# bluecube/codecad

Measured on AMD Instinct MI355X. Metric: SDF Mvoxels/s (grid_eval+subdivision), 512^3 menger_sponge, higher is better.
Workload: dtype f32

## Files before the change

### codecad_amd/csrc/hip_util.hip

```cpp
#include <hip/hip_runtime.h>
#include <hip/hiprtc.h>

#include <algorithm>
#include <atomic>
#include <cmath>
#include <cstdio>
#include <cstdlib>
#include <cstring>
#include <mutex>
#include <sstream>
#include <string>
#include <vector>

#include <dirent.h>
#include <dlfcn.h>
#include <fcntl.h>
#include <spawn.h>
#include <sys/stat.h>
#include <sys/wait.h>
#include <unistd.h>

extern char** environ;

#include "../../include/hip_util.h"
// ... 35 lines not shown
    size_t lds;
    size_t regfile_bytes;
    int voxels_per_lane;
};

}

struct hu_tape_s {
    Rec* recs_dev = nullptr;
    Rec* recs_do_dev = nullptr;
    float* extra_dev = nullptr;
    int n_instr = 0;
    int n_regs = 0;
    int n_slots = 0;
    int n_point_slots = 0, n_result_slots = 0;
    int flags = 0;
    sdf::SpecProgram program;
    struct SpecKernels* spec = nullptr;
    std::string spec_source;
    sdf::SpecMeta spec_meta;
};

namespace {

bool distance_only(const hu_tape_s* t)
{
    static const bool forced_full = [] { const char* e = getenv("HU_FULL_INTERPRETER"); return e && e[0] == '1'; }();
    return !forced_full && t->recs_do_dev != nullptr;
}

int launch_shape(const hu_tape_s* t, LaunchShape& ls, bool distance_only_kernel, int max_voxels_per_lane = 2,
                 bool lanes_are_independent = false)
{
    static const int forced = [] { const char* e = getenv("HU_VOXELS_PER_LANE"); return e ? atoi(e) : 0; }();
    const size_t lane_bytes = distance_only_kernel ? (size_t)t->n_point_slots * 16 + (size_t)t->n_result_slots * 4
                                                   : (size_t)t->n_slots * 16;
    const size_t two_voxel_limit = distance_only_kernel ? 48 * 1024 : 32 * 1024;
    const int by_rule = (forced == 1 || forced == 2) ? forced : ((lane_bytes * 2 * 256 <= two_voxel_limit) ? 2 : 1);
    const int wanted = by_rule < max_voxels_per_lane ? by_rule : max_voxels_per_lane;
    const Rec* prog = distance_only_kernel ? t->recs_do_dev : t->recs_dev;
    ls.prog = prog;
    ls.n4 = (uint32_t)(distance_only_kernel ? t->n_point_slots : t->n_slots);
    for (int n = wanted; n >= 1; --n) {
        const size_t per_lane = (distance_only_kernel ? (size_t)t->n_point_slots * 16 + (size_t)t->n_result_slots * 4
                                                      : (size_t)t->n_slots * 16) * n;
        uint32_t bs = 256;
        while (bs > 64 && per_lane * bs > 48 * 1024) bs >>= 1;
        auto waves_per_cu = [&](uint32_t lanes) {
            const size_t groups = kMaxLds / (per_lane * lanes + kScratchBytes), waves = groups * (lanes / 64u);
            return waves < 32 ? waves : (size_t)32;
        };
        static const uint32_t forced_block = [] { const char* e = getenv("HU_BLOCK"); return e ? (uint32_t)atoi(e) : 0u; }();
        if (forced_block == 64u || forced_block == 128u || forced_block == 256u) bs = forced_block < bs ? forced_block : bs;
        else if (lanes_are_independent && bs == 256u && waves_per_cu(64u) > waves_per_cu(256u)) bs = 64u;
        const size_t regfile = per_lane * bs;
        if (regfile + kScratchBytes <= kMaxLds) {
            ls.block = bs;
            ls.regfile_bytes = regfile;
            ls.lds = regfile + kScratchBytes;
            ls.voxels_per_lane = n;
            return HU_OK;
        }
    }
    return fail(HU_ERR_UNSUPPORTED, "tape keeps " + std::to_string(t->n_slots) +
                                        " values live at once; at most 159 fit the 160 KiB LDS register file");
}

template <typename K>
int allow_big_lds(K kernel)
{
    HU_HIP(hipFuncSetAttribute(reinterpret_cast<const void*>(kernel), hipFuncAttributeMaxDynamicSharedMemorySize, (int)kMaxLds));
    return HU_OK;
}

template <int N>
int ensure_attrs_n()
{
    int rc;
    if ((rc = allow_big_lds(k_grid_eval<InterpEval<false>, 0, N>))) return rc;
    if ((rc = allow_big_lds(k_grid_eval<InterpEval<false>, 1, N>))) return rc;
    if ((rc = allow_big_lds(k_grid_eval<InterpEval<true>, 1, N>))) return rc;
    if ((rc = allow_big_lds(k_grid_eval_blocks<InterpEval<false>, 0, N>))) return rc;
    if ((rc = allow_big_lds(k_grid_eval_blocks<InterpEval<false>, 1, N>))) return rc;
    if ((rc = allow_big_lds(k_grid_eval_blocks<InterpEval<true>, 1, N>))) return rc;
    if ((rc = allow_big_lds(k_classify<InterpEval<false>, false, false, N>))) return rc;
    if ((rc = allow_big_lds(k_classify<InterpEval<false>, false, true, N>))) return rc;
    if ((rc = allow_big_lds(k_classify<InterpEval<false>, true, false, N>))) return rc;
    if ((rc = allow_big_lds(k_classify<InterpEval<false>, true, true, N>))) return rc;
    if ((rc = allow_big_lds(k_classify<InterpEval<true>, false, false, N>))) return rc;
    if ((rc = allow_big_lds(k_classify<InterpEval<true>, false, true, N>))) return rc;
    if ((rc = allow_big_lds(k_classify<InterpEval<true>, true, false, N>))) return rc;
    if ((rc = allow_big_lds(k_classify<InterpEval<true>, true, true, N>))) return rc;
    return HU_OK;
}

int ensure_attrs()
{
    static thread_local int done_for_device = -1;
    int dev = 0;
    HU_HIP(hipGetDevice(&dev));
    if (done_for_device == dev) return HU_OK;
    int rc;
    if ((rc = ensure_attrs_n<1>())) return rc;
    if ((rc = ensure_attrs_n<2>())) return rc;
    HU_HIP(hu_render::allow_big_lds(kMaxLds));
    HU_HIP(hu_interference::allow_big_lds(kMaxLds));
    HU_HIP(hu_clearance::allow_big_lds(kMaxLds));
    done_for_device = dev;
    return HU_OK;
}

uint32_t brick_tiles(uint32_t nx, uint32_t sy, uint32_t sz)
{
    return (nx % 4u == 0u && sy % 4u == 0u && sz % 8u == 0u) ? 1u : 0u;
}
bool boxes_worthwhile(uint64_t nx, uint64_t sy, uint64_t sz)
{
    const uint64_t padded = ((nx + 3u) & ~3ull) * ((sy + 3u) & ~3ull) * ((sz + 7u) & ~7ull);
    return padded <= 2u * nx * sy * sz;
}

uint32_t units_per_launch(uint32_t chunks, uint32_t threads)
{
    const uint64_t by_items = 0xffffffffull / threads / chunks, by_groups = 0x7fffffffull / chunks;
    const uint64_t n = by_items < by_groups ? by_items : by_groups;
    return n < 1 ? 1u : (uint32_t)n;
}

int check_dims(const uint32_t dims[3], uint64_t& cells)
{
    if (!dims) return fail(HU_ERR_BAD_ARG, "dims is NULL");
    if (dims[0] == 0 || dims[1] == 0 || dims[2] == 0) return fail(HU_ERR_BAD_ARG, "dims must be >= 1 on every axis");
    cells = (uint64_t)dims[0] * dims[1] * dims[2];
    return HU_OK;
}

}

struct SpecKernels {
    std::vector<hipModule_t> modules;
    uint32_t groups = 0;
    hipFunction_t dense[2] = {nullptr, nullptr};
    hipFunction_t blocks[2] = {nullptr, nullptr};
    hipFunction_t dense_ragged[2] = {nullptr, nullptr};
    hipFunction_t blocks_ragged[2] = {nullptr, nullptr};
    hipFunction_t dense_runs[2] = {nullptr, nullptr};
    hipFunction_t blocks_runs[2] = {nullptr, nullptr};
    hipFunction_t classify[2][2] = {{nullptr, nullptr}, {nullptr, nullptr}};
    hipFunction_t ray_caster = nullptr, bitmap = nullptr;
    hipFunction_t box_masks = nullptr;
    bool deferred = false;
    double coord_limit = 0.0;
    int tabs[6] = {0, 0, 0, 0, 0, 0};
    int prune_words = 0;
    int prune_bits = 0;
    bool prune_all = false;
    struct MaskBuffer { hipStream_t stream; uint32_t* ptr; size_t bytes; };
    std::vector<MaskBuffer> mask_buffers;
};

namespace {

constexpr int kSpecVoxelsPerLane = 2;
constexpr uint32_t kSpecBlock = 256;

uint32_t spec_flags(const hu_tape_s* t, double max_abs_coordinate)
{
    static const bool off = [] { const char* e = getenv("HU_INRANGE"); return e && e[0] == '0'; }();
    return (!off && t->spec && max_abs_coordinate < t->spec->coord_limit) ? sdf::kFlagInRange : 0u;
}
double grid_reach(const float corner[3], float step, const uint32_t dims[3])
{
    double m = 0.0;
    for (int c = 0; c < 3; ++c) {
        const double a = std::fabs((double)corner[c]), b = std::fabs((double)corner[c] + (double)step * (double)dims[c]);
        m = std::max(m, std::max(a, b));
    }
    return m;
}
double list_reach(double resolution, double ox, double oy, double oz, double block_extent)
{
    return 2147483648.0 * std::fabs(resolution) + std::max(std::fabs(ox), std::max(std::fabs(oy), std::fabs(oz))) + std::fabs(block_extent);
}

bool defer_directions()
{
    static const bool off = [] { const char* e = getenv("HU_DEFER_DIRECTIONS"); return e && e[0] == '0'; }();
    return !off;
}

std::string generate_source(const hu_tape_s* t, sdf::SpecMeta* meta = nullptr)
{
    return sdf::specialised_source(t->program, defer_directions(), meta);
}
uint32_t box_table_bytes(const SpecKernels* k)
{
    return (uint32_t)((k->tabs[0] + k->tabs[1] + k->tabs[2]) * sdf::BoxTabs::kAxis + (k->tabs[3] + k->tabs[4]) * sdf::BoxTabs::kPairX +
                      k->tabs[5] * sdf::BoxTabs::kPairYZ) * 4u;
}

void keep_programs(hu_tape_s* t, const sdf::DecodedTape& d)
{
    t->program.full = d.recs;
    t->program.dist = d.recs_do;
    t->program.n_slots = d.n_slots;
    t->program.n_point_slots = d.n_point_slots;
    t->program.n_result_slots = d.n_result_slots;
}

struct SpecEval { const float* extra; uint32_t flags; };

constexpr int kSpecKernelCount = 19;
constexpr uint32_t spec_bit(int i) { return 1u << i; }
constexpr uint32_t kSpecGroupOf[kSpecKernelCount] = {spec_bit(0), spec_bit(1), spec_bit(2), spec_bit(3), spec_bit(4), spec_bit(5), spec_bit(6), spec_bit(7),
                                                      spec_bit(8), spec_bit(9), spec_bit(10), spec_bit(11), spec_bit(12), spec_bit(13), spec_bit(14),
                                                      spec_bit(15), spec_bit(16), spec_bit(17), spec_bit(18)};
static_assert(HU_SPEC_DENSE == (spec_bit(0) | spec_bit(1) | spec_bit(10) | spec_bit(11) | spec_bit(12) | spec_bit(15) | spec_bit(16)), "hip_util.h");
static_assert(HU_SPEC_BLOCKS == (spec_bit(2) | spec_bit(3) | spec_bit(10) | spec_bit(13) | spec_bit(14) | spec_bit(17) | spec_bit(18)), "hip_util.h");
static_assert(HU_SPEC_CLASSIFY == (spec_bit(4) | spec_bit(5) | spec_bit(6) | spec_bit(7) | spec_bit(10)), "hip_util.h");
static_assert(HU_SPEC_RENDER == (spec_bit(8) | spec_bit(9)), "hip_util.h");
static_assert(HU_SPEC_ALL == (HU_SPEC_DENSE | HU_SPEC_BLOCKS | HU_SPEC_CLASSIFY | HU_SPEC_RENDER) && HU_SPEC_ALL == spec_bit(kSpecKernelCount) - 1u, "hip_util.h");
const char* const kSpecKernelNames[kSpecKernelCount] = {
    "sdfk::k_grid_eval<sdfk::JitEval, 0, 2>",           "sdfk::k_grid_eval<sdfk::JitEval, 1, 2>",
    "sdfk::k_grid_eval_blocks<sdfk::JitEval, 0, 2>",    "sdfk::k_grid_eval_blocks<sdfk::JitEval, 1, 2>",
    "sdfk::k_classify<sdfk::JitEval, false, false, 2>", "sdfk::k_classify<sdfk::JitEval, false, true, 2>",
    "sdfk::k_classify<sdfk::JitEval, true, false, 2>",  "sdfk::k_classify<sdfk::JitEval, true, true, 2>",
    "sdfk::k_ray_caster<sdfk::JitEval>",                "sdfk::k_bitmap<sdfk::JitEval>",
    "sdfk::k_box_masks<sdfk::JitEval>",
    "sdfk::k_grid_eval_ragged<sdfk::JitEval, 0, 2>",        "sdfk::k_grid_eval_ragged<sdfk::JitEval, 1, 2>",
    "sdfk::k_grid_eval_blocks_ragged<sdfk::JitEval, 0, 2>", "sdfk::k_grid_eval_blocks_ragged<sdfk::JitEval, 1, 2>",
    "sdfk::k_grid_eval_runs<sdfk::JitEval, 0, 2>",          "sdfk::k_grid_eval_runs<sdfk::JitEval, 1, 2>",
    "sdfk::k_grid_eval_blocks_runs<sdfk::JitEval, 0, 2>",   "sdfk::k_grid_eval_blocks_runs<sdfk::JitEval, 1, 2>"};

int prepare_masks(hu_tape_s* t, MaskArgs& m, hipStream_t stream, const uint32_t** masks)
{
    *masks = nullptr;
    SpecKernels* k = t->spec;
    if (!k || !k->box_masks || k->prune_words <= 0 || m.n_boxes == 0) return HU_OK;
    static const bool off = [] { const char* e = getenv("HU_PRUNE_RUN"); return e && e[0] == '0'; }();
    if (off) return HU_OK;
    const size_t bytes = (size_t)m.n_boxes * (size_t)k->prune_words * sizeof(uint32_t);
    SpecKernels::MaskBuffer* buf = nullptr;
    for (auto& b : k->mask_buffers) if (b.stream == stream) buf = &b;
    if (!buf || buf->bytes < bytes) {
        hipStreamCaptureStatus capturing = hipStreamCaptureStatusNone;
        if (stream && hipStreamIsCapturing(stream, &capturing) == hipSuccess && capturing != hipStreamCaptureStatusNone) return HU_OK;
        (void)hipGetLastError();
        if (!buf) { k->mask_buffers.push_back(SpecKernels::MaskBuffer{stream, nullptr, 0}); buf = &k->mask_buffers.back(); }
        if (buf->ptr) HU_HIP(hipFree(buf->ptr));
        buf->ptr = nullptr; buf->bytes = 0;
        const size_t want = bytes + bytes / 2 + 4096;
        HU_HIP(hipMalloc((void**)&buf->ptr, want));
        buf->bytes = want;
    }
    m.out = buf->ptr;
    SpecEval ev{t->extra_dev, 0u};
    void* args[] = {&ev, &m};
    HU_HIP(hipModuleLaunchKernel(k->box_masks, (m.n_boxes + 63u) / 64u, 1, 1, 64, 1, 1, 0, stream, args, nullptr));
    *masks = buf->ptr;
    return HU_OK;
}

}

int hu_fail_external(int code, const char* message)
{
    if (code == HU_ERR_HIP) (void)hipGetLastError();
    return fail(code, message);
}

extern "C" {

int hu_abi_version(void) { return HU_ABI_VERSION; }
const char* hu_last_error(void) { return g_last_error.c_str(); }

int hu_device_count(int* count)
{
    if (!count) return fail(HU_ERR_BAD_ARG, "count is NULL");
    int n = 0;
    hipError_t e = hipGetDeviceCount(&n);
    if (e != hipSuccess) {
        *count = 0;
        return fail(HU_ERR_NO_DEVICE, std::string("hipGetDeviceCount: ") + hipGetErrorString(e));
    }
    *count = n;
    return HU_OK;
}

int hu_set_device(int ordinal)
{
    HU_HIP(hipSetDevice(ordinal));
    return HU_OK;
}

int hu_device_name(int ordinal, char* buf, size_t buflen)
{
    if (!buf || !buflen) return fail(HU_ERR_BAD_ARG, "buf is NULL");
    hipDeviceProp_t prop;
    HU_HIP(hipGetDeviceProperties(&prop, ordinal));
    std::snprintf(buf, buflen, "%s (%s, %d CUs)", prop.name, prop.gcnArchName, prop.multiProcessorCount);
    return HU_OK;
}

int hu_synchronize(void)
{
    HU_HIP(hipDeviceSynchronize());
    return HU_OK;
}

int hu_malloc(void** out_dev, size_t bytes)
{
    if (!out_dev) return fail(HU_ERR_BAD_ARG, "out_dev is NULL");
    *out_dev = nullptr;
    HU_HIP(hipMalloc(out_dev, bytes ? bytes : 1));
    return HU_OK;
}

int hu_free(void* dev)
{
    if (dev) HU_HIP(hipFree(dev));
    return HU_OK;
}

int hu_host_alloc(void** out_host, size_t bytes)
{
    if (!out_host) return fail(HU_ERR_BAD_ARG, "out_host is NULL");
    HU_HIP(hipHostMalloc(out_host, bytes ? bytes : 1, hipHostMallocDefault));
    return HU_OK;
}

int hu_host_free(void* host)
{
    if (host) HU_HIP(hipHostFree(host));
    return HU_OK;
}

int hu_memcpy_h2d(void* dst, const void* src, size_t n, void* stream)
{
    HU_HIP(hipMemcpyAsync(dst, src, n, hipMemcpyHostToDevice, (hipStream_t)stream));
    return HU_OK;
}

int hu_memcpy_d2h(void* dst, const void* src, size_t n, void* stream)
{
    HU_HIP(hipMemcpyAsync(dst, src, n, hipMemcpyDeviceToHost, (hipStream_t)stream));
    return HU_OK;
}

int hu_memcpy_d2d(void* dst, const void* src, size_t n, void* stream)
{
    HU_HIP(hipMemcpyAsync(dst, src, n, hipMemcpyDeviceToDevice, (hipStream_t)stream));
// ... 21 lines not shown
    return HU_OK;
}

int hu_stream_synchronize(void* s)
{
    HU_HIP(hipStreamSynchronize((hipStream_t)s));
    return HU_OK;
}

int hu_stream_wait_event(void* s, void* ev)
{
    HU_HIP(hipStreamWaitEvent((hipStream_t)s, (hipEvent_t)ev, 0));
    return HU_OK;
}

int hu_event_create(void** out)
{
    if (!out) return fail(HU_ERR_BAD_ARG, "out is NULL");
    hipEvent_t e;
    HU_HIP(hipEventCreate(&e));
    *out = e;
    return HU_OK;
}

int hu_event_destroy(void* e)
{
    if (e) HU_HIP(hipEventDestroy((hipEvent_t)e));
    return HU_OK;
}

int hu_event_record(void* e, void* s)
{
    HU_HIP(hipEventRecord((hipEvent_t)e, (hipStream_t)s));
    return HU_OK;
}

int hu_event_synchronize(void* e)
{
    HU_HIP(hipEventSynchronize((hipEvent_t)e));
    return HU_OK;
}

int hu_event_elapsed_ms(void* a, void* b, float* out_ms)
{
    if (!out_ms) return fail(HU_ERR_BAD_ARG, "out_ms is NULL");
    HU_HIP(hipEventElapsedTime(out_ms, (hipEvent_t)a, (hipEvent_t)b));
    return HU_OK;
}

int hu_tape_create(const float* tape, size_t n, hu_tape* out)
{
    if (!tape || !out) return fail(HU_ERR_BAD_ARG, "tape/out is NULL");
    *out = nullptr;
    sdf::DecodedTape d;
    std::string err = sdf::decode_tape(tape, n, d);
    if (!err.empty()) return fail(HU_ERR_BAD_TAPE, "malformed tape: " + err);
    hu_tape_s* t = new hu_tape_s();
    t->n_instr = d.n_instructions;
    t->n_regs = d.n_regs;
    t->n_slots = d.n_slots;
    t->n_point_slots = d.n_point_slots;
    t->n_result_slots = d.n_result_slots;
    t->flags = d.direction_feeds_distance ? 1 : 0;
    keep_programs(t, d);
    hipError_t e = hipMalloc((void**)&t->recs_dev, d.fused.size() * sizeof(Rec));
    if (e == hipSuccess && !d.fused_do.empty()) {
        e = hipMalloc((void**)&t->recs_do_dev, d.fused_do.size() * sizeof(Rec));
        if (e == hipSuccess) e = hipMemcpy(t->recs_do_dev, d.fused_do.data(), d.fused_do.size() * sizeof(Rec), hipMemcpyHostToDevice);
    }
    if (e == hipSuccess) e = hipMalloc((void**)&t->extra_dev, d.extra.size() * sizeof(float));
    if (e == hipSuccess) e = hipMemcpy(t->recs_dev, d.fused.data(), d.fused.size() * sizeof(Rec), hipMemcpyHostToDevice);
    if (e == hipSuccess) e = hipMemcpy(t->extra_dev, d.extra.data(), d.extra.size() * sizeof(float), hipMemcpyHostToDevice);
    if (e != hipSuccess) {
        (void)hipFree(t->recs_dev);
        (void)hipFree(t->recs_do_dev);
        (void)hipFree(t->extra_dev);
        delete t;
        return fail(HU_ERR_HIP, std::string("tape upload: ") + hipGetErrorString(e));
    }
    *out = t;
    return HU_OK;
}

int hu_tape_destroy(hu_tape t)
{
    if (!t) return HU_OK;
    if (t->spec) {
        for (auto& b : t->spec->mask_buffers) (void)hipFree(b.ptr);
        for (hipModule_t m : t->spec->modules) (void)hipModuleUnload(m);
        delete t->spec;
    }
    (void)hipFree(t->recs_dev);
    (void)hipFree(t->recs_do_dev);
    (void)hipFree(t->extra_dev);
    delete t;
    return HU_OK;
}

int hu_tape_info(hu_tape t, int* n_instructions, int* n_registers, int* flags)
{
    if (!t) return fail(HU_ERR_BAD_ARG, "tape is NULL");
    if (n_instructions) *n_instructions = t->n_instr;
    if (n_registers) *n_registers = t->n_slots;
    if (flags) *flags = t->flags;
    return HU_OK;
}

int hu_grid_eval_slab(hu_tape t, const float corner[4], float step, const uint32_t dims[3],
                      uint32_t x0, uint32_t x_count, int layout, void* out_dev, void* stream)
{
    if (!t || !corner || !out_dev) return fail(HU_ERR_BAD_ARG, "NULL argument");
    if (layout != 0 && layout != 1) return fail(HU_ERR_BAD_ARG, "layout must be 0 (float4) or 1 (pymcubes float)");
    uint64_t cells;
    int rc;
    if ((rc = check_dims(dims, cells))) return rc;
    if ((uint64_t)x0 + x_count > dims[0]) return fail(HU_ERR_BAD_ARG, "slab exceeds the grid's x extent");
    const uint64_t plane = (uint64_t)dims[1] * dims[2];
    if (plane >= (1ull << 30)) return fail(HU_ERR_BAD_ARG, "dims[1]*dims[2] must be below 2^30");
    const uint32_t spec_max_x = [&] { const uint32_t m = (uint32_t)((1ull << 30) / plane); return m >= 16u ? m & ~15u : m; }();
    const bool spec_ragged = t->spec && t->spec->deferred && !(brick_tiles(x_count, dims[1], dims[2]) && (x_count <= spec_max_x || spec_max_x % 4u == 0u));
    const bool spec_runs = spec_ragged && !boxes_worthwhile(x_count < spec_max_x ? x_count : spec_max_x, dims[1], dims[2]);
    if (t->spec && t->spec->dense[layout] && (!spec_ragged || (spec_runs ? t->spec->dense_runs[layout] : t->spec->dense_ragged[layout]))) {
        const uint32_t max_x = spec_max_x;
        SpecEval ev{t->extra_dev, spec_flags(t, grid_reach(corner, step, dims))};
        float cx = corner[0], cy = corner[1], cz = corner[2];
        uint32_t sx = dims[0];
        Dim sy = make_dim(dims[1]), sz = make_dim(dims[2]);
        for (uint32_t done = 0; done < x_count;) {
            const uint32_t nx = (x_count - done < max_x) ? (x_count - done) : max_x;
            uint32_t n_cells = (uint32_t)(nx * plane), xs = x0 + done;
            void* o = (layout == 0) ? (void*)(static_cast<float4*>(out_dev) + (size_t)done * plane) : out_dev;
            uint32_t boxes = (t->spec->deferred && !spec_runs) ? 1u : 0u;
            const bool ragged = boxes && !brick_tiles(nx, dims[1], dims[2]);
            static const uint32_t run_block = [] { const char* e = getenv("HU_RUN_BLOCK"); const int v = e ? atoi(e) : 0; return (v == 64 || v == 128 || v == 256) ? (uint32_t)v : 256u; }();
            const uint32_t block = boxes ? kSpecBlock : run_block;
            static const uint32_t store_bound_kib = [] { const char* e = getenv("HU_STORE_BOUND_LDS"); const int v = e ? atoi(e) : 40; return (uint32_t)((v >= 0 && v <= 64) ? v : 40); }();
            const uint32_t idle_lds = (layout == 0 && !boxes && !t->spec->deferred && t->n_instr <= 16) ? store_bound_kib * 1024u : 0u;
            const uint32_t per_block = block * kSpecVoxelsPerLane;
            uint32_t grid = (n_cells + per_block - 1) / per_block;
            const uint32_t* masks = nullptr;
            if (boxes) {
                grid = ((nx + 15u) / 16u) * ((dims[1] + 15u) / 16u) * ((dims[2] + 15u) / 16u);
                MaskArgs m{};
                m.mode = 0u; m.n_boxes = grid; m.chunks = grid; m.boxes_y = (dims[1] + 15u) / 16u; m.boxes_z = (dims[2] + 15u) / 16u;
                m.nx = nx; m.ny = dims[1]; m.nz = dims[2]; m.xs0 = xs; m.cx = cx; m.cy = cy; m.cz = cz; m.step = step;
                if ((layout == 1 || t->spec->prune_all) && (rc = prepare_masks(t, m, (hipStream_t)stream, &masks))) return rc;
            }
            if (spec_runs) {
                void* args[] = {&ev, &cx, &cy, &cz, &step, &sx, &sy, &sz, &xs, &n_cells, &o};
                HU_HIP(hipModuleLaunchKernel(t->spec->dense_runs[layout], grid, 1, 1, block, 1, 1, 0u, (hipStream_t)stream, args, nullptr));
            } else {
                void* args[] = {&ev, &cx, &cy, &cz, &step, &sx, &sy, &sz, &xs, &n_cells, &boxes, &o, &masks};
                HU_HIP(hipModuleLaunchKernel(ragged ? t->spec->dense_ragged[layout] : t->spec->dense[layout], grid, 1, 1, block, 1, 1,
                                             boxes ? box_table_bytes(t->spec) : idle_lds, (hipStream_t)stream, args, nullptr));
            }
            done += nx;
        }
        return HU_OK;
    }
    LaunchShape ls;
    if ((rc = launch_shape(t, ls, layout == 1 && distance_only(t), 2, true))) return rc;
    if ((rc = ensure_attrs())) return rc;
    const uint32_t max_x = (uint32_t)((1ull << 30) / plane);
    for (uint32_t done = 0; done < x_count;) {
        const uint32_t nx = (x_count - done < max_x) ? (x_count - done) : max_x;
        const uint32_t n_cells = (uint32_t)(nx * plane);
        const uint32_t per_block = ls.block * ls.voxels_per_lane;
        const uint32_t blocks = (n_cells + per_block - 1) / per_block;
        void* o = (layout == 0) ? (void*)(static_cast<float4*>(out_dev) + (size_t)done * plane) : out_dev;
#define HU_LAUNCH_DENSE(L, D, NV)                                                                                  \
    hipLaunchKernelGGL((k_grid_eval<InterpEval<D>, L, NV>), dim3(blocks), dim3(ls.block), ls.lds, (hipStream_t)stream, \
                       (InterpEval<D>{ls.prog, t->extra_dev, ls.n4}), corner[0], corner[1], corner[2], step, dims[0],  \
                       make_dim(dims[1]), make_dim(dims[2]), x0 + done, n_cells,                                       \
                       0u , o, (const uint32_t*)nullptr)
        const bool d_only = layout == 1 && distance_only(t);
        if (ls.voxels_per_lane == 2) {
            if (layout == 0) HU_LAUNCH_DENSE(0, false, 2);
            else if (d_only) HU_LAUNCH_DENSE(1, true, 2);
            else HU_LAUNCH_DENSE(1, false, 2);
        } else {
            if (layout == 0) HU_LAUNCH_DENSE(0, false, 1);
            else if (d_only) HU_LAUNCH_DENSE(1, true, 1);
            else HU_LAUNCH_DENSE(1, false, 1);
        }
#undef HU_LAUNCH_DENSE
        HU_HIP(hipGetLastError());
        done += nx;
    }
    return HU_OK;
}

int hu_grid_eval(hu_tape t, const float corner[4], float step, const uint32_t dims[3], void* out_dev, void* stream)
{
    if (!dims) return fail(HU_ERR_BAD_ARG, "dims is NULL");
    return hu_grid_eval_slab(t, corner, step, dims, 0, dims[0], 0, out_dev, stream);
}

int hu_grid_eval_pymcubes(hu_tape t, const float corner[4], float step, const uint32_t dims[3], void* out_dev, void* stream)
{
    if (!dims) return fail(HU_ERR_BAD_ARG, "dims is NULL");
    return hu_grid_eval_slab(t, corner, step, dims, 0, dims[0], 1, out_dev, stream);
}

static int grid_eval_blocks_impl(hu_tape t, const int32_t* blocks_dev, uint32_t n_blocks, const uint32_t* n_dev, double resolution,
                                 const double origin[3], float step, const uint32_t dims[3], int layout,
                                 void* out_dev, void* stream)
{
    if (!t || !origin || !out_dev || (!blocks_dev && n_blocks)) return fail(HU_ERR_BAD_ARG, "NULL argument");
    if (layout != 0 && layout != 1) return fail(HU_ERR_BAD_ARG, "layout must be 0 or 1");
    uint64_t cells;
    int rc;
    if ((rc = check_dims(dims, cells))) return rc;
    if (cells > (1ull << 24)) return fail(HU_ERR_BAD_ARG, "a block may have at most 2^24 cells (256^3)");
    if (n_blocks == 0) return HU_OK;
    const bool blocks_ragged = t->spec && t->spec->deferred && !brick_tiles(dims[0], dims[1], dims[2]);
    const bool blocks_runs = blocks_ragged && !boxes_worthwhile(dims[0], dims[1], dims[2]);
    if (t->spec && t->spec->blocks[layout] && (!blocks_ragged || (blocks_runs ? t->spec->blocks_runs[layout] : t->spec->blocks_ragged[layout]))) {
        const uint32_t per_block = kSpecBlock * kSpecVoxelsPerLane;
        uint32_t chunks = (uint32_t)((cells + per_block - 1) / per_block);
        uint32_t bricks = 0u;
        const bool ragged = blocks_ragged && !blocks_runs;
        if (t->spec->deferred && !blocks_runs) {
            const uint32_t bxn = (dims[0] + 15u) / 16u, byn = (dims[1] + 15u) / 16u, bzn = (dims[2] + 15u) / 16u;
            bricks = (byn << 16) | bzn;
            chunks = bxn * byn * bzn;
        }
        const double extent = (double)step * (double)std::max(dims[0], std::max(dims[1], dims[2]));
        SpecEval ev{t->extra_dev, spec_flags(t, list_reach(resolution, origin[0], origin[1], origin[2], extent))};
        const int4* b = (const int4*)blocks_dev;
        double res = resolution, ox = origin[0], oy = origin[1], oz = origin[2];
        uint32_t sx = dims[0];
        Dim sy = make_dim(dims[1]), sz = make_dim(dims[2]);
        const uint32_t piece = units_per_launch(chunks, kSpecBlock);
        for (uint32_t b0 = 0; b0 < n_blocks; b0 += piece) {
            uint32_t first = b0;
            const uint32_t count = n_blocks - b0 < piece ? n_blocks - b0 : piece;
            const uint32_t* masks = nullptr;
            if (bricks) {
                MaskArgs m{};
                m.mode = 1u; m.n_boxes = chunks * count; m.chunks = chunks; m.boxes_y = bricks >> 16; m.boxes_z = bricks & 0xffffu;
                m.nx = dims[0]; m.ny = dims[1]; m.nz = dims[2]; m.unit_base = b0; m.units = b; m.n_units_dev = n_dev; m.step = step;
                m.res = res; m.ox = ox; m.oy = oy; m.oz = oz;
                if ((layout == 1 || t->spec->prune_all) && (rc = prepare_masks(t, m, (hipStream_t)stream, &masks))) return rc;
            }
            if (blocks_runs) {
                void* args[] = {&ev, &b, &n_dev, &first, &chunks, &res, &ox, &oy, &oz, &step, &sx, &sy, &sz, &out_dev};
                HU_HIP(hipModuleLaunchKernel(t->spec->blocks_runs[layout], chunks * count, 1, 1, kSpecBlock, 1, 1, 0u, (hipStream_t)stream, args, nullptr));
            } else {
                void* args[] = {&ev, &b, &n_dev, &first, &chunks, &bricks, &res, &ox, &oy, &oz, &step, &sx, &sy, &sz, &out_dev, &masks};
                HU_HIP(hipModuleLaunchKernel(ragged ? t->spec->blocks_ragged[layout] : t->spec->blocks[layout], chunks * count, 1, 1, kSpecBlock, 1, 1,
                                             bricks ? box_table_bytes(t->spec) : 0u, (hipStream_t)stream, args, nullptr));
            }
        }
        return HU_OK;
    }
    LaunchShape ls;
    if ((rc = launch_shape(t, ls, layout == 1 && distance_only(t), 2, true))) return rc;
    if ((rc = ensure_attrs())) return rc;
    const uint32_t per_block = ls.block * ls.voxels_per_lane;
    const uint32_t chunks = (uint32_t)((cells + per_block - 1) / per_block);
    const dim3 block(ls.block);
    const uint32_t piece = units_per_launch(chunks, ls.block);
#define HU_LAUNCH_BLOCKS(L, D, NV)                                                                                 \
    hipLaunchKernelGGL((k_grid_eval_blocks<InterpEval<D>, L, NV>), grid, block, ls.lds, (hipStream_t)stream,           \
                       (InterpEval<D>{ls.prog, t->extra_dev, ls.n4}), (const int4*)blocks_dev, n_dev, b0, chunks, 0u, resolution, \
                       origin[0], origin[1], origin[2], step, dims[0], make_dim(dims[1]), make_dim(dims[2]), out_dev, (const uint32_t*)nullptr)
    const bool d_only = layout == 1 && distance_only(t);
    for (uint32_t b0 = 0; b0 < n_blocks; b0 += piece) {
        const dim3 grid(chunks * (n_blocks - b0 < piece ? n_blocks - b0 : piece));
        if (ls.voxels_per_lane == 2) {
            if (layout == 0) HU_LAUNCH_BLOCKS(0, false, 2);
            else if (d_only) HU_LAUNCH_BLOCKS(1, true, 2);
            else HU_LAUNCH_BLOCKS(1, false, 2);
        } else {
            if (layout == 0) HU_LAUNCH_BLOCKS(0, false, 1);
            else if (d_only) HU_LAUNCH_BLOCKS(1, true, 1);
            else HU_LAUNCH_BLOCKS(1, false, 1);
        }
    }
#undef HU_LAUNCH_BLOCKS
    HU_HIP(hipGetLastError());
    return HU_OK;
}

int hu_grid_eval_blocks(hu_tape t, const int32_t* blocks_dev, uint32_t n_blocks, double resolution,
                        const double origin[3], float step, const uint32_t dims[3], int layout,
                        void* out_dev, void* stream)
{
    return grid_eval_blocks_impl(t, blocks_dev, n_blocks, nullptr, resolution, origin, step, dims, layout, out_dev, stream);
}

int hu_grid_eval_blocks_indirect(hu_tape t, const int32_t* blocks_dev, const uint32_t* n_blocks_dev, uint32_t max_blocks,
                                 double resolution, const double origin[3], float step, const uint32_t dims[3], int layout,
                                 void* out_dev, void* stream)
{
    if (!n_blocks_dev) return fail(HU_ERR_BAD_ARG, "n_blocks_dev is NULL");
    return grid_eval_blocks_impl(t, blocks_dev, max_blocks, n_blocks_dev, resolution, origin, step, dims, layout, out_dev, stream);
}

}

namespace {

template <bool MASS, bool BATCH>
int launch_classify(hu_tape t, ClassifyArgs& a, uint32_t n_parents, const uint32_t dims[3], void* stream)
{
    uint64_t cells;
    int rc;
    if ((rc = check_dims(dims, cells))) return rc;
    if (cells > (1ull << 24)) return fail(HU_ERR_BAD_ARG, "at most 2^24 cells (256^3) per block: cell indices are uchar4");
    if (dims[0] > 256 || dims[1] > 256 || dims[2] > 256)
        return fail(HU_ERR_BAD_ARG, "grid size > 256 would overflow the uchar4 cell index (reference subdivision.py:206-208)");
    if (n_parents == 0) return HU_OK;
    if (t->spec && t->spec->classify[MASS ? 1 : 0][BATCH ? 1 : 0]) {
        const uint32_t per_block = kSpecBlock * kSpecVoxelsPerLane;
        a.sx = dims[0]; a.sy = dims[1]; a.sz = dims[2];
        a.dy = make_dim(dims[1]); a.dz = make_dim(dims[2]);
        a.chunks = (uint32_t)((cells + per_block - 1) / per_block);
        a.scratch_offset = 0;
        a.boxes = 0;

        const uint64_t bxn = (dims[0] + 15u) / 16u, byn = (dims[1] + 15u) / 16u, bzn = (dims[2] + 15u) / 16u;
        uint64_t enough = t->spec->prune_bits > 0 ? 64u : 8192u;
        if (const char* e = getenv("HU_CLASSIFY_BOX_MIN")) enough = (uint64_t)atoll(e);
        if (t->spec->deferred && cells > 256u && bxn * byn * bzn * n_parents >= enough && boxes_worthwhile(dims[0], dims[1], dims[2])) {
            a.boxes = ((uint32_t)byn << 16) | (uint32_t)bzn;
            a.chunks = (uint32_t)(bxn * byn * bzn);
            a.scratch_offset = box_table_bytes(t->spec);
        }
        const double extent = (double)a.step * (double)std::max(dims[0], std::max(dims[1], dims[2]));
        const float c3[3] = {a.cx, a.cy, a.cz};
        const double reach = !BATCH ? grid_reach(c3, a.step, dims)
                             : MASS ? HUGE_VAL
                                    : list_reach(a.res, a.ox, a.oy, a.oz, extent + std::fabs((double)a.int_step * a.res));
        SpecEval ev{t->extra_dev, spec_flags(t, reach)};
        const uint32_t piece = units_per_launch(a.chunks, kSpecBlock);
        for (uint32_t p0 = 0; p0 < n_parents; p0 += piece) {
            a.parent_base = p0;
            a.masks = nullptr;
            if (a.boxes) {
                MaskArgs m{};
                m.mode = !BATCH ? 2u : MASS ? 4u : 3u;
                m.n_boxes = a.chunks * (n_parents - p0 < piece ? n_parents - p0 : piece); m.chunks = a.chunks;
                m.boxes_y = a.boxes >> 16; m.boxes_z = a.boxes & 0xffffu; m.nx = dims[0]; m.ny = dims[1]; m.nz = dims[2];
                m.unit_base = p0; m.units = a.parents; m.n_units_dev = a.n_parents_dev; m.cx = a.cx; m.cy = a.cy; m.cz = a.cz; m.step = a.step;
                m.int_step = a.int_step; m.dimension = a.dimension; m.res = a.res; m.ox = a.ox; m.oy = a.oy; m.oz = a.oz; m.s = a.s;
                if ((rc = prepare_masks(t, m, (hipStream_t)stream, &a.masks))) return rc;
            }
            void* args[] = {&ev, &a};
            HU_HIP(hipModuleLaunchKernel(t->spec->classify[MASS ? 1 : 0][BATCH ? 1 : 0],
                                         a.chunks * (n_parents - p0 < piece ? n_parents - p0 : piece), 1, 1, kSpecBlock, 1, 1,
                                         (unsigned)(a.scratch_offset + kScratchBytes), (hipStream_t)stream, args, nullptr));
        }
        return HU_OK;
    }
    LaunchShape ls;
    if ((rc = launch_shape(t, ls, distance_only(t)))) return rc;
    if ((rc = ensure_attrs())) return rc;
    a.sx = dims[0];
    a.sy = dims[1];
    a.sz = dims[2];
    a.dy = make_dim(dims[1]);
    a.dz = make_dim(dims[2]);
    const uint32_t per_block = ls.block * ls.voxels_per_lane;
    a.chunks = (uint32_t)((cells + per_block - 1) / per_block);
    a.scratch_offset = (uint32_t)ls.regfile_bytes;
    a.boxes = 0;
    a.masks = nullptr;
    const dim3 block(ls.block);
    const bool d_only = distance_only(t);
    const uint32_t piece = units_per_launch(a.chunks, ls.block);
#define HU_LAUNCH_CLASSIFY(D, NV)                                                                                \
    hipLaunchKernelGGL((k_classify<InterpEval<D>, MASS, BATCH, NV>), grid, block, ls.lds, (hipStream_t)stream,     \
                       (InterpEval<D>{ls.prog, t->extra_dev, ls.n4}), a)
    for (uint32_t p0 = 0; p0 < n_parents; p0 += piece) {
        a.parent_base = p0;
        const dim3 grid(a.chunks * (n_parents - p0 < piece ? n_parents - p0 : piece));
        if (ls.voxels_per_lane == 2) {
            if (d_only) HU_LAUNCH_CLASSIFY(true, 2);
            else HU_LAUNCH_CLASSIFY(false, 2);
        } else {
            if (d_only) HU_LAUNCH_CLASSIFY(true, 1);
            else HU_LAUNCH_CLASSIFY(false, 1);
        }
    }
#undef HU_LAUNCH_CLASSIFY
    HU_HIP(hipGetLastError());
    return HU_OK;
}

}

extern "C" {

int hu_subdivision_step(hu_tape t, const float corner[4], float step, float threshold, const uint32_t dims[3],
                        uint32_t* counter_dev, void* list_dev, void* stream)
{
    if (!t || !corner || !counter_dev || !list_dev) return fail(HU_ERR_BAD_ARG, "NULL argument");
    ClassifyArgs a;
    std::memset(&a, 0, sizeof(a));
    a.cx = corner[0]; a.cy = corner[1]; a.cz = corner[2];
    a.step = step; a.thr = threshold;
    a.counter = counter_dev; a.list = list_dev; a.capacity = 0xffffffffu;
    return launch_classify<false, false>(t, a, 1, dims, stream);
}

int hu_mass_properties(hu_tape t, const float corner[4], float step, float threshold, const uint32_t dims[3],
                       uint32_t* sum_dev, uint32_t* counter_dev, void* list_dev, void* stream)
{
    if (!t || !corner || !sum_dev || !counter_dev || !list_dev) return fail(HU_ERR_BAD_ARG, "NULL argument");
    ClassifyArgs a;
    std::memset(&a, 0, sizeof(a));
    a.cx = corner[0]; a.cy = corner[1]; a.cz = corner[2];
    a.step = step; a.thr = threshold;
    a.counter = counter_dev; a.list = list_dev; a.capacity = 0xffffffffu;
    a.sums = sum_dev;
    return launch_classify<true, false>(t, a, 1, dims, stream);
}

int hu_subdivision_level(hu_tape t, const int32_t* parents_dev, uint32_t n_parents, int32_t int_step,
                         const uint32_t dims[3], int dimension, double resolution, const double origin[3],
                         float step, float threshold, uint32_t* counter_dev, int32_t* children_dev,
                         uint32_t capacity, void* stream)
{
    if (!t || !origin || !counter_dev || (!children_dev && capacity) || (!parents_dev && n_parents))
        return fail(HU_ERR_BAD_ARG, "NULL argument");
    if (dimension != 2 && dimension != 3) return fail(HU_ERR_BAD_ARG, "dimension must be 2 or 3");
    ClassifyArgs a;
    std::memset(&a, 0, sizeof(a));
    a.parents = parents_dev;
    a.int_step = int_step; a.dimension = dimension;
    a.res = resolution; a.ox = origin[0]; a.oy = origin[1]; a.oz = origin[2];
    a.step = step; a.thr = threshold;
    a.counter = counter_dev; a.list = children_dev; a.capacity = capacity;
    return launch_classify<false, true>(t, a, n_parents, dims, stream);
}

int hu_subdivision_level_indirect(hu_tape t, const int32_t* parents_dev, const uint32_t* n_parents_dev, uint32_t max_parents,
                                  int32_t int_step, const uint32_t dims[3], int dimension, double resolution,
                                  const double origin[3], float step, float threshold, uint32_t* counter_dev,
                                  int32_t* children_dev, uint32_t capacity, void* stream)
{
    if (!t || !origin || !counter_dev || !n_parents_dev || (!children_dev && capacity) || (!parents_dev && max_parents))
        return fail(HU_ERR_BAD_ARG, "NULL argument");
    if (dimension != 2 && dimension != 3) return fail(HU_ERR_BAD_ARG, "dimension must be 2 or 3");
    ClassifyArgs a;
    std::memset(&a, 0, sizeof(a));
    a.parents = parents_dev;
    a.n_parents_dev = n_parents_dev;
    a.int_step = int_step; a.dimension = dimension;
    a.res = resolution; a.ox = origin[0]; a.oy = origin[1]; a.oz = origin[2];
    a.step = step; a.thr = threshold;
    a.counter = counter_dev; a.list = children_dev; a.capacity = capacity;
    return launch_classify<false, true>(t, a, max_parents, dims, stream);
}

int hu_subdivision_level_owned(hu_tape t, const int32_t* parents_dev, const uint32_t* n_parents_dev, uint32_t max_parents,
                               int32_t int_step, const uint32_t dims[3], int dimension, double resolution,
                               const double origin[3], float step, float threshold, uint32_t* counter_dev,
                               int32_t* children_dev, uint32_t capacity, uint32_t world, uint32_t rank, void* stream)
{
    if (!t || !origin || !counter_dev || !n_parents_dev || (!children_dev && capacity) || (!parents_dev && max_parents))
        return fail(HU_ERR_BAD_ARG, "NULL argument");
    if (dimension != 2 && dimension != 3) return fail(HU_ERR_BAD_ARG, "dimension must be 2 or 3");
    if (world == 0 || rank >= world) return fail(HU_ERR_BAD_ARG, "rank must be below world");
    ClassifyArgs a;
    std::memset(&a, 0, sizeof(a));
    a.parents = parents_dev;
    a.n_parents_dev = n_parents_dev;
    a.int_step = int_step; a.dimension = dimension;
    a.res = resolution; a.ox = origin[0]; a.oy = origin[1]; a.oz = origin[2];
    a.step = step; a.thr = threshold;
    a.counter = counter_dev; a.list = children_dev; a.capacity = capacity;
    a.own = make_dim(world); a.own_rank = rank;
    return launch_classify<false, true>(t, a, max_parents, dims, stream);
}

int hu_mass_properties_level_owned(hu_tape t, const double* parents_dev, const uint32_t* n_parents_dev, uint32_t max_parents, double s,
                                   const uint32_t dims[3], float step, float threshold, uint32_t* sums_dev,
                                   uint32_t* counter_dev, double* children_dev, uint32_t capacity, uint32_t world, uint32_t rank, void* stream)
{
// ... 628 lines not shown
    for (int i = 0; i < kSpecKernelCount; ++i)
        if (kSpecGroupOf[i] & groups) (void)hiprtcAddNameExpression(prog, kSpecKernelNames[i]);
    std::vector<const char*> opts;
    for (const std::string& w : options) opts.push_back(w.c_str());
    const hiprtcResult rc = hiprtcCompileProgram(prog, (int)opts.size(), opts.data());
    if (rc != HIPRTC_SUCCESS) {
        size_t n = 0;
        std::string log;
        if (hiprtcGetProgramLogSize(prog, &n) == HIPRTC_SUCCESS && n > 1) {
            log.resize(n);
            (void)hiprtcGetProgramLog(prog, &log[0]);
        }
        (void)hiprtcDestroyProgram(&prog);
        return fail(HU_ERR_UNSUPPORTED, std::string("hipRTC compile failed: ") + hiprtcGetErrorString(rc) + "\n" + log.substr(0, 4000));
    }
    size_t size = 0;
    (void)hiprtcGetCodeSize(prog, &size);
    img.code.resize(size);
    (void)hiprtcGetCode(prog, img.code.data());
    img.lowered.clear();
    for (int i = 0; i < kSpecKernelCount; ++i) {
        if (!(kSpecGroupOf[i] & groups)) continue;
        const char* name = kSpecKernelNames[i];
        const char* lowered = nullptr;
        if (hiprtcGetLoweredName(prog, name, &lowered) != HIPRTC_SUCCESS || !lowered) {
            (void)hiprtcDestroyProgram(&prog);
            return fail(HU_ERR_UNSUPPORTED, std::string("kernel missing from the specialised module: ") + name);
        }
        img.lowered.emplace_back(lowered);
    }
    (void)hiprtcDestroyProgram(&prog);
    return HU_OK;
}

static int specialised_image(const std::string& src, const char* include_dir, const char* cache_dir, bool only_if_cached, uint32_t groups,
                             SpecImage& img, int* from_cache, bool replace_cached = false)
{
    if (from_cache) *from_cache = 0;
    img.code.clear();
    const std::vector<std::string> options = spec_options(include_dir, spec_source_is_big(src.size()));
    uint64_t key[2];
    std::string path;
    const bool cached = cache_dir && *cache_dir && spec_cache_key(src, include_dir, options, groups, key);
    if (cached) {
        path = spec_cache_path(cache_dir, key);
        if (!replace_cached && spec_cache_load(path, key, groups, img)) {
            if (from_cache) *from_cache = 1;
            return HU_OK;
        }
        img.code.clear();
    }
    if (only_if_cached) return HU_OK;
    int rc = HU_ERR_UNSUPPORTED;
    for (int attempt = 0; attempt < 2 && rc != HU_OK; ++attempt) {
        const std::string pch = spec_pch(include_dir, cache_dir, options, g_pch_beside_refused);
        if (pch.empty()) break;
        std::vector<std::string> with = options;
        with.push_back("-include-pch");
        with.push_back(pch);
        if ((rc = compile_specialised(src, with, groups, img))) {
            const bool in_dir = cache_dir && *cache_dir && pch.compare(0, std::strlen(cache_dir), cache_dir) == 0;
            if (in_dir) {
                g_pch_refused = true;
                (void)std::remove(pch.c_str());
            } else {
                g_pch_beside_refused = true;
            }
        }
    }
    if (rc != HU_OK && (rc = compile_specialised(src, options, groups, img))) return rc;
    if (cached) {
        spec_cache_store(cache_dir, path, key, img);
        spec_cache_prune(cache_dir);
    }
    return HU_OK;
}

int hu_tape_compile_cached(const float* tape, size_t n, const char* include_dir, const char* cache_dir, size_t* code_bytes,
                           int* from_cache)
{
    return hu_tape_compile_groups(tape, n, include_dir, cache_dir, HU_SPEC_ALL, code_bytes, from_cache);
}

int hu_tape_compile_groups(const float* tape, size_t n, const char* include_dir, const char* cache_dir, uint32_t groups,
                           size_t* code_bytes, int* from_cache)
{
    if (!tape || !include_dir) return fail(HU_ERR_BAD_ARG, "NULL argument");
    if (groups == 0 || (groups & ~(uint32_t)HU_SPEC_ALL)) return fail(HU_ERR_BAD_ARG, "groups must be a non-empty set of HU_SPEC_* bits");
    sdf::DecodedTape d;
    const std::string err = sdf::decode_tape(tape, n, d);
    if (!err.empty()) return fail(HU_ERR_BAD_TAPE, "malformed tape: " + err);
    hu_tape_s t;
    t.n_slots = d.n_slots;
    keep_programs(&t, d);
    SpecImage img;
    int rc;
    if ((rc = specialised_image(generate_source(&t), include_dir, cache_dir, false, groups, img, from_cache))) return rc;
    if (code_bytes) *code_bytes = img.code.size();
    return HU_OK;
}

int hu_spec_pch_prepare(const char* include_dir, const char* dir, char* path, size_t capacity)
{
    if (!include_dir || !dir) return fail(HU_ERR_BAD_ARG, "NULL argument");
    const std::string pch = spec_pch(include_dir, dir, spec_options(include_dir, false), true);
    const std::string pch_big = spec_pch(include_dir, dir, spec_options(include_dir, true), true);
    if (path && capacity) std::snprintf(path, capacity, "%s%s%s", pch.c_str(), (pch.empty() || pch_big.empty()) ? "" : "\n", pch_big.c_str());
    return HU_OK;
}

int hu_tape_compile_check(const float* tape, size_t n, const char* include_dir, size_t* code_bytes)
{
    return hu_tape_compile_cached(tape, n, include_dir, nullptr, code_bytes, nullptr);
}

int hu_tape_specialize_cached(hu_tape t, const char* include_dir, const char* cache_dir, int only_if_cached, int* from_cache)
{
    return hu_tape_specialize_groups(t, include_dir, cache_dir, only_if_cached, HU_SPEC_ALL, from_cache);
}

static int load_specialised(hu_tape t, const SpecImage& img, uint32_t set, hipError_t* why)
{
    hipModule_t module = nullptr;
    hipFunction_t loaded[kSpecKernelCount] = {};
    hipError_t e = hipModuleLoadData(&module, img.code.data());
    size_t next = 0;
    for (int i = 0; i < kSpecKernelCount && e == hipSuccess; ++i)
        if (kSpecGroupOf[i] & set) e = (next < img.lowered.size()) ? hipModuleGetFunction(&loaded[i], module, img.lowered[next++].c_str()) : hipErrorNotFound;
    if (e != hipSuccess) {
        if (module) (void)hipModuleUnload(module);
        (void)hipGetLastError();
        if (why) *why = e;
        return HU_ERR_HIP;
    }
    if (!t->spec) t->spec = new SpecKernels();
    SpecKernels* k = t->spec;
    hipFunction_t* slots[kSpecKernelCount] = {&k->dense[0], &k->dense[1], &k->blocks[0], &k->blocks[1],
                                              &k->classify[0][0], &k->classify[0][1], &k->classify[1][0], &k->classify[1][1],
                                              &k->ray_caster, &k->bitmap, &k->box_masks,
                                              &k->dense_ragged[0], &k->dense_ragged[1], &k->blocks_ragged[0], &k->blocks_ragged[1],
                                              &k->dense_runs[0], &k->dense_runs[1], &k->blocks_runs[0], &k->blocks_runs[1]};
    const uint32_t missing = set & ~k->groups;
    for (int i = 0; i < kSpecKernelCount; ++i)
        if (kSpecGroupOf[i] & missing) *slots[i] = loaded[i];
    k->modules.push_back(module);
    k->groups |= missing;
    const sdf::SpecMeta& meta = t->spec_meta;
    k->deferred = meta.deferred;
    k->coord_limit = meta.coord_limit;
    k->prune_words = meta.prune_words;
    k->prune_bits = meta.prune_bits;
    k->prune_all = meta.prune_all;
    std::memcpy(k->tabs, meta.tabs, sizeof k->tabs);
    return HU_OK;
}

int hu_tape_specialize_groups(hu_tape t, const char* include_dir, const char* cache_dir, int only_if_cached, uint32_t groups, int* from_cache)
{
    if (from_cache) *from_cache = 0;
    if (!t || !include_dir) return fail(HU_ERR_BAD_ARG, "NULL argument");
    if (groups & ~(uint32_t)HU_SPEC_ALL) return fail(HU_ERR_BAD_ARG, "groups must be a set of HU_SPEC_* bits");
    auto missing = [&] { return t->spec ? (groups & ~t->spec->groups) : groups; };
    if (missing() == 0) return HU_OK;
    if (t->spec_source.empty()) t->spec_source = generate_source(t, &t->spec_meta);
    const std::string& src = t->spec_source;
    const bool cache = cache_dir && *cache_dir;
    bool all_cached = true;
    for (int step = 0; step < 3 && missing(); ++step) {
        if (step < 2 && !cache) continue;
        if (step == 2 && only_if_cached) break;
        std::vector<uint32_t> sets;
        if (step == 1) {
            for (int i = 0; i < kSpecKernelCount; ++i)
                if ((kSpecGroupOf[i] & missing()) && kSpecGroupOf[i] != groups) sets.push_back(kSpecGroupOf[i]);
        } else {
            sets.push_back(step == 0 ? groups : missing());
        }
        for (uint32_t set : sets) {
            for (int attempt = 0; attempt < 2; ++attempt) {
                SpecImage img;
                int crc, cached = 0;
                if ((crc = specialised_image(src, include_dir, cache_dir, step < 2, set, img, &cached, attempt != 0))) return crc;
                if (img.code.empty()) break;
                hipError_t e = hipSuccess;
                if (load_specialised(t, img, set, &e) == HU_OK) {
                    all_cached = all_cached && cached;
                    break;
                }
                if (step < 2) break;
                if (!cached || attempt == 1) return fail(HU_ERR_HIP, std::string("loading the specialised module: ") + hipGetErrorString(e));
            }
        }
    }
    if (from_cache) *from_cache = (all_cached && missing() == 0) ? 1 : 0;
    return HU_OK;
}

int hu_tape_specialize(hu_tape t, const char* include_dir) { return hu_tape_specialize_cached(t, include_dir, nullptr, 0, nullptr); }

static int launch_process_polygon(bool batch, PolygonArgs& a, uint32_t n_blocks, void* stream)
{
    if (a.gx < 2 || a.gy < 2) return fail(HU_ERR_BAD_ARG, "the corner grid needs at least 2x2 samples");
    if (a.gx > 512 || a.gy > 512) return fail(HU_ERR_BAD_ARG, "corner grids above 512 overflow the link encoding (polygon2d.py:46)");
    if (n_blocks == 0) return HU_OK;
    if (n_blocks > 65535u) return fail(HU_ERR_BAD_ARG, "at most 65535 blocks per launch");
    const uint32_t cells = (a.gx - 1u) * (a.gy - 1u) * 2u;
    HU_HIP(hu_render::process_polygon(batch, a, dim3((cells + 255u) / 256u, n_blocks), (hipStream_t)stream));
    return HU_OK;
}

int hu_process_polygon(const float box_corner[2], float box_step, const void* corners_dev, const uint32_t grid[2],
                       void* vertices_dev, uint32_t* links_dev, uint32_t* starts_dev, uint32_t* start_counter_dev,
                       void* stream)
{
    if (!box_corner || !corners_dev || !grid || !vertices_dev || !links_dev || !starts_dev || !start_counter_dev)
        return fail(HU_ERR_BAD_ARG, "NULL argument");
    PolygonArgs a{};
    a.corners = static_cast<const float4*>(corners_dev);
    a.gx = grid[0] + 1u;
    a.gy = grid[1] + 1u;
    a.cx = box_corner[0];
    a.cy = box_corner[1];
    a.step = box_step;
    a.vertices = static_cast<float2*>(vertices_dev);
    a.links = links_dev;
    a.starts = starts_dev;
    a.start_counter = start_counter_dev;
    return launch_process_polygon(false, a, 1, stream);
}

int hu_process_polygon_blocks(const void* corners_dev, const int32_t* blocks_dev, uint32_t n_blocks, double resolution,
                              const double origin[3], float step, const uint32_t dims[2], void* vertices_dev,
                              uint32_t* links_dev, uint32_t* starts_dev, uint32_t* start_counters_dev, void* stream)
{
    if (!origin || !dims) return fail(HU_ERR_BAD_ARG, "NULL argument");
    if (n_blocks && (!corners_dev || !blocks_dev || !vertices_dev || !links_dev || !starts_dev || !start_counters_dev))
        return fail(HU_ERR_BAD_ARG, "NULL argument");
    PolygonArgs a{};
    a.corners = static_cast<const float4*>(corners_dev);
    a.gx = dims[0];
    a.gy = dims[1];
    a.step = step;
    a.blocks = reinterpret_cast<const int4*>(blocks_dev);
    a.res = resolution;
    a.ox = origin[0];
    a.oy = origin[1];
    a.vertices = static_cast<float2*>(vertices_dev);
    a.links = links_dev;
    a.starts = starts_dev;
    a.start_counter = start_counters_dev;
    return launch_process_polygon(true, a, n_blocks, stream);
}

int hu_selftest_math(uint64_t counts[4])
{
    if (!counts) return fail(HU_ERR_BAD_ARG, "counts is NULL");
    unsigned long long* dev = nullptr;
    HU_HIP(hipMalloc((void**)&dev, 4 * sizeof(unsigned long long)));
    hipError_t e = hipMemset(dev, 0, 4 * sizeof(unsigned long long));
    if (e == hipSuccess) {
        e = hu_render::selftest_math(dev);
    }
    unsigned long long host[4] = {0, 0, 0, 0};
    if (e == hipSuccess) e = hipMemcpy(host, dev, sizeof host, hipMemcpyDeviceToHost);
    (void)hipFree(dev);
    if (e != hipSuccess) return fail(HU_ERR_HIP, std::string("hu_selftest_math: ") + hipGetErrorString(e));
    for (int i = 0; i < 4; ++i) counts[i] = host[i];
    return HU_OK;
}

int hu_selftest_minmax3(uint64_t counts[3])
{
    if (!counts) return fail(HU_ERR_BAD_ARG, "counts is NULL");
    unsigned long long* dev = nullptr;
    HU_HIP(hipMalloc((void**)&dev, 3 * sizeof(unsigned long long)));
    hipError_t e = hipMemset(dev, 0, 3 * sizeof(unsigned long long));
    if (e == hipSuccess) e = hu_render::selftest_minmax3(dev);
    unsigned long long host[3] = {0, 0, 0};
    if (e == hipSuccess) e = hipMemcpy(host, dev, sizeof host, hipMemcpyDeviceToHost);
    (void)hipFree(dev);
    if (e != hipSuccess) return fail(HU_ERR_HIP, std::string("hu_selftest_minmax3: ") + hipGetErrorString(e));
    for (int i = 0; i < 3; ++i) counts[i] = host[i];
    return HU_OK;
}

int hu_tape_source(const float* tape, size_t n, char* buf, size_t capacity, size_t* needed)
{
    if (!tape || !needed || (!buf && capacity)) return fail(HU_ERR_BAD_ARG, "NULL argument");
    sdf::DecodedTape d;
    const std::string err = sdf::decode_tape(tape, n, d);
    if (!err.empty()) return fail(HU_ERR_BAD_TAPE, "malformed tape: " + err);
    hu_tape_s t;
    t.n_slots = d.n_slots;
    keep_programs(&t, d);
    const std::string src = generate_source(&t);
    *needed = src.size() + 1;
    if (capacity >= src.size() + 1) std::memcpy(buf, src.c_str(), src.size() + 1);
    return HU_OK;
}

int hu_tape_listing(const float* tape, size_t n, int which, char* buf, size_t capacity, size_t* needed)
{
    if (!tape || !needed || (!buf && capacity)) return fail(HU_ERR_BAD_ARG, "NULL argument");
    if (which < 0 || which > 3) return fail(HU_ERR_BAD_ARG, "which must be 0..3");
    sdf::DecodedTape d;
    const std::string err = sdf::decode_tape(tape, n, d);
// ... 57 lines not shown
```

### codecad_amd/csrc/kernels.hpp

```cpp
#pragma once

#include "interp.hpp"

#ifdef SDF_WAVES_PER_EU
#define SDF_KERNEL_ATTRS __attribute__((amdgpu_waves_per_eu(SDF_WAVES_PER_EU, SDF_WAVES_PER_EU)))
#else
#define SDF_KERNEL_ATTRS
#endif

namespace sdfk {

using sdf::Rec;

template <bool DO> struct InterpEval {
    static constexpr bool kBricks = false;
    const Rec* prog;
    const float* extra;
    uint32_t n4;
    template <class T> __device__ __forceinline__ sdf::V4<T> operator()(T px, T py, T pz, void* lds) const
    {
        sdf::Regs<T> regs(lds, threadIdx.x, blockDim.x, n4);
        return sdf::run_tape<T, DO>(prog, extra, px, py, pz, regs);
    }
    template <class T> __device__ __forceinline__ T dist(T px, T py, T pz, void* lds) const { return (*this)(px, py, pz, lds).w; }
};


__device__ __forceinline__ float sample(float corner, float step, uint32_t i) { return corner + step * (float)i; }

struct Dim {
    uint32_t n, m, s;
};
inline Dim make_dim(uint32_t n)
{
    if (n <= 1u) return Dim{n, 0u, 0u};
    uint32_t L = 0;
    while ((1ull << L) < n) ++L;
    return Dim{n, (uint32_t)((((1ull << L) - n) << 32) / n + 1ull), L - 1u};
}
__device__ __forceinline__ uint32_t div(uint32_t x, Dim d)
{
    const uint32_t t = __umulhi(d.m, x);
    const uint32_t q = (t + ((x - t) >> 1)) >> d.s;
    return d.n == 1u ? x : q;
}

#ifndef SDF_NT_STORES
#define SDF_NT_STORES 0
#endif
typedef float f4v __attribute__((ext_vector_type(4)));
__device__ __forceinline__ void store_voxel(float4* p, float4 v)
{
#if SDF_NT_STORES
    f4v t;
    t.x = v.x; t.y = v.y; t.z = v.z; t.w = v.w;
    __builtin_nontemporal_store(t, reinterpret_cast<f4v*>(p));
#else
    *p = v;
#endif
}
__device__ __forceinline__ void store_voxel(float* p, float v)
{
#if SDF_NT_STORES
    __builtin_nontemporal_store(v, p);
#else
    *p = v;
#endif
}

template <int N> struct Pack { using T = float; };
template <> struct Pack<2> { using T = sdf::f2; };
__device__ __forceinline__ float pack(const float (&v)[1]) { return v[0]; }
__device__ __forceinline__ sdf::f2 pack(const float (&v)[2]) { return sdf::make_f2(v[0], v[1]); }

template <int N> struct Cells {
    uint32_t x[N], y[N], z[N];
    bool active[N];
    __device__ __forceinline__ Cells(uint32_t lin0, uint32_t n_cells, Dim dy, Dim dz, uint32_t stride = 1u)
    {
        const uint32_t sy = dy.n, sz = dz.n;
#pragma unroll
        for (int i = 0; i < N; ++i) {
            if (i == 0 || stride != 1u) {
                const uint32_t lin = lin0 + (uint32_t)i * stride;
                active[i] = lin < n_cells;
                const uint32_t l = active[i] ? lin : 0u;
                const uint32_t t = div(l, dz);
                z[i] = l - t * sz;
                x[i] = div(t, dy);
                y[i] = t - x[i] * sy;
            } else {
                active[i] = active[0] && (lin0 + i < n_cells);
                const bool wrap_z = z[i - 1] + 1u == sz;
                const bool wrap_y = wrap_z && (y[i - 1] + 1u == sy);
                z[i] = wrap_z ? 0u : z[i - 1] + 1u;
                y[i] = wrap_y ? 0u : (wrap_z ? y[i - 1] + 1u : y[i - 1]);
                x[i] = wrap_y ? x[i - 1] + 1u : x[i - 1];
            }
        }
    }
    __device__ __forceinline__ typename Pack<N>::T position(float corner, float step, const uint32_t (&c)[N], uint32_t c0 = 0) const
    {
        float v[N];
#pragma unroll
        for (int i = 0; i < N; ++i) v[i] = sample(corner, step, c0 + c[i]);
        return pack(v);
    }
};
__device__ __forceinline__ uint32_t sx_slab(uint32_t n_cells, uint32_t sy, uint32_t sz) { return n_cells / (sy * sz); }

template <int N> __device__ __forceinline__ uint32_t first_cell(uint32_t block)
{
    return (block * blockDim.x + (threadIdx.x & ~63u)) * N + (threadIdx.x & 63u);
}
constexpr uint32_t kLaneStride = 64u;

template <int N>
__device__ __forceinline__ void wg_compact_slots(const bool (&flag)[N], uint32_t* __restrict__ counter, uint32_t* scratch,
                                                 uint32_t (&slot)[N])
{
    const uint32_t lane = threadIdx.x & 63u, wave = threadIdx.x >> 6;
    const uint64_t below = (1ull << lane) - 1ull;
    uint32_t prefix = 0, total_w = 0;
#pragma unroll
    for (int i = 0; i < N; ++i) {
        const uint64_t mask = __ballot(flag[i]);
        prefix += __popcll(mask & below);
        total_w += __popcll(mask);
    }
    if (lane == 0) scratch[wave] = total_w;
    __syncthreads();
    if (threadIdx.x == 0) {
        const uint32_t nw = (blockDim.x + 63u) >> 6;
        uint32_t total = 0;
        for (uint32_t w = 0; w < nw; ++w) {
            uint32_t c = scratch[w];
            scratch[w] = total;
            total += c;
        }
        scratch[4] = total ? atomicAdd(counter, total) : 0u;
    }
    __syncthreads();
    slot[0] = scratch[4] + scratch[wave] + prefix;
#pragma unroll
    for (int i = 1; i < N; ++i) slot[i] = slot[i - 1] + (flag[i - 1] ? 1u : 0u);
}

__device__ __forceinline__ uint32_t wave_sum_to_last_lane(uint32_t v)
{
    v += (uint32_t)__builtin_amdgcn_update_dpp(0, (int)v, 0x111, 0xf, 0xf, false);
    v += (uint32_t)__builtin_amdgcn_update_dpp(0, (int)v, 0x112, 0xf, 0xf, false);
    v += (uint32_t)__builtin_amdgcn_update_dpp(0, (int)v, 0x114, 0xf, 0xf, false);
    v += (uint32_t)__builtin_amdgcn_update_dpp(0, (int)v, 0x118, 0xf, 0xf, false);
    v += (uint32_t)__builtin_amdgcn_update_dpp(0, (int)v, 0x142, 0xa, 0xf, false);
    v += (uint32_t)__builtin_amdgcn_update_dpp(0, (int)v, 0x143, 0xc, 0xf, false);
    return v;
}

struct BoxOut {
    void* out;
    size_t base;
    uint32_t sxa, sy, sz, xa;
    uint32_t nx;
};
template <class E> __device__ __forceinline__ float walk_coordinate(float v)
{
    if constexpr (E::kPruneAll) return sdf::opaque(v);
    else return v;
}
struct BoxTables {
    sdf::lds_float *x, *y, *z, *xy, *xz, *yz;
};
template <class E, class PR>
__device__ __forceinline__ BoxTables box_tables(const E& ev, float4* lds, float cx, float cy, float cz, float step, uint32_t xs0,
                                                uint32_t x0, uint32_t y0, uint32_t z0, uint32_t nx, uint32_t ny, uint32_t nz, const PR& pr)
{
    const uint32_t lane = threadIdx.x & 63u, wave = threadIdx.x >> 6;
    constexpr int NX = E::kTabXX, NY = E::kTabXY, NZ = E::kTabXZ, NXY = E::kPairXY, NXZ = E::kPairXZ, NYZ = E::kPairYZ;
    using Tabs = sdf::BoxTabs;
    sdf::lds_float* const tx = (sdf::lds_float*)lds;
    sdf::lds_float* const ty = tx + NX * Tabs::kAxis;
    sdf::lds_float* const tz = ty + NY * Tabs::kAxis;
    sdf::lds_float* const txy = tz + NZ * Tabs::kAxis;
    sdf::lds_float* const txz = txy + NXY * Tabs::kPairX;
    sdf::lds_float* const tyz = txz + NXZ * Tabs::kPairX;
    if constexpr (NX + NY + NZ > 0) {
        if (wave == 0u) {
            if constexpr (NX > 0)
                if (lane < nx) ev.template tab_x_x<Tabs::kAxis>(sample(cx, step, xs0 + x0 + lane), tx + lane);
        } else if (wave == 1u) {
            if constexpr (NY > 0)
                if (lane < ny) ev.template tab_x_y<Tabs::kAxis>(sample(cy, step, y0 + lane), ty + lane);
        } else if (wave == 2u) {
            if constexpr (NZ > 0)
                if (lane < nz) ev.template tab_x_z<Tabs::kAxis>(sample(cz, step, z0 + lane), tz + lane);
        }
        __syncthreads();
    }
    if constexpr (NXY + NXZ + NYZ > 0) {
        const uint32_t r = threadIdx.x >> 4, c = threadIdx.x & 15u;
        if constexpr (NXY > 0)
            if (r < ny && c < nx)
                ev.template tab_x_xy<Tabs::kPairX>(sample(cx, step, xs0 + x0 + c), sample(cy, step, y0 + r), Tabs{tx + c, ty + r, tz, txy, txz, tyz}, pr,
                                                   txy + (r * Tabs::kRowX + c));
        if constexpr (NXZ > 0)
            if (r < nz && c < nx)
                ev.template tab_x_xz<Tabs::kPairX>(sample(cx, step, xs0 + x0 + c), sample(cz, step, z0 + r), Tabs{tx + c, ty, tz + r, txy, txz, tyz}, pr,
                                                   txz + (r * Tabs::kRowX + c));
        if constexpr (NYZ > 0)
            if (r < ny && c < nz)
                ev.template tab_x_yz<Tabs::kPairYZ>(sample(cy, step, y0 + r), sample(cz, step, z0 + c), Tabs{tx, ty + r, tz + c, txy, txz, tyz}, pr,
                                                    tyz + (r * Tabs::kRowYZ + c));
        __syncthreads();
    }
    return BoxTables{tx, ty, tz, txy, txz, tyz};
}

template <class E, int LAYOUT, int N, bool RAGGED = false>
__device__ __forceinline__ void box_eval(const E& ev, float4* lds, float cx, float cy, float cz, float step, uint32_t xs0,
                                         uint32_t x0, uint32_t y0, uint32_t z0, const BoxOut& o, const uint32_t* __restrict__ masks,
                                         uint32_t box = blockIdx.x)
{
    using T = typename Pack<N>::T;
    using Tabs = sdf::BoxTabs;
    const uint32_t lane = threadIdx.x & 63u, wave = threadIdx.x >> 6;
    const uint32_t sx = o.sxa, sy = o.sy, sz = o.sz;
    const uint32_t nx = min(16u, o.nx - x0), ny = min(16u, sy - y0), nz = min(16u, sz - z0);
    const sdf::Prune<E::kPruneWords> pr = sdf::load_prune<E::kPruneWords>(masks, box);
    const BoxTables t = box_tables(ev, lds, cx, cy, cz, step, xs0, x0, y0, z0, nx, ny, nz, pr);
    sdf::lds_float* const tx = t.x; sdf::lds_float* const ty = t.y; sdf::lds_float* const tz = t.z;
    sdf::lds_float* const txy = t.xy; sdf::lds_float* const txz = t.xz; sdf::lds_float* const tyz = t.yz;
    const uint32_t nbz = RAGGED ? (nz + 7u) >> 3 : nz >> 3;
    const uint32_t bz = nbz == 2u ? (wave & 1u) : 0u, dby = 4u / nbz;
    const uint32_t zl = bz * 8u + (lane & 7u), z = z0 + zl, xl = lane >> 5;
    const bool z_inside = !RAGGED || zl < nz;
    const float pz = sample(cz, step, z);
    uint32_t yl = (nbz == 2u ? (wave >> 1) : wave) * 4u + ((lane >> 3) & 3u);
    Tabs col{tx + xl, ty + yl, tz + zl, txy + (yl * Tabs::kRowX + xl), txz + (zl * Tabs::kRowX + xl), tyz + (yl * Tabs::kRowYZ + zl)};
    const size_t plane = (size_t)sy * sz;
    size_t at = LAYOUT == 0 ? o.base + ((size_t)z + (size_t)sz * ((size_t)(y0 + yl) + (size_t)sy * (x0 + xl)))
                            : o.base + ((size_t)z + ((size_t)(o.xa + x0 + xl) + (size_t)(sy - 1u - (y0 + yl)) * sx) * sz);
    const size_t second = LAYOUT == 0 ? 2u * plane : 2u * (size_t)sz, brick = 2u * second;
    const size_t rows = (size_t)(4u * dby) * (LAYOUT == 0 ? (size_t)sz : (size_t)sx * sz);
    const uint32_t row_in_brick = (lane >> 3) & 3u, bricks_x = RAGGED ? (nx + 3u) >> 2 : nx >> 2;
    for (; (RAGGED ? yl - row_in_brick : yl) < ny; yl += 4u * dby) {
        const float py = sample(cy, step, y0 + yl);
        const bool row_inside = !RAGGED || (z_inside && yl < ny);
        Tabs tb = col;
        const auto hoisted = ev.hoist_x(py, walk_coordinate<E>(pz), tb, pr);
        size_t p = at;
#pragma unroll 1
        for (uint32_t j = 0; j < bricks_x; ++j) {
            asm volatile("" ::: "memory");
            float xs[N];
#pragma unroll
            for (int i = 0; i < N; ++i) xs[i] = sample(cx, step, xs0 + x0 + j * 4u + xl + 2u * i);
            const T px = pack(xs);
            const float pyb = walk_coordinate<E>(py), pzb = walk_coordinate<E>(pz);
            const auto prb = pr.fresh();
            if (LAYOUT == 0) {
                const sdf::V4<T> r = ev.eval_hoisted_x(px, pyb, pzb, hoisted, tb, prb);
#pragma unroll
                for (int i = 0; i < N; ++i)
                    if (!RAGGED || (row_inside && j * 4u + xl + 2u * (uint32_t)i < nx))
                        store_voxel(static_cast<float4*>(o.out) + p + (size_t)i * second, sdf::voxel(r, i));
            } else {
                const T w = ev.dist_hoisted_x(px, pyb, pzb, hoisted, tb, prb);
#pragma unroll
                for (int i = 0; i < N; ++i)
                    if (!RAGGED || (row_inside && j * 4u + xl + 2u * (uint32_t)i < nx))
                        store_voxel(static_cast<float*>(o.out) + p + (size_t)i * second, sdf::get(w, i));
            }
            tb.x += 4; tb.xy += 4; tb.xz += 4;
            p += brick;
        }
        col.y += 4u * dby; col.xy += 4u * dby * Tabs::kRowX; col.yz += 4u * dby * Tabs::kRowYZ;
        at = LAYOUT == 0 ? at + rows : at - rows;
    }
}

template <class E, int LAYOUT, int N>
__device__ __forceinline__ void grid_eval_runs(const E& ev, float4* lds, float cx, float cy, float cz, float step, uint32_t sx, Dim dy, Dim dz,
                                               uint32_t x0, uint32_t n_cells, void* __restrict__ out);

template <class E, int LAYOUT, int N, bool RAGGED>
__device__ __forceinline__ void grid_eval_boxes(const E& ev, float4* lds, float cx, float cy, float cz, float step, uint32_t sx, uint32_t sy, uint32_t sz,
                                                uint32_t x0, uint32_t n_cells, void* __restrict__ out, const uint32_t* __restrict__ masks)
{
    const uint32_t nx_slab = sx_slab(n_cells, sy, sz);
    const uint32_t boxes_z = (sz + 15u) >> 4, boxes_y = (sy + 15u) >> 4;
    uint32_t b = blockIdx.x;
#if !defined(SDF_BOX_ORDER) || SDF_BOX_ORDER
    {
        const uint32_t k = b & 7u, q = gridDim.x >> 3, r = gridDim.x & 7u;
        b = k * q + (k < r ? k : r) + (b >> 3);
    }
#endif
    const uint32_t qz = b % boxes_z, qt = b / boxes_z, qy = qt % boxes_y, qx = qt / boxes_y;
    const BoxOut o{out, 0, sx, sy, sz, LAYOUT == 0 ? 0u : x0, nx_slab};
    box_eval<E, LAYOUT, N, RAGGED>(ev, lds, cx, cy, cz, step, x0, qx * 16u, qy * 16u, qz * 16u, o, masks, b);
}

template <class E, int LAYOUT, int N>
__global__ void __launch_bounds__(256) SDF_KERNEL_ATTRS
k_grid_eval(const E ev, float cx, float cy, float cz, float step, uint32_t sx, Dim dy, Dim dz, uint32_t x0,
            uint32_t n_cells, uint32_t boxes, void* __restrict__ out, const uint32_t* __restrict__ masks)
{
    extern __shared__ float4 lds[];
    if constexpr (E::kBricks && N == 2) {
        grid_eval_boxes<E, LAYOUT, N, false>(ev, lds, cx, cy, cz, step, sx, dy.n, dz.n, x0, n_cells, out, masks);
    } else {
        grid_eval_runs<E, LAYOUT, N>(ev, lds, cx, cy, cz, step, sx, dy, dz, x0, n_cells, out);
    }
}
template <class E, int LAYOUT, int N>
__global__ void __launch_bounds__(256) SDF_KERNEL_ATTRS
k_grid_eval_ragged(const E ev, float cx, float cy, float cz, float step, uint32_t sx, Dim dy, Dim dz, uint32_t x0,
                   uint32_t n_cells, uint32_t boxes, void* __restrict__ out, const uint32_t* __restrict__ masks)
{
    extern __shared__ float4 lds[];
    if constexpr (E::kBricks && N == 2) grid_eval_boxes<E, LAYOUT, N, true>(ev, lds, cx, cy, cz, step, sx, dy.n, dz.n, x0, n_cells, out, masks);
}

template <class E, int LAYOUT, int N>
__global__ void __launch_bounds__(256) SDF_KERNEL_ATTRS
k_grid_eval_runs(const E ev, float cx, float cy, float cz, float step, uint32_t sx, Dim dy, Dim dz, uint32_t x0,
                 uint32_t n_cells, void* __restrict__ out)
{
    extern __shared__ float4 lds[];
    if constexpr (E::kBricks) grid_eval_runs<E, LAYOUT, N>(ev, lds, cx, cy, cz, step, sx, dy, dz, x0, n_cells, out);
}

template <class E, int LAYOUT, int N>
__device__ __forceinline__ void grid_eval_runs(const E& ev, float4* lds, float cx, float cy, float cz, float step, uint32_t sx, Dim dy, Dim dz,
                                               uint32_t x0, uint32_t n_cells, void* __restrict__ out)
{
    const uint32_t sy = dy.n, sz = dz.n;
    using T = typename Pack<N>::T;
    const uint32_t lin0 = first_cell<N>(blockIdx.x);
    const Cells<N> c(lin0, n_cells, dy, dz, kLaneStride);
    const T px = c.position(cx, step, c.x, x0), py = c.position(cy, step, c.y), pz = c.position(cz, step, c.z);
    if (LAYOUT == 0) {
        const sdf::V4<T> r = ev(px, py, pz, lds);
#pragma unroll
        for (int i = 0; i < N; ++i) {
            if (!c.active[i]) continue;
            store_voxel(static_cast<float4*>(out) + lin0 + (uint32_t)i * kLaneStride, sdf::voxel(r, i));
        }
    } else {
        const T w = ev.dist(px, py, pz, lds);
#pragma unroll
        for (int i = 0; i < N; ++i) {
            if (!c.active[i]) continue;
            const size_t idx = (size_t)c.z[i] + ((size_t)(x0 + c.x[i]) + (size_t)(sy - 1u - c.y[i]) * sx) * sz;
            store_voxel(static_cast<float*>(out) + idx, sdf::get(w, i));
        }
    }
}

template <class E, int LAYOUT, int N, bool BOXES, bool RAGGED = false>
__device__ __forceinline__ void grid_eval_blocks_body(const E& ev, float4* lds, const int4* __restrict__ blocks, const uint32_t* __restrict__ n_blocks_dev,
                                                      uint32_t b0, uint32_t chunks, uint32_t bricks, double res, double ox, double oy, double oz, float step,
                                                      uint32_t sx, Dim dy, Dim dz, void* __restrict__ out, const uint32_t* __restrict__ masks)
{
    const uint32_t sy = dy.n, sz = dz.n;
    using T = typename Pack<N>::T;
    const uint32_t chunk = blockIdx.x % chunks, b = b0 + blockIdx.x / chunks;
    if (n_blocks_dev && b >= *n_blocks_dev) return;
    const uint32_t cells = sx * sy * sz;
    const int4 ic = blocks[b];
    const float cx = (float)((double)ic.x * res + ox);
    const float cy = (float)((double)ic.y * res + oy);
    const float cz = (float)((double)ic.z * res + oz);
    if constexpr (BOXES) {
        const uint32_t boxes_z = bricks & 0xffffu, boxes_y = bricks >> 16;
        const uint32_t qz = chunk % boxes_z, qt = chunk / boxes_z, qy = qt % boxes_y, qx = qt / boxes_y;
        const BoxOut o{out, (size_t)b * cells, sx, sy, sz, 0u, sx};
        box_eval<E, LAYOUT, N, RAGGED>(ev, lds, cx, cy, cz, step, 0u, qx * 16u, qy * 16u, qz * 16u, o, masks);
        return;
    }
    const uint32_t lin0 = first_cell<N>(chunk);
    const Cells<N> c(lin0, cells, dy, dz, kLaneStride);
    const T px = c.position(cx, step, c.x), py = c.position(cy, step, c.y), pz = c.position(cz, step, c.z);
    const size_t base = (size_t)b * cells;
    if (LAYOUT == 0) {
        const sdf::V4<T> r = ev(px, py, pz, lds);
#pragma unroll
        for (int i = 0; i < N; ++i)
            if (c.active[i]) store_voxel(static_cast<float4*>(out) + base + lin0 + (uint32_t)i * kLaneStride, sdf::voxel(r, i));
    } else {
        const T w = ev.dist(px, py, pz, lds);
#pragma unroll
        for (int i = 0; i < N; ++i)
            if (c.active[i])
                store_voxel(static_cast<float*>(out) + base + (size_t)c.z[i] + ((size_t)c.x[i] + (size_t)(sy - 1u - c.y[i]) * sx) * sz, sdf::get(w, i));
    }
}
template <class E, int LAYOUT, int N>
__global__ void __launch_bounds__(256) SDF_KERNEL_ATTRS
k_grid_eval_blocks(const E ev, const int4* __restrict__ blocks, const uint32_t* __restrict__ n_blocks_dev, uint32_t b0,
                   uint32_t chunks, uint32_t bricks, double res, double ox, double oy, double oz, float step, uint32_t sx,
                   Dim dy, Dim dz, void* __restrict__ out, const uint32_t* __restrict__ masks)
{
    extern __shared__ float4 lds[];
    grid_eval_blocks_body<E, LAYOUT, N, (E::kBricks && N == 2)>(ev, lds, blocks, n_blocks_dev, b0, chunks, bricks, res, ox, oy, oz, step, sx, dy, dz, out, masks);
}
template <class E, int LAYOUT, int N>
__global__ void __launch_bounds__(256) SDF_KERNEL_ATTRS
k_grid_eval_blocks_ragged(const E ev, const int4* __restrict__ blocks, const uint32_t* __restrict__ n_blocks_dev, uint32_t b0,
                          uint32_t chunks, uint32_t bricks, double res, double ox, double oy, double oz, float step, uint32_t sx,
                          Dim dy, Dim dz, void* __restrict__ out, const uint32_t* __restrict__ masks)
{
    extern __shared__ float4 lds[];
    if constexpr (E::kBricks && N == 2)
        grid_eval_blocks_body<E, LAYOUT, N, true, true>(ev, lds, blocks, n_blocks_dev, b0, chunks, bricks, res, ox, oy, oz, step, sx, dy, dz, out, masks);
}

template <class E, int LAYOUT, int N>
__global__ void __launch_bounds__(256) SDF_KERNEL_ATTRS
k_grid_eval_blocks_runs(const E ev, const int4* __restrict__ blocks, const uint32_t* __restrict__ n_blocks_dev, uint32_t b0,
                        uint32_t chunks, double res, double ox, double oy, double oz, float step, uint32_t sx, Dim dy, Dim dz,
                        void* __restrict__ out)
{
    extern __shared__ float4 lds[];
    if constexpr (E::kBricks)
        grid_eval_blocks_body<E, LAYOUT, N, false>(ev, lds, blocks, n_blocks_dev, b0, chunks, 0u, res, ox, oy, oz, step, sx, dy, dz, out, nullptr);
}

struct ClassifyArgs {
    const void* parents;
    uint32_t parent_base;
    const uint32_t* n_parents_dev;
    uint32_t chunks;
    uint32_t sx, sy, sz;
    Dim dy, dz;
    float cx, cy, cz;
    float step, thr;
    int32_t int_step;
    int32_t dimension;
    double res, ox, oy, oz;
    double s;
    uint32_t* counter;
    void* list;
    uint32_t capacity;
    uint32_t* sums;
    uint32_t scratch_offset;
    uint32_t boxes;
    const uint32_t* masks;
    Dim own;
    uint32_t own_rank;
};
__device__ __forceinline__ uint32_t row_hash(uint32_t a, uint32_t b, uint32_t c, uint32_t d)
{
    uint32_t h = a * 0x9e3779b1u;
    h = (h ^ (h >> 15)) + b * 0x85ebca77u;
    h = (h ^ (h >> 13)) + c * 0xc2b2ae3du;
    h = (h ^ (h >> 16)) + d * 0x27d4eb2fu;
    return h ^ (h >> 15);
}
__device__ __forceinline__ bool owned(const ClassifyArgs& a, uint32_t parent_hash, uint32_t cell)
{
    uint32_t v = parent_hash + cell * 0x9e3779b1u;
    v = (v ^ (v >> 15)) * 0x85ebca77u;
    v ^= v >> 13;
    const bool mine = v - div(v, a.own) * a.own.n == a.own_rank;
    return a.own.n <= 1u ? true : mine;
}

template <class E, bool MASS, bool BATCH, int N>
__global__ void __launch_bounds__(256) k_classify(const E ev, const ClassifyArgs a)
{
    using T = typename Pack<N>::T;
    extern __shared__ float4 lds[];
    uint32_t* scratch = reinterpret_cast<uint32_t*>(reinterpret_cast<char*>(lds) + a.scratch_offset);
    const uint32_t b = BATCH ? a.parent_base + blockIdx.x / a.chunks : 0u;
    const uint32_t chunk = BATCH ? blockIdx.x % a.chunks : blockIdx.x;
    const uint32_t cells = a.sx * a.sy * a.sz;
    if (BATCH && a.n_parents_dev && b >= *a.n_parents_dev) return;

    float cx = a.cx, cy = a.cy, cz = a.cz;
    int4 ipar = make_int4(0, 0, 0, 0);
    double pcx = 0.0, pcy = 0.0, pcz = 0.0, pcw = 0.0;
    if (BATCH) {
        if (MASS) {
            const double4 pc = static_cast<const double4*>(a.parents)[b];
            pcx = pc.x; pcy = pc.y; pcz = pc.z; pcw = pc.w;
            const double h = a.s / 2;
            cx = (float)(pcx + h); cy = (float)(pcy + h); cz = (float)(pcz + h);
        } else {
            ipar = static_cast<const int4*>(a.parents)[b];
            const double h = (double)a.int_step / 2;
            cx = (float)(((double)ipar.x + h) * a.res + a.ox);
            cy = (float)(((double)ipar.y + h) * a.res + a.oy);
            cz = (float)(((double)ipar.z + (a.dimension == 3 ? h : 0.0)) * a.res + a.oz);
        }
    }
    if (MASS) {
        if (threadIdx.x < 10) scratch[8 + threadIdx.x] = 0u;
    }
    const uint32_t phash = !BATCH ? 0u
                           : MASS ? row_hash((uint32_t)__double2loint(pcx) ^ (uint32_t)__double2hiint(pcx), (uint32_t)__double2loint(pcy) ^ (uint32_t)__double2hiint(pcy),
                                             (uint32_t)__double2loint(pcz) ^ (uint32_t)__double2hiint(pcz), (uint32_t)__double2loint(pcw) ^ (uint32_t)__double2hiint(pcw))
                                  : row_hash((uint32_t)ipar.x, (uint32_t)ipar.y, (uint32_t)ipar.z, (uint32_t)ipar.w);

    if constexpr (E::kBricks && N == 2) {
        if (a.boxes) {
            using Tabs = sdf::BoxTabs;
            const uint32_t lane = threadIdx.x & 63u, wave = threadIdx.x >> 6;
            const uint32_t boxes_z = a.boxes & 0xffffu, boxes_y = a.boxes >> 16;
            const uint32_t qz = chunk % boxes_z, qt = chunk / boxes_z, qy = qt % boxes_y, qx = qt / boxes_y;
            const uint32_t x0 = qx * 16u, y0 = qy * 16u, z0 = qz * 16u;
            const uint32_t nx = min(16u, a.sx - x0), ny = min(16u, a.sy - y0), nz = min(16u, a.sz - z0);
            const sdf::Prune<E::kPruneWords> pr = sdf::load_prune<E::kPruneWords>(a.masks, blockIdx.x);
            const BoxTables t = box_tables(ev, lds, cx, cy, cz, a.step, 0u, x0, y0, z0, nx, ny, nz, pr);
            if (MASS) __syncthreads();
            const bool nothing_ambiguous = MASS && a.thr == 0.0f;
            const uint64_t below = (1ull << lane) - 1ull;
            uint32_t v[10] = {0, 0, 0, 0, 0, 0, 0, 0, 0, 0};
            constexpr uint32_t kStep = (uint32_t)Tabs::kPairStep;
            const uint32_t x_end = x0 + nx;
            auto brick = [&](uint32_t xv, uint32_t y, uint32_t z, float py, float pz, const Tabs& tb, const auto& hoisted, bool live) {
                const T px = sdf::make_f2(sample(cx, a.step, xv), sample(cx, a.step, xv + kStep));
                const T w = ev.dist_hoisted_x(px, walk_coordinate<E>(py), walk_coordinate<E>(pz), hoisted, tb, pr.fresh());
                bool amb[2];
#pragma unroll
                for (int i = 0; i < 2; ++i) {
                    const float wi = sdf::get(w, i);
                    const uint32_t x = xv + kStep * (uint32_t)i;
                    const bool mine = live & (x < x_end) & owned(a, phash, z + a.sz * (y + a.sy * x));
                    if (MASS) {
                        const bool in = wi <= -a.thr, inside = in && mine;
                        amb[i] = mine && !in && (wi < a.thr);
                        const uint32_t m = inside ? 1u : 0u;
                        const uint32_t xm = inside ? x : 0u, ym = inside ? y : 0u, zm = inside ? z : 0u;
                        v[0] += __umul24(xm, x); v[1] += __umul24(xm, y); v[2] += __umul24(xm, z); v[3] += xm;
                        v[4] += __umul24(ym, y); v[5] += __umul24(ym, z); v[6] += ym;
                        v[7] += __umul24(zm, z); v[8] += zm; v[9] += m;
                    } else {
                        amb[i] = mine && (wi > -a.thr) && (wi < a.thr);
                    }
                }
                if (!nothing_ambiguous) {
                    const uint64_t m0 = __ballot(amb[0]), m1 = __ballot(amb[1]);
                    const uint32_t n0 = __popcll(m0), total = n0 + __popcll(m1);
                    if (total) {
                        uint32_t base = 0u;
                        if (lane == 0u) base = atomicAdd(a.counter, total);
                        base = __builtin_amdgcn_readfirstlane(base);
                        const uint32_t slot[2] = {base + (uint32_t)__popcll(m0 & below), base + n0 + (uint32_t)__popcll(m1 & below)};
#pragma unroll
                        for (int i = 0; i < 2; ++i) {
                            if (!(amb[i] && slot[i] < a.capacity)) continue;
                            const uint32_t x = xv + kStep * (uint32_t)i;
                            if (!BATCH) {
                                static_cast<uchar4*>(a.list)[slot[i]] = make_uchar4((unsigned char)x, (unsigned char)y, (unsigned char)z, 0);
                            } else if (MASS) {
                                static_cast<double4*>(a.list)[slot[i]] =
                                    make_double4((double)x * a.s + pcx, (double)y * a.s + pcy, (double)z * a.s + pcz, pcw);
                            } else {
                                static_cast<int4*>(a.list)[slot[i]] =
                                    make_int4(ipar.x + (int)x * a.int_step, ipar.y + (int)y * a.int_step, ipar.z + (int)z * a.int_step, ipar.w);
                            }
                        }
                    }
                }
            };
            const uint32_t nbz = (nz + 7u) >> 3, bz = nbz == 2u ? (wave & 1u) : 0u, dby = 4u / nbz;
            const uint32_t zl = bz * 8u + (lane & 7u), z = z0 + zl, xl = lane >> 5;
            const float pz = sample(cz, a.step, z);
            const uint32_t row_in_brick = (lane >> 3) & 3u;
            for (uint32_t yl = (nbz == 2u ? (wave >> 1) : wave) * 4u + row_in_brick; yl - row_in_brick < ny; yl += 4u * dby) {
                const uint32_t y = y0 + yl;
                const bool live = (zl < nz) & (yl < ny);
                const float py = sample(cy, a.step, y);
                Tabs tb{t.x + xl, t.y + yl, t.z + zl, t.xy + (yl * Tabs::kRowX + xl), t.xz + (zl * Tabs::kRowX + xl), t.yz + (yl * Tabs::kRowYZ + zl)};
                const auto hoisted = ev.hoist_x(py, walk_coordinate<E>(pz), tb, pr);
#pragma unroll 1
                for (uint32_t j = 0; j < ((nx + 3u) >> 2); ++j) {
                    asm volatile("" ::: "memory");
                    brick(x0 + j * 4u + xl, y, z, py, pz, tb, hoisted, live);
                    tb.x += 4; tb.xy += 4; tb.xz += 4;
                }
            }
            if (MASS) {
#pragma unroll
                for (int i = 0; i < 10; ++i) {
                    const uint32_t sum = wave_sum_to_last_lane(v[i]);
                    if (lane == 63u && sum) atomicAdd(&scratch[8 + i], sum);
                }
                __syncthreads();
                if (threadIdx.x < 10) {
                    const uint32_t total = scratch[8 + threadIdx.x];
                    if (total) atomicAdd(&a.sums[(size_t)b * 10 + threadIdx.x], total);
                }
            }
            return;
        }
    }

    const uint32_t lin0 = (chunk * blockDim.x + threadIdx.x) * N;
    const Cells<N> c(lin0, cells, a.dy, a.dz);
    const T w = ev.dist(c.position(cx, a.step, c.x), c.position(cy, a.step, c.y), c.position(cz, a.step, c.z), lds);

    bool ambiguous[N];
    if (MASS) {
        bool inside[N];
        bool any_inside = false;
#pragma unroll
        for (int i = 0; i < N; ++i) {
            const float wi = sdf::get(w, i);
            const bool own = owned(a, phash, lin0 + (uint32_t)i);
            const bool mine = c.active[i] & own, in = wi <= -a.thr;
            inside[i] = mine & in;
            ambiguous[i] = mine & !in & (wi < a.thr);
            any_inside |= inside[i];
        }
        const uint64_t imask = __ballot(any_inside);
        __syncthreads();
        if (imask != 0ull) {
            uint32_t v[10] = {0, 0, 0, 0, 0, 0, 0, 0, 0, 0};
#pragma unroll
            for (int i = 0; i < N; ++i) {
                const uint32_t m = inside[i] ? 1u : 0u;
                const uint32_t x = c.x[i], y = c.y[i], z = c.z[i];
                const uint32_t xm = inside[i] ? x : 0u, ym = inside[i] ? y : 0u, zm = inside[i] ? z : 0u;
                v[0] += __umul24(xm, x); v[1] += __umul24(xm, y); v[2] += __umul24(xm, z); v[3] += xm;
                v[4] += __umul24(ym, y); v[5] += __umul24(ym, z); v[6] += ym;
                v[7] += __umul24(zm, z); v[8] += zm; v[9] += m;
            }
#pragma unroll
            for (int i = 0; i < 10; ++i) {
                const uint32_t sum = wave_sum_to_last_lane(v[i]);
                if ((threadIdx.x & 63u) == 63u && sum) atomicAdd(&scratch[8 + i], sum);
            }
        }
    } else {
#pragma unroll
        for (int i = 0; i < N; ++i) {
            const float wi = sdf::get(w, i);
            const bool own = owned(a, phash, lin0 + (uint32_t)i);
            ambiguous[i] = c.active[i] & own & (wi > -a.thr) & (wi < a.thr);
        }
    }

    const bool nothing_ambiguous = MASS && a.thr == 0.0f;
    uint32_t slot[N];
    if (nothing_ambiguous) {
#pragma unroll
        for (int i = 0; i < N; ++i) slot[i] = 0u;
        __syncthreads();
    } else {
        wg_compact_slots<N>(ambiguous, a.counter, scratch, slot);
    }
#pragma unroll
    for (int i = 0; i < N; ++i) {
        if (nothing_ambiguous || !(ambiguous[i] && slot[i] < a.capacity)) continue;
        const uint32_t x = c.x[i], y = c.y[i], z = c.z[i];
        if (!BATCH) {
            static_cast<uchar4*>(a.list)[slot[i]] = make_uchar4((unsigned char)x, (unsigned char)y, (unsigned char)z, 0);
        } else if (MASS) {
            static_cast<double4*>(a.list)[slot[i]] =
                make_double4((double)x * a.s + pcx, (double)y * a.s + pcy, (double)z * a.s + pcz, pcw);
        } else {
            static_cast<int4*>(a.list)[slot[i]] =
                make_int4(ipar.x + (int)x * a.int_step, ipar.y + (int)y * a.int_step, ipar.z + (int)z * a.int_step, ipar.w);
        }
    }
    if (MASS) {
        if (threadIdx.x < 10) {
            const uint32_t v = scratch[8 + threadIdx.x];
            if (v) atomicAdd(&a.sums[(size_t)b * 10 + threadIdx.x], v);
        }
    }
}

struct MaskArgs {
    uint32_t mode;
    uint32_t n_boxes;
    uint32_t chunks;
    uint32_t boxes_y, boxes_z;
    uint32_t nx, ny, nz;
    uint32_t xs0;
    uint32_t unit_base;
    const void* units;
    const uint32_t* n_units_dev;
    float cx, cy, cz, step;
    int32_t int_step, dimension;
    double res, ox, oy, oz, s;
    uint32_t* out;
};
template <class E> __global__ void __launch_bounds__(64) k_box_masks(const E ev, const MaskArgs a)
{
    if constexpr (E::kBricks) {
        constexpr int W = E::kPruneWords;
        if constexpr (W > 0) {
            const uint32_t box = blockIdx.x * blockDim.x + threadIdx.x;
            if (box >= a.n_boxes) return;
            const uint32_t unit = a.unit_base + box / a.chunks, chunk = box % a.chunks;
            sdf::Prune<W> pr;
#pragma unroll
            for (int i = 0; i < W; ++i) pr.w[i] = 0xffffffffu;
            if (!(a.n_units_dev && unit >= *a.n_units_dev)) {
                float cx = a.cx, cy = a.cy, cz = a.cz;
                if (a.mode == 1u) {
                    const int4 ic = static_cast<const int4*>(a.units)[unit];
                    cx = (float)((double)ic.x * a.res + a.ox); cy = (float)((double)ic.y * a.res + a.oy); cz = (float)((double)ic.z * a.res + a.oz);
                } else if (a.mode == 3u) {
                    const int4 ip = static_cast<const int4*>(a.units)[unit];
                    const double h = (double)a.int_step / 2;
                    cx = (float)(((double)ip.x + h) * a.res + a.ox); cy = (float)(((double)ip.y + h) * a.res + a.oy);
                    cz = (float)(((double)ip.z + (a.dimension == 3 ? h : 0.0)) * a.res + a.oz);
                } else if (a.mode == 4u) {
                    const double4 pc = static_cast<const double4*>(a.units)[unit];
                    const double h = a.s / 2;
                    cx = (float)(pc.x + h); cy = (float)(pc.y + h); cz = (float)(pc.z + h);
                }
                const uint32_t qz = chunk % a.boxes_z, qt = chunk / a.boxes_z, qy = qt % a.boxes_y, qx = qt / a.boxes_y;
                const uint32_t x0 = qx * 16u, y0 = qy * 16u, z0 = qz * 16u;
                const float ex = 0.5f * (float)(min(16u, a.nx - x0) - 1u), ey = 0.5f * (float)(min(16u, a.ny - y0) - 1u),
                            ez = 0.5f * (float)(min(16u, a.nz - z0) - 1u);
                const float hx = a.step * ex, hy = a.step * ey, hz = a.step * ez;
                ev.prune(sample(cx, a.step, a.xs0 + x0) + hx, sample(cy, a.step, y0) + hy, sample(cz, a.step, z0) + hz,
                         __builtin_fabsf(hx), __builtin_fabsf(hy), __builtin_fabsf(hz), pr);
            }
#pragma unroll
            for (int i = 0; i < W; ++i) a.out[(size_t)box * W + i] = pr.w[i];
        }
    }
}
// ... 352 lines not shown
```

### codecad_amd/csrc/specialise.hpp

```cpp
#pragma once

#include <algorithm>
#include <array>
#include <cmath>
#include <cstdio>
#include <cstdlib>
#include <cstring>
#include <functional>
#include <numeric>
#include <sstream>
#include <string>
#include <vector>

#include "tape.hpp"

namespace sdf {

struct SpecProgram {
    std::vector<Rec> full;
    std::vector<Rec> dist;
    int n_slots = 0, n_point_slots = 0, n_result_slots = 0;
};

namespace spec_detail {

inline std::string rec_literal(const Rec& r, bool clear_fold, uint32_t hdr)
{
    std::ostringstream o;
    char buf[32];
    std::snprintf(buf, sizeof buf, "0x%08xu", hdr);
    o << "Rec{" << buf << ", {";
    for (int i = 0; i < SDF_REC_DWORDS - 1; ++i) {
        uint32_t bits;
        std::memcpy(&bits, &r.p[i], 4);
        if (clear_fold && i == kFoldParam) bits = 0;
        std::snprintf(buf, sizeof buf, "0x%08xu", bits);
        o << (i ? ", " : "") << "__builtin_bit_cast(float, " << buf << ")";
    }
    o << "}}";
    return o.str();
}

inline std::string flit(float v)
{
    uint32_t bits;
    std::memcpy(&bits, &v, 4);
    char buf[48];
    std::snprintf(buf, sizeof buf, "__builtin_bit_cast(float, 0x%08xu)", bits);
    return buf;
}

inline uint32_t fold_of(const Rec& r)
{
    uint32_t f;
    std::memcpy(&f, &r.p[kFoldParam], 4);
    return f;
}

enum Kind { POINT, RESULT };
enum Role { LEAF, UNARY, WITH_POINT, SELECT, POINT_OP };

struct Node {
    Kind kind;
    Role role;
    int rec;
    uint32_t op;
    int a = -1;
    int b = -1;
};

inline bool is_leaf(uint32_t op)
{
    switch (op) {
    case OP_RECTANGLE: case OP_CIRCLE: case OP_REGULAR_POLYGON2D: case OP_POLYGON2D: case OP_SPHERE: case OP_HALF_SPACE:
    case OP_INVOLUTE_GEAR:
        return true;
    default: return false;
    }
}
inline bool is_unary_result(uint32_t op)
{
    switch (op) {
    case OP_TRANSFORMATION_FROM: case OPX_FROM_SCALE: case OPX_FROM_AXIS_X: case OPX_FROM_AXIS_Y: case OPX_FROM_AXIS_Z:
    case OPX_FROM_MATRIX: case OP_OFFSET: case OP_SHELL:
        return true;
    default: return false;
    }
}
inline bool is_select(uint32_t op) { return op == OP_UNION || op == OP_INTERSECTION || op == OP_SUBTRACTION; }
inline bool reads_input_distance(uint32_t op) { return op == OP_SHELL || op == OP_EXTRUSION; }

inline bool build_graph(const std::vector<Rec>& recs, std::vector<Node>& nodes, int& root, std::vector<int>* rec_node = nullptr)
{
    std::vector<int> slot(256, -1);
    int last = -1;
    root = -1;
    if (rec_node) rec_node->assign(recs.size(), -1);
    for (int i = 0; i < (int)recs.size(); ++i) {
        const Rec& r = recs[i];
        const uint32_t op = r.hdr & 0xffu, reg = (r.hdr >> 8) & 0xffffu, fold = fold_of(r);
        if (reg >= 256u) return false;
        if (fold & kFoldLoad) last = slot[fold & 0xffu];
        Node n;
        n.rec = i;
        n.op = op;
        bool made = true;
        if (op == OP_RETURN) { root = last; break; }
        else if (op == OP_STORE) { slot[reg] = last; made = false; }
        else if (op == OP_LOAD) { last = slot[reg]; made = false; }
        else if (op == OPX_POINT || op == OP_INITIAL_TRANSFORMATION_TO || op == OPX_INIT_ROW_X) { n.kind = POINT; n.role = POINT_OP; }
        else if (op == OPX_INIT_ROWS_YZ) {
            if (last < 0 || nodes[last].op != OPX_INIT_ROW_X) return false;
            n.kind = POINT; n.role = POINT_OP; n.a = last;
        }
        else if (produces_point(op)) {
            if (last < 0 || nodes[last].kind != POINT) return false;
            n.kind = POINT; n.role = POINT_OP; n.a = last;
        }
        else if (op == OP_MIRROR) {
            if (last < 0) return false;
            n.kind = nodes[last].kind; n.role = n.kind == POINT ? POINT_OP : UNARY; n.a = last;
        }
        else if (is_leaf(op)) {
            if (last < 0 || nodes[last].kind != POINT) return false;
            n.kind = RESULT; n.role = LEAF; n.a = last;
        }
        else if (is_unary_result(op)) {
            if (last < 0 || nodes[last].kind != RESULT) return false;
            n.kind = RESULT; n.role = UNARY; n.a = last;
        }
        else if (reads_point_operand(op)) {
            if (last < 0 || nodes[last].kind != RESULT || slot[reg] < 0 || nodes[slot[reg]].kind != POINT) return false;
            n.kind = RESULT; n.role = WITH_POINT; n.a = last; n.b = slot[reg];
        }
        else if (is_select(op)) {
            if (r.p[0] >= 0.0f) return false;
            if (last < 0 || nodes[last].kind != RESULT || slot[reg] < 0 || nodes[slot[reg]].kind != RESULT) return false;
            n.kind = RESULT; n.role = SELECT; n.a = last; n.b = slot[reg];
        }
        else return false;
        if (made) {
            nodes.push_back(n);
            last = (int)nodes.size() - 1;
        }
        if (rec_node) (*rec_node)[i] = last;
        if (fold & kFoldStore) slot[(fold >> 16) & 0xffu] = last;
    }
    return root >= 0 && nodes[root].kind == RESULT;
}

struct Step { int node; int negate; };

struct Path {
    int leaf;
    std::vector<std::pair<int, bool>> choices;
    std::vector<Step> up;
};

inline bool collect_paths(const std::vector<Node>& nodes, int at, Path cur, std::vector<Path>& out, size_t limit)
{
    const Node& n = nodes[at];
// ... 412 lines not shown
constexpr const char* kTableName[6] = {"X", "Y", "Z", "XY", "XZ", "YZ"};

inline std::string table_load(const Stmt& s, int column, bool single = false)
{
    return std::string("tb.template ") + kTableName[table_slot(s.deps)] + (single && (s.deps & DX) ? "1" : "") + "<" + std::to_string(column) + ">()";
}

struct PruneInfo {
    int n_bits = 0;
    std::vector<int> scope_of;
    std::vector<int> parent;
    std::vector<int> bit;
    struct Sel { int a_scope = 0, b_scope = 0; };
    std::vector<Sel> sel;
    std::vector<int> select_of_choice;
    std::vector<char> need_iv;
    int words() const { return (n_bits + 31) / 32; }
    bool guarded(int i) const { return i < (int)sel.size() && (sel[i].a_scope || sel[i].b_scope); }
    std::string alive(int scope) const { return "pr.template alive<" + std::to_string(bit[scope]) + ">()"; }
    std::vector<int> path(int scope) const
    {
        std::vector<int> p;
        for (int s = scope; s > 0; s = parent[s]) p.push_back(s);
        std::reverse(p.begin(), p.end());
        return p;
    }
};
constexpr int kMaxPruneBits = 512;

inline PruneInfo analyse_pruning(const Phase1& ph, int min_cost)
{
    const std::vector<Stmt>& st = ph.e.st;
    const int n = ph.n_phase1;
    PruneInfo pi;
    pi.scope_of.assign(st.size(), 0);
    pi.sel.assign(st.size(), PruneInfo::Sel());
    pi.select_of_choice.assign(st.size(), -1);
    pi.need_iv.assign(st.size(), 0);
    pi.parent.push_back(-1);
    pi.bit.push_back(-1);
    if (min_cost <= 0 || ph.root < 0) return pi;
    std::vector<char> lo(st.size(), 0), hi(st.size(), 0);
    for (int i = 0; i < n; ++i) {
        const Stmt& s = st[i];
        const int a = s.iv_a, b = s.iv_b;
        switch (s.iv) {
        case IV_LEAF: lo[i] = hi[i] = 1; break;
        case IV_SCALE: if (s.iv_c > 0.0f) { lo[i] = lo[a]; hi[i] = hi[a]; } else if (s.iv_c < 0.0f) { lo[i] = hi[a]; hi[i] = lo[a]; } else lo[i] = hi[i] = 1; break;
        case IV_OFFSET: lo[i] = lo[a]; hi[i] = hi[a]; break;
        case IV_SHELL: lo[i] = 1; hi[i] = lo[a] && hi[a]; break;
        case IV_PERP: lo[i] = lo[a] || lo[b]; hi[i] = hi[a] && hi[b]; break;
        case IV_MIN: lo[i] = lo[a] && lo[b]; hi[i] = hi[a] || hi[b]; break;
        case IV_MAX: lo[i] = lo[a] || lo[b]; hi[i] = hi[a] && hi[b]; break;
        case IV_MAXNEG: lo[i] = lo[a] || hi[b]; hi[i] = hi[a] && lo[b]; break;
        default: break;
        }
    }
    auto is_select = [&](int i) { return st[i].iv == IV_MIN || st[i].iv == IV_MAX || st[i].iv == IV_MAXNEG; };
    for (const auto& sc : ph.choice_of_select) pi.select_of_choice[sc.second] = sc.first;
    std::vector<int> choice_of(st.size(), -1);
    for (const auto& sc : ph.choice_of_select) choice_of[sc.first] = sc.second;
    std::vector<char> in_graph(st.size(), 0);
    std::vector<std::vector<int>> users(st.size());
    {
        std::vector<int> stack{ph.root};
        for (const auto& sc : ph.choice_of_select) stack.push_back(sc.second);
        while (!stack.empty()) {
            const int i = stack.back();
            stack.pop_back();
            if (in_graph[i]) continue;
            in_graph[i] = 1;
            for (int o : st[i].ops) { users[o].push_back(i); stack.push_back(o); }
        }
    }
    const std::vector<int> cost = statement_costs(ph);
    auto depth_of = [&](int s) { int d = 0; for (; s > 0; s = pi.parent[s]) ++d; return d; };
    auto lca = [&](int x, int y) {
        int dx = depth_of(x), dy = depth_of(y);
        while (dx > dy) { x = pi.parent[x]; --dx; }
        while (dy > dx) { y = pi.parent[y]; --dy; }
        while (x != y) { x = pi.parent[x]; y = pi.parent[y]; }
        return x;
    };
    std::vector<char> placed(st.size(), 0);
    auto place = [&](int i) {
        if (!in_graph[i] || placed[i]) return;
        placed[i] = 1;
        int scope = -1;
        if (i == ph.root) scope = 0;
        if (pi.select_of_choice[i] >= 0) scope = pi.scope_of[pi.select_of_choice[i]];
        for (int u : users[i]) {
            int at = pi.scope_of[u];
            const int sel = is_select(u) ? u : pi.select_of_choice[u];
            if (sel >= 0 && pi.guarded(sel) && st[u].ops.size() == 2) {
                const bool on_a = st[u].ops[0] == i, on_b = st[u].ops[1] == i;
                const int base = pi.scope_of[sel];
                if (on_a && !on_b) at = pi.sel[sel].a_scope ? pi.sel[sel].a_scope : base;
                else if (on_b && !on_a) at = pi.sel[sel].b_scope ? pi.sel[sel].b_scope : base;
                else at = base;
            }
            scope = scope < 0 ? at : lca(scope, at);
        }
        pi.scope_of[i] = scope < 0 ? 0 : scope;
        if (is_select(i)) {
            const int a = st[i].iv_a, b = st[i].iv_b;
            bool can_a = false, can_b = false;
            if (st[i].iv == IV_MIN) { can_b = hi[a] && lo[b]; can_a = hi[b] && lo[a]; }
            else if (st[i].iv == IV_MAX) { can_b = lo[a] && hi[b]; can_a = lo[b] && hi[a]; }
            else { can_b = lo[a] && lo[b]; can_a = hi[b] && hi[a]; }
            if (a == b) can_a = can_b = false;
            auto open = [&](int operand) {
                if (cost[operand] < min_cost || pi.n_bits >= kMaxPruneBits) return 0;
                pi.parent.push_back(pi.scope_of[i]);
                pi.bit.push_back(pi.n_bits++);
                return (int)pi.parent.size() - 1;
            };
            if (can_a) pi.sel[i].a_scope = open(a);
            if (can_b) pi.sel[i].b_scope = open(b);
        }
    };
    for (int i = (int)st.size() - 1; i >= 0; --i) {
        if (i < n && is_select(i) && choice_of[i] >= 0) {
            place(i);
            place(choice_of[i]);
        }
        place(i);
    }
    if (pi.n_bits == 0) return pi;
    std::vector<int> stack;
    for (int i = 0; i < n; ++i) if (in_graph[i] && pi.guarded(i)) { stack.push_back(st[i].iv_a); stack.push_back(st[i].iv_b); }
    int leaves = 0, conditional = 0;
    while (!stack.empty()) {
        const int i = stack.back();
        stack.pop_back();
        if (i < 0 || pi.need_iv[i]) continue;
        pi.need_iv[i] = 1;
        if (st[i].iv == IV_LEAF) { ++leaves; conditional += st[i].iv_conds.empty() ? 0 : 1; }
        if (st[i].iv != IV_LEAF && st[i].iv != IV_UNKNOWN) { stack.push_back(st[i].iv_a); stack.push_back(st[i].iv_b); }
    }
    static const int cond_share = [] { const char* e = std::getenv("HU_PRUNE_COND_SHARE"); return e && *e ? std::atoi(e) : 50; }();
    if (leaves > 0 && conditional * 100 > leaves * cond_share) {
        PruneInfo none;
        none.scope_of.assign(st.size(), 0);
        none.sel.assign(st.size(), PruneInfo::Sel());
        none.select_of_choice = pi.select_of_choice;
        none.need_iv.assign(st.size(), 0);
        none.parent.push_back(-1);
        none.bit.push_back(-1);
        return none;
    }
    return pi;
}

struct ScopedItem {
    int id;
    std::string decl;
    std::string assign;
};
inline std::string emit_scoped(const PruneInfo& pi, const std::vector<ScopedItem>& items, const std::string& pad = "    ")
{
    std::ostringstream o;
    for (const ScopedItem& it : items) o << pad << "decltype(" << it.decl << ") t" << it.id << ";\n";
    std::vector<int> open;
    auto indent = [&]() { return pad + std::string(4 * open.size(), ' '); };
    for (const ScopedItem& it : items) {
        const std::vector<int> want = pi.path(pi.scope_of[it.id]);
        size_t keep = 0;
        while (keep < open.size() && keep < want.size() && open[keep] == want[keep]) ++keep;
        while (open.size() > keep) { open.pop_back(); o << indent() << "}\n"; }
        while (open.size() < want.size()) {
            o << indent() << "if (" << pi.alive(want[open.size()]) << ") {\n";
            open.push_back(want[open.size()]);
        }
        o << indent() << it.assign << "\n";
    }
    while (!open.empty()) { open.pop_back(); o << indent() << "}\n"; }
    return o.str();
}
inline std::string guarded_select(const PruneInfo& pi, const Stmt& s, int id, const std::function<std::string(int)>& name)
{
    const PruneInfo::Sel& g = pi.sel[id];
    const std::string t = "t" + std::to_string(id), a = name(s.ops[0]), b = name(s.ops[1]);
    const std::string as = "as<decltype(" + t + ")>(";
    const std::string only_a = t + " = " + as + a + ");", only_b = t + " = " + as + (s.iv == IV_MAXNEG ? "-(" + b + ")" : b) + ");";
    const std::string both = t + " = " + render(s, name) + ";";
    if (g.a_scope && g.b_scope)
        return "if (" + pi.alive(g.a_scope) + " && " + pi.alive(g.b_scope) + ") " + both + " else if (" + pi.alive(g.a_scope) + ") " + only_a + " else " + only_b;
    if (g.b_scope) return "if (" + pi.alive(g.b_scope) + ") " + both + " else " + only_a;
    return "if (" + pi.alive(g.a_scope) + ") " + both + " else " + only_b;
}
inline std::string guarded_choice(const PruneInfo& pi, const Stmt& s, int id, int select, const std::function<std::string(int)>& name)
{
    const PruneInfo::Sel& g = pi.sel[select];
    const std::string t = "t" + std::to_string(id), both = t + " = " + render(s, name) + ";";
    const std::string constant = t + " = mask_const<decltype(" + t + ")>(";
    if (g.a_scope && g.b_scope)
        return "if (" + pi.alive(g.a_scope) + " && " + pi.alive(g.b_scope) + ") " + both + " else " + constant + pi.alive(g.a_scope) + ");";
    if (g.b_scope) return "if (" + pi.alive(g.b_scope) + ") " + both + " else " + constant + "true);";
    return "if (" + pi.alive(g.a_scope) + ") " + both + " else " + constant + "false);";
}

inline Variant render_variant(const Phase1& ph, const std::vector<char>& hoistable, const std::vector<int>& roots,
                              const std::vector<char>& tabc = std::vector<char>(), const std::vector<int>* tab_index = nullptr,
                              const std::vector<char>& held = std::vector<char>(), const PruneInfo* pi = nullptr)
{
    const bool scoped = pi && pi->n_bits > 0;
    const std::vector<Stmt>& st = ph.e.st;
    const int n = (int)st.size();
    auto invariant = [&](int i) { return hoistable[i] != 0; };
    auto tabled = [&](int i) { return i < (int)tabc.size() && tabc[i] != 0; };
    auto is_held = [&](int i) { return i < (int)held.size() && held[i] != 0; };
    auto column = [&](int i) { return table_load(st[i], tab_index ? (*tab_index)[i] : 0); };
    std::vector<char> in_main(n, 0), frontier(n, 0), in_pre(n, 0), tab_read(n, 0), pre_load(n, 0);
    std::vector<int> stack(roots.begin(), roots.end());
    while (!stack.empty()) {
        const int i = stack.back();
        stack.pop_back();
        if (i < 0) continue;
        if (is_held(i)) { frontier[i] = 1; continue; }
        if (tabled(i)) { tab_read[i] = 1; continue; }
        if (invariant(i)) { frontier[i] = 1; continue; }
        if (in_main[i]) continue;
        in_main[i] = 1;
        for (int o : st[i].ops) stack.push_back(o);
    }
    for (int i = 0; i < n; ++i) if (frontier[i]) stack.push_back(i);
    while (!stack.empty()) {
        const int i = stack.back();
        stack.pop_back();
        if (in_pre[i] || pre_load[i]) continue;
        if (tabled(i)) { pre_load[i] = 1; continue; }
        in_pre[i] = 1;
        for (int o : st[i].ops) stack.push_back(o);
    }
    Variant v;
    auto plain = [&](int i) { return st[i].ops.empty() ? st[i].text : "t" + std::to_string(i); };
    std::ostringstream pre, main;
    auto scoped_item = [&](int i, const std::string& rhs, const std::function<std::string(int)>& name) {
        const std::string t = "t" + std::to_string(i);
        if (pi->guarded(i) && rhs.compare(0, 3, "tb.") != 0) return ScopedItem{i, rhs, guarded_select(*pi, st[i], i, name)};
        const int sel = pi->select_of_choice[i];
        if (sel >= 0 && pi->guarded(sel)) return ScopedItem{i, rhs, guarded_choice(*pi, st[i], i, sel, name)};
        return ScopedItem{i, rhs, t + " = " + rhs + ";"};
    };
    std::vector<ScopedItem> pre_items;
    for (int i = 0; i < n; ++i) {
        if (st[i].ops.empty()) continue;
        if (scoped) {
            if (pre_load[i]) pre_items.push_back(ScopedItem{i, column(i), "t" + std::to_string(i) + " = " + column(i) + ";"});
            else if (in_pre[i]) pre_items.push_back(scoped_item(i, render(st[i], plain), plain));
            continue;
        }
        if (pre_load[i]) pre << "    const auto t" << i << " = " << column(i) << ";\n";
        else if (in_pre[i]) pre << "    const auto t" << i << " = " << render(st[i], plain) << ";\n";
    }
    if (scoped) pre << emit_scoped(*pi, pre_items);
    std::ostringstream members, values;
    for (int i = 0; i < n; ++i)
        if (frontier[i]) {
            members << " plain_t<decltype(t" << i << ")> t" << i << ";";
            values << (v.n_hoisted ? ", " : "") << "t" << i;
            ++v.n_hoisted;
        }
    if (v.n_hoisted) {
        pre << "    struct Hoisted {" << members.str() << " };\n    return Hoisted{" << values.str() << "};\n";
        v.pre = pre.str();
    }
    auto in_walk = [&](int i) { return st[i].ops.empty() ? st[i].text : (frontier[i] ? "h.t" : "t") + std::to_string(i); };
    std::vector<int> readers(n, 0), fused_inner(n, -1);
    static const bool fuse = [] { const char* e = std::getenv("HU_MINMAX3"); return !(e && e[0] == '0'); }();
    for (int i = 0; i < n; ++i) if (in_main[i]) for (int o : st[i].ops) ++readers[o];
    for (int r : roots) if (r >= 0) ++readers[r];
    std::vector<char> dead(n, 0);
    for (int i = 0; fuse && i < n; ++i) {
        if (!in_main[i] || st[i].ops.size() != 2) continue;
        if (st[i].text != "min_x($0, $1)" && st[i].text != "max_x($0, $1)") continue;
        const int j = st[i].ops[0];
        if (!in_main[j] || readers[j] != 1 || st[j].text != st[i].text || fused_inner[j] >= 0) continue;
        if (scoped && (pi->guarded(i) || pi->guarded(j) || pi->scope_of[i] != pi->scope_of[j])) continue;
        fused_inner[i] = j;
        dead[j] = 1;
    }
    std::vector<ScopedItem> main_items;
    for (int i = 0; i < n; ++i) {
        if (st[i].ops.empty()) continue;
        std::string rhs;
        if (tab_read[i]) rhs = column(i);
        else if (in_main[i] && !dead[i]) {
            if (fused_inner[i] >= 0) {
                const Stmt& in = st[fused_inner[i]];
                rhs = std::string(st[i].text[1] == 'i' ? "min3_x(" : "max3_x(") + in_walk(in.ops[0]) + ", " + in_walk(in.ops[1]) + ", " + in_walk(st[i].ops[1]) + ")";
            } else rhs = render(st[i], in_walk);
        } else continue;
        if (!scoped) main << "    const auto t" << i << " = " << rhs << ";\n";
        else if (tab_read[i] || fused_inner[i] >= 0) main_items.push_back(ScopedItem{i, rhs, "t" + std::to_string(i) + " = " + rhs + ";"});
        else main_items.push_back(scoped_item(i, rhs, in_walk));
    }
    if (scoped) main << emit_scoped(*pi, main_items);
    v.main = main.str();
    v.handed = frontier;
    v.tab_read = tab_read;
    v.tab_main = tab_read;
    for (int i = 0; i < n; ++i) if (pre_load[i]) v.tab_read[i] = 1;
    return v;
}

inline std::string render_table_builder(const Phase1& ph, uint8_t deps, const std::vector<int>& tab_index, const std::vector<char>& tabc,
                                        const std::vector<char>& used, std::vector<char>* reads = nullptr, const PruneInfo* pi = nullptr)
{
    const std::vector<Stmt>& st = ph.e.st;
    const int n = (int)st.size();
    const bool pair = (deps & (deps - 1)) != 0;
    std::vector<char> in(n, 0), loads(n, 0);
    std::vector<int> stack;
    for (int i = 0; i < n; ++i) if (used[i] && st[i].deps == deps && !st[i].ops.empty()) stack.push_back(i);
    while (!stack.empty()) {
        const int i = stack.back();
        stack.pop_back();
        if (in[i] || loads[i]) continue;
        if (pair && i < (int)tabc.size() && tabc[i] == 1) { loads[i] = 1; if (reads) (*reads)[i] = 1; continue; }
        in[i] = 1;
        for (int o : st[i].ops) stack.push_back(o);
    }
    auto plain = [&](int i) { return st[i].ops.empty() ? st[i].text : "t" + std::to_string(i); };
    std::ostringstream o;
    const bool scoped = pi && pi->n_bits > 0 && pair;
    std::vector<ScopedItem> items;
    for (int i = 0; i < n; ++i) {
        if (st[i].ops.empty()) continue;
        const std::string t = "t" + std::to_string(i);
        if (loads[i]) {
            const std::string rhs = table_load(st[i], tab_index[i], true);
            if (scoped) items.push_back(ScopedItem{i, rhs, t + " = " + rhs + ";"});
            else o << "    const auto " << t << " = " << rhs << ";\n";
        }
        if (!in[i]) continue;
        const std::string rhs = render(st[i], plain);
        const std::string store = used[i] && st[i].deps == deps ? "out[" + std::to_string(tab_index[i]) + " * S] = " + t + ";" : std::string();
        if (scoped) {
            const int sel = pi->select_of_choice[i];
            const std::string assign = pi->guarded(i) ? guarded_select(*pi, st[i], i, plain)
                                       : sel >= 0 && pi->guarded(sel) ? guarded_choice(*pi, st[i], i, sel, plain) : t + " = " + rhs + ";";
            items.push_back(ScopedItem{i, rhs, assign + (store.empty() ? "" : " " + store)});
        } else {
            o << "    const auto " << t << " = " << rhs << ";\n";
            if (!store.empty()) o << "    " << store << "\n";
        }
    }
    if (scoped) o << emit_scoped(*pi, items);
    return o.str();
}

inline std::string render_prune_function(const Phase1& ph, const PruneInfo& pi)
{
    const std::vector<Stmt>& st = ph.e.st;
    const int n = ph.n_phase1;
    std::ostringstream o;
    o << "template <class PR> __device__ __forceinline__ void tape_prune(float px, float py, float pz, float hx, float hy, float hz, "
         "const float* __restrict__ extra, PR& out)\n{\n    using namespace sdf;\n";
    if (pi.n_bits == 0) { o << "}\n"; return o.str(); }
    o << "    const uint32_t flags = 0u;\n";
    std::vector<char> in(st.size(), 0), cond_used(ph.conds.size(), 0);
    std::vector<int> stack;
    for (int i = 0; i < n; ++i)
        if (pi.need_iv[i] && st[i].iv == IV_LEAF) {
            stack.push_back(i);
            for (int c : st[i].iv_conds) { cond_used[c] = 1; stack.push_back(ph.conds[c].u); }
        }
    while (!stack.empty()) {
        const int i = stack.back();
        stack.pop_back();
        if (in[i]) continue;
        in[i] = 1;
        for (int op : st[i].ops) stack.push_back(op);
    }
    auto plain = [&](int i) { return st[i].ops.empty() ? st[i].text : "t" + std::to_string(i); };
    for (int i = 0; i < n; ++i)
        if (in[i] && !st[i].ops.empty()) o << "    const auto t" << i << " = " << render(st[i], plain) << ";\n";
    o << "    const float kUp = 1.0009765625f;\n"
      << "    const float rad[8] = {0.0f, hx * kUp, hy * kUp, iv_hypot(hx, hy) * kUp, hz * kUp, iv_hypot(hx, hz) * kUp, iv_hypot(hy, hz) * kUp, "
         "iv_hypot(iv_hypot(hx, hy), hz) * kUp};\n"
      << "    const float B = __builtin_fmaxf(__builtin_fmaxf(__builtin_fabsf(px) + hx, __builtin_fabsf(py) + hy), __builtin_fabsf(pz) + hz);\n";
    auto up = [](double v) { return flit(std::nextafter((float)(v * (1.0 + 1e-6)), HUGE_VALF)); };
    auto iv = [](int i) { return "i" + std::to_string(i); };
    for (size_t c = 0; c < ph.conds.size(); ++c) {
        if (!cond_used[c]) continue;
        const Phase1::Cond& k = ph.conds[c];
        const Stmt& u = st[k.u];
        o << "    const bool same" << c << " = iv_same_cell(" << plain(k.u) << ", " << up(k.lip) << " * rad[" << (int)u.deps << "] + (" << up(u.g)
          << " * B + " << up(u.o) << ") * kIvMargin, " << flit(k.inv) << ");\n";
    }
    for (int i = 0; i < n; ++i) {
        if (!pi.need_iv[i]) continue;
        const Stmt& s = st[i];
        o << "    const Iv " << iv(i) << " = ";
        switch (s.iv) {
        case IV_LEAF: {
            std::string ok;
            for (int c : s.iv_conds) ok += (ok.empty() ? "" : " && ") + ("same" + std::to_string(c));
            if (!ok.empty()) o << "!(" << ok << ") ? iv_unknown() : ";
            o << "iv_leaf(" << plain(i) << ", " << up(s.iv_l) << " * rad[" << (int)s.deps << "], (" << up(s.g) << " * B + " << up(s.o) << ") * kIvMargin)";
            break;
        }
        case IV_SCALE: o << (s.iv_c == 0.0f ? std::string("iv_zero()") : "iv_scale(" + iv(s.iv_a) + ", " + flit(s.iv_c) + ")"); break;
        case IV_OFFSET: o << "iv_offset(" << iv(s.iv_a) << ", " << flit(s.iv_c) << ")"; break;
        case IV_SHELL: o << "iv_shell(" << iv(s.iv_a) << ", " << flit(s.iv_c) << ")"; break;
        case IV_PERP: o << "iv_perp(" << iv(s.iv_a) << ", " << iv(s.iv_b) << ")"; break;
        case IV_MIN: o << "iv_min(" << iv(s.iv_a) << ", " << iv(s.iv_b) << ")"; break;
        case IV_MAX: o << "iv_max(" << iv(s.iv_a) << ", " << iv(s.iv_b) << ")"; break;
        case IV_MAXNEG: o << "iv_max(" << iv(s.iv_a) << ", iv_neg(" << iv(s.iv_b) << "))"; break;
        default: o << "iv_unknown()"; break;
        }
        o << ";\n";
    }
    const int words = pi.words();
    for (int w = 0; w < words; ++w) o << "    uint32_t w" << w << " = 0xffffffffu;\n";
    auto kill = [&](int scope, const std::string& cond) {
        if (!scope) return;
        const int b = pi.bit[scope];
        o << "    if (" << cond << ") w" << (b >> 5) << " &= ~" << (1u << (b & 31)) << "u;\n";
    };
    for (int i = 0; i < n; ++i) {
        if (!pi.guarded(i)) continue;
        const Stmt& s = st[i];
        const std::string a = iv(s.iv_a), b = iv(s.iv_b);
        if (s.iv == IV_MIN) { kill(pi.sel[i].b_scope, a + ".hi < " + b + ".lo"); kill(pi.sel[i].a_scope, b + ".hi < " + a + ".lo"); }
        else if (s.iv == IV_MAX) { kill(pi.sel[i].b_scope, a + ".lo > " + b + ".hi"); kill(pi.sel[i].a_scope, b + ".lo > " + a + ".hi"); }
        else { kill(pi.sel[i].b_scope, a + ".lo > -" + b + ".lo"); kill(pi.sel[i].a_scope, "-" + b + ".hi > " + a + ".hi"); }
    }
    for (int w = 0; w < words; ++w) o << "    out.w[" << w << "] = w" << w << ";\n";
    o << "}\n";
    return o.str();
}

}

struct SpecMeta {
    bool deferred = false;
    double coord_limit = 0.0;
    int tabs[6] = {0, 0, 0, 0, 0, 0};
    int prune_words = 0;
    int prune_bits = 0;
    bool prune_all = false;
    bool plain_in_place = false;
};
constexpr size_t kInPlaceDeferredPaths = 40;
constexpr int kMaxTableColumns = 48;
constexpr int kMaxPairColumns = 16;
constexpr int kMaxPairTotal = 24;

inline bool emit_deferred(std::ostringstream& o, const SpecProgram& p, size_t max_paths = 400, SpecMeta* meta = nullptr)
{
    using namespace spec_detail;
    if (p.dist.empty() || p.dist.size() != p.full.size()) return false;
    std::vector<Node> nodes;
    int root;
    if (!build_graph(p.full, nodes, root)) return false;
    std::vector<Path> paths;
    if (!collect_paths(nodes, root, Path(), paths, max_paths)) return false;
    if (paths.size() < 2) return false;

    std::vector<char> is_choice(p.full.size(), 0), keep_w(p.full.size(), 0);
    for (const Path& path : paths) {
        for (auto& c : path.choices) is_choice[c.first] = 1;
        for (const Step& s : path.up)
            if (s.node >= 0 && reads_input_distance(nodes[s.node].op)) keep_w[nodes[s.node].rec] = 1;
    }
    Phase1 ph;
    std::vector<std::array<int, 3>> pt(nodes.size(), {{-1, -1, -1}});
    if (!symbolic_phase1(p, nodes, root, is_choice, keep_w, ph, &pt)) return false;
    if (meta) meta->coord_limit = coordinate_limit(ph);
    ph.n_phase1 = (int)ph.e.st.size();
    static const int prune_min = [] {
        const char* off = std::getenv("HU_PRUNE");
        if (off && off[0] == '0') return 0;
        const char* e = std::getenv("HU_PRUNE_MIN");
        return e && *e ? std::atoi(e) : 6;
    }();
    const PruneInfo prune = analyse_pruning(ph, prune_min);
    static const int prune_eval_min = [] { const char* e = std::getenv("HU_PRUNE_EVAL_MIN"); return e && *e ? std::atoi(e) : 64; }();
    const bool prune_all = prune.n_bits >= prune_eval_min;
    if (meta) { meta->prune_bits = prune.n_bits; meta->prune_words = prune.words(); meta->prune_all = prune_all; }
    std::vector<int> dist_roots{ph.root}, eval_roots{ph.root};
    for (int v : ph.choice_of_rec) if (v >= 0) eval_roots.push_back(v);
    for (int v : ph.keep_w_of_rec) if (v >= 0) eval_roots.push_back(v);

    Emitter& e = ph.e;
    const int zero = e.add("0.0f", {});
    struct PathCode { std::string mask; int d[3]; };
    std::vector<PathCode> codes;
    {
        auto full_record = [&](const Rec& r, const int (&last)[4], const int (&operand)[4]) {
            const uint32_t op = r.hdr & 0xffu;
            return e.add("run_record_full<" + std::to_string(op) + ">(" + rec_literal(r, true, op) + ", extra, v4x($0, $1, $2, $3), v4x($4, $5, $6, $7), m)",
                         {last[0], last[1], last[2], last[3], operand[0], operand[1], operand[2], operand[3]});
        };
        auto mulc = [&](int v, float c) { return e.add("$0 * " + flit(c), {v}); };
        for (const Path& path : paths) {
            PathCode code;
            for (size_t k = 0; k < path.choices.size(); ++k)
                code.mask += std::string(k ? " & " : "") + (path.choices[k].second ? "" : "~") + "as_mask(@" + std::to_string(ph.choice_of_rec[path.choices[k].first]) + "@, T())";
            if (path.choices.empty()) code.mask = "mask_of<T>::all()";
            const Node& leaf = nodes[path.leaf];
            const Rec& lr = p.full[leaf.rec];
            const std::array<int, 3>& c = pt[leaf.a];
            int d[3] = {zero, zero, zero};
            if (leaf.op == OP_RECTANGLE) {
                const int v = e.add("rect_dir_x($0, $1, " + flit(lr.p[0]) + ", " + flit(lr.p[1]) + ", m, flags)", {c[0], c[1]});
                d[0] = e.add("$0.x", {v}); d[1] = e.add("$0.y", {v});
            } else if (leaf.op == OP_CIRCLE) {
                const int v = e.add("circle_dir_x($0, $1, m)", {c[0], c[1]});
                d[0] = e.add("$0.x", {v}); d[1] = e.add("$0.y", {v});
            } else if (leaf.op == OP_SPHERE) {
                const int v = e.add("sphere_dir_x($0, $1, $2, m)", {c[0], c[1], c[2]});
                d[0] = e.add("$0.x", {v}); d[1] = e.add("$0.y", {v}); d[2] = e.add("$0.z", {v});
            } else if (leaf.op == OP_HALF_SPACE) {
                d[1] = e.add("-1.0f", {});
            } else {
                const int last[4] = {c[0], c[1], zero, zero}, none4[4] = {zero, zero, zero, zero};
                const int v = full_record(lr, last, none4);
                d[0] = e.add("$0.x", {v}); d[1] = e.add("$0.y", {v}); d[2] = e.add("$0.z", {v});
            }
            for (const Step& stp : path.up) {
                if (stp.node < 0) {
                    for (int k = 0; k < 3; ++k) d[k] = e.neg(d[k]);
                    continue;
                }
                const Node& n = nodes[stp.node];
                const Rec& r = p.full[n.rec];
                const float* q = r.p;
                const int w_in = reads_input_distance(n.op) ? ph.keep_w_of_rec[n.rec] : zero;
                switch (n.op) {
                case OPX_FROM_SCALE:
                    for (int k = 0; k < 3; ++k) d[k] = mulc(d[k], q[0]);
                    break;
                case OPX_FROM_AXIS_X: case OPX_FROM_AXIS_Y: case OPX_FROM_AXIS_Z: {
                    const int ax = n.op == OPX_FROM_AXIS_X ? 0 : n.op == OPX_FROM_AXIS_Y ? 1 : 2, u = (ax + 1) % 3, v = (ax + 2) % 3;
                    const int along = d[ax], du = d[u], dv = d[v];
                    d[ax] = mulc(along, q[0]);
                    int ru = mulc(e.neg(dv), q[2]), rv = mulc(du, q[2]);
                    if (q[1] != 0.0f) {
                        ru = e.add("fma_x($0, " + flit(q[1]) + ", $1)", {du, ru});
                        rv = e.add("fma_x($0, " + flit(q[1]) + ", $1)", {dv, rv});
                    }
                    d[u] = ru;
                    d[v] = rv;
                    break;
                }
                case OPX_FROM_MATRIX: {
                    const int x = d[0], y = d[1], z = d[2];
                    for (int k = 0; k < 3; ++k)
                        d[k] = e.add("fma_x($0, " + flit(q[3 * k]) + ", fma_x($1, " + flit(q[3 * k + 1]) + ", $2 * " + flit(q[3 * k + 2]) + "))", {x, y, z});
                    break;
                }
                case OP_OFFSET: break;
                case OP_SHELL:
                    for (int k = 0; k < 3; ++k) d[k] = e.add("shell_dir_x($0, $1)", {d[k], w_in});
                    break;
                case OP_MIRROR: d[0] = e.neg(d[0]); break;
                case OP_EXTRUSION: {
                    const int v = e.add("extrusion_dir_x($0, $1, $2, $3, $4, " + flit(q[0]) + ", m, flags)", {d[0], d[1], d[2], w_in, pt[n.b][2]});
                    d[0] = e.add("$0.x", {v}); d[1] = e.add("$0.y", {v}); d[2] = e.add("$0.z", {v});
                    break;
                }
                case OP_SYMMETRICAL_FROM: d[0] = e.add("symm_dir_x($0, $1)", {d[0], pt[n.b][0]}); break;
                default: {
                    const int last[4] = {d[0], d[1], d[2], w_in};
                    const int operand[4] = {n.role == WITH_POINT ? pt[n.b][0] : zero, n.role == WITH_POINT ? pt[n.b][1] : zero,
                                            n.role == WITH_POINT ? pt[n.b][2] : zero, zero};
                    const int v = full_record(r, last, operand);
                    d[0] = e.add("$0.x", {v}); d[1] = e.add("$0.y", {v}); d[2] = e.add("$0.z", {v});
                    break;
                }
                }
            }
            code.d[0] = d[0]; code.d[1] = d[1]; code.d[2] = d[2];
            codes.push_back(code);
        }
    }
    std::vector<char> lives(e.st.size(), 0), kept_w(e.st.size(), 0);
    for (int v : ph.choice_of_rec) if (v >= 0) lives[v] = 1;
    for (int v : ph.keep_w_of_rec) if (v >= 0) kept_w[v] = 1;
    const std::vector<int> p1_cost = statement_costs(ph);
    static const int recompute_limit = [] { const char* e = std::getenv("HU_KEEP_RECOMPUTE"); return e && *e ? std::atoi(e) : 40; }();
    auto phase2_for = [&](const std::vector<char>& hoistable, const std::vector<char>& tabc, const std::vector<int>* tab_index,
                          std::vector<char>* tab_used) {
        const std::vector<Stmt>& st = e.st;
        auto outer = [&](int id) { return st[id].ops.empty() ? st[id].text : (id < (int)hoistable.size() && hoistable[id] ? "h.t" : "t") + std::to_string(id); };
        auto tabled = [&](int id) { return id < (int)tabc.size() && tabc[id] != 0; };
        auto handed = [&](int id) { return id < (int)hoistable.size() && hoistable[id] != 0; };
        std::function<bool(int)> again = [&](int id) -> bool {
            if (e.st[id].ops.empty() || tabled(id) || handed(id)) return true;
            if (e.st[id].mask || prune.guarded(id) || e.st[id].text.compare(0, 10, "run_record") == 0) return false;
            for (int op : e.st[id].ops) if (!again(op)) return false;
            return true;
        };
        std::vector<char> live_here = lives;
        for (int i = 0; i < (int)kept_w.size(); ++i)
            if (kept_w[i] && !handed(i) && !tabled(i) && !(p1_cost[i] <= recompute_limit && again(i))) live_here[i] = 1;
        std::ostringstream o2;
        o2 << "    // ---- phase 2\n"
           << "    const auto qx = opaque(px); const auto qy = opaque(py); const auto qz = opaque(pz);\n";
        if (!tabc.empty()) o2 << "    asm volatile(\"\" ::: \"memory\");\n";
        o2 << "    V4<T> dir = v4<T>(bc<T>(0.0f), bc<T>(0.0f), bc<T>(0.0f), bc<T>(0.0f));\n";
        auto block_body = [&](size_t k, const std::string& pad) {
            const PathCode& code = codes[k];
            std::ostringstream ob;
            std::vector<char> inside(st.size(), 0), loads(st.size(), 0);
            std::vector<int> stack{code.d[0], code.d[1], code.d[2]};
            while (!stack.empty()) {
                const int i = stack.back();
                stack.pop_back();
                if (inside[i] || loads[i] || st[i].ops.empty() || live_here[i] || (i < (int)hoistable.size() && hoistable[i])) continue;
                if (tabled(i)) { loads[i] = 1; if (tab_used) (*tab_used)[i] = 1; continue; }
                inside[i] = 1;
                for (int op : st[i].ops) stack.push_back(op);
            }
            auto name = [&](int id) -> std::string {
                if (st[id].ops.empty()) return st[id].text == "px" ? "qx" : st[id].text == "py" ? "qy" : st[id].text == "pz" ? "qz" : st[id].text;
                return inside[id] || loads[id] ? "u" + std::to_string(id) : outer(id);
            };
            for (int i = 0; i < (int)st.size(); ++i) {
                if (loads[i]) ob << pad << "const auto u" << i << " = " << table_load(st[i], tab_index ? (*tab_index)[i] : 0) << ";\n";
                else if (inside[i]) ob << pad << "const auto u" << i << " = " << render(st[i], name) << ";\n";
            }
            ob << pad << "dir.x = sel(m, as<T>(" << name(code.d[0]) << "), dir.x); dir.y = sel(m, as<T>(" << name(code.d[1])
               << "), dir.y); dir.z = sel(m, as<T>(" << name(code.d[2]) << "), dir.z);\n";
            return ob.str();
        };
        static const bool tree = [] { const char* e = std::getenv("HU_PHASE2_TREE"); return !(e && e[0] == '0'); }();
        if (tree) {
            size_t next = 0;
            std::function<void(int, const std::string&, int)> walk = [&](int at, const std::string& lanes, int depth) {
                const Node& n = nodes[at];
                const std::string pad(4 + 4 * (size_t)depth, ' ');
                if (n.role == LEAF) {
                    o2 << pad << "{   // the primitive of record " << n.rec << "\n" << pad << "    const M m = " << (lanes.empty() ? "mask_of<T>::all()" : lanes) << ";\n"
                       << block_body(next++, pad + "    ") << pad << "}\n";
                } else if (n.role == SELECT) {
                    const std::string c = "as_mask(" + outer(ph.choice_of_rec[n.rec]) + ", T())", id = std::to_string(n.rec);
                    const std::string ma = "m" + id + "a", mb = "m" + id + "b";
                    o2 << pad << "const M " << ma << " = " << (lanes.empty() ? "" : lanes + " & ") << c << ", " << mb << " = " << (lanes.empty() ? "" : lanes + " & ") << "~" << c << ";\n"
                       << pad << "if (wave_any(" << ma << ")) {\n";
                    walk(n.a, ma, depth + 1);
                    o2 << pad << "}\n" << pad << "if (wave_any(" << mb << ")) {\n";
                    walk(n.b, mb, depth + 1);
                    o2 << pad << "}\n";
                } else walk(n.a, lanes, depth);
            };
            walk(root, "", 0);
        } else
        for (size_t k = 0; k < paths.size(); ++k) {
            const PathCode& code = codes[k];
            std::string mask;
            for (size_t i = 0; i < code.mask.size(); ++i) {
                if (code.mask[i] != '@') { mask += code.mask[i]; continue; }
                const size_t end = code.mask.find('@', i + 1);
                mask += outer(std::atoi(code.mask.substr(i + 1, end - i - 1).c_str()));
                i = end;
            }
            o2 << "    {   // the primitive of record " << nodes[paths[k].leaf].rec << " along one path to the root\n        const M m = " << mask
               << ";\n        if (wave_any(m)) {\n" << block_body(k, "            ") << "        }\n    }\n";
        }
        return o2.str();
    };

    const char* head = "    using namespace sdf;\n    using T = wider_t<wider_t<PX, PY>, PZ>;\n    using M = typename mask_of<T>::type;\n";
    struct Form { const char* suffix; uint8_t walk; };
    const Form forms[2] = {{"", 0}, {"_x", DX}};
    auto knob = [](const char* name, int fallback) { const char* e = std::getenv(name); return e && *e ? std::atoi(e) : fallback; };
    const int tab_min = knob("HU_TAB_MIN", 2);
    const bool plain_in_place = paths.size() > kInPlaceDeferredPaths;
    if (meta) meta->plain_in_place = plain_in_place;
    for (const Form& f : forms) {
        if (f.walk == 0 && plain_in_place) continue;
        const std::vector<char> hoistable = hoistable_set(ph, f.walk, knob("HU_HOIST_MIN_X", 8));
        std::vector<char> tabc;
        std::vector<int> tab_index(ph.e.st.size(), -1);
        int n_tab[6] = {0, 0, 0, 0, 0, 0};
        std::vector<char> held, used;
        if (f.walk != 0 && tab_min > 0) {
            const std::vector<int> tab_cost = statement_costs(ph);
            tabc = table_candidates(ph, tab_min, knob("HU_TAB_PAIR_MIN", 3));
            for (;;) {
                const Variant probe = render_variant(ph, hoistable, dist_roots, tabc);
                held.assign(ph.e.st.size(), 0);
                int budget = knob("HU_TAB_HOLD_X", prune_all ? 0 : 12);
                for (int i = 0; i < (int)probe.tab_main.size(); ++i) {
                    if (!probe.tab_main[i] || !tabc[i] || (ph.e.st[i].deps & f.walk)) continue;
                    const int regs = (ph.e.st[i].deps & DX) ? 2 : 1;
                    if (budget >= regs) { held[i] = 1; budget -= regs; }
                }
                const Variant all = render_variant(ph, hoistable, eval_roots, tabc, nullptr, held);
                used = all.tab_read;
                for (int i = 0; i < (int)held.size(); ++i) if (held[i]) used[i] = 1;
                (void)phase2_for(all.handed, tabc, nullptr, &used);
                for (uint8_t pair : {(uint8_t)(DX | DY), (uint8_t)(DX | DZ), (uint8_t)(DY | DZ)})
                    (void)render_table_builder(ph, pair, tab_index, tabc, std::vector<char>(used), &used);
                std::fill(tab_index.begin(), tab_index.end(), -1);
                std::fill(n_tab, n_tab + 6, 0);
                bool over = false;
                std::vector<int> order;
                for (int i = 0; i < (int)used.size(); ++i) if (used[i]) order.push_back(i);
                int wanted[6] = {0, 0, 0, 0, 0, 0};
                for (int i : order) ++wanted[table_slot(ph.e.st[i].deps)];
                const bool crowded = wanted[0] > kMaxTableColumns || wanted[1] > kMaxTableColumns || wanted[2] > kMaxTableColumns || wanted[3] > kMaxPairColumns ||
                                     wanted[4] > kMaxPairColumns || wanted[5] > kMaxPairColumns || wanted[3] + wanted[4] + wanted[5] > kMaxPairTotal;
                if (crowded) std::stable_sort(order.begin(), order.end(), [&](int x, int y) { return tab_cost[x] > tab_cost[y]; });
                for (int i : order) {
                    const int slot = table_slot(ph.e.st[i].deps);
                    const bool fits = slot < 3 ? n_tab[slot] < kMaxTableColumns
                                               : n_tab[slot] < kMaxPairColumns && n_tab[3] + n_tab[4] + n_tab[5] < kMaxPairTotal;
                    if (fits) tab_index[i] = n_tab[slot]++;
                    else { over = true; used[i] = 0; }
                }
                if (!over) break;
                for (int i = 0; i < (int)tabc.size(); ++i) if (tab_index[i] < 0) tabc[i] = 0;
            }
            if (std::accumulate(n_tab, n_tab + 6, 0) == 0) { tabc.clear(); held.clear(); }
        }
        if (meta && f.walk != 0) for (int a = 0; a < 6; ++a) meta->tabs[a] = n_tab[a];
        const PruneInfo* pi_dist = f.walk != 0 ? &prune : nullptr;
        const PruneInfo* pi = f.walk != 0 && prune_all ? &prune : nullptr;
        const Variant vd = render_variant(ph, hoistable, dist_roots, tabc, &tab_index, held, pi_dist),
                      ve = render_variant(ph, hoistable, eval_roots, tabc, &tab_index, held, pi);
        const Variant& pre_of = ve;
        const bool hoists = f.walk != 0 && pre_of.n_hoisted > 0;
        if (f.walk != 0) {
            o << "// hoisted out of walks along x: " << pre_of.n_hoisted << " values; table columns: "
              << n_tab[0] << " / " << n_tab[1] << " / " << n_tab[2] << " (x / y / z), " << n_tab[3] << " / " << n_tab[4] << " / " << n_tab[5] << " (xy / xz / yz)\n"
              << "template <class PX, class PY, class PZ, class TB, class PR> __device__ __forceinline__ auto tape_pre" << f.suffix
              << "(PX px, PY py, PZ pz, const float* __restrict__ extra, uint32_t flags, const TB& tb, const PR& pr)\n{\n    using namespace sdf;\n";
            if (hoists) o << pre_of.pre;
            else o << "    struct Hoisted {};\n    return Hoisted{};\n";
            o << "}\n";
            const char* slot_name[6] = {"x", "y", "z", "xy", "xz", "yz"};
            const uint8_t slot_deps[6] = {DX, DY, DZ, DX | DY, DX | DZ, DY | DZ};
            for (int a = 0; a < 3; ++a)
                o << "template <int S, class L> __device__ __forceinline__ void tape_tab" << f.suffix << "_" << slot_name[a] << "(float p"
                  << slot_name[a] << ", const float* __restrict__ extra, uint32_t flags, L out)\n{\n    using namespace sdf;\n"
                  << (n_tab[a] ? render_table_builder(ph, slot_deps[a], tab_index, tabc, used) : std::string()) << "}\n";
            for (int a = 3; a < 6; ++a)
                o << "template <int S, class TB, class PR, class L> __device__ __forceinline__ void tape_tab" << f.suffix << "_" << slot_name[a]
                  << "(float px, float py, float pz, const float* __restrict__ extra, uint32_t flags, const TB& tb, const PR& pr, L out)\n{\n    using namespace sdf;\n"
                  << (n_tab[a] ? render_table_builder(ph, slot_deps[a], tab_index, tabc, used, nullptr, pi) : std::string()) << "}\n";
            o << render_prune_function(ph, prune);
        }
        const std::string h_param = f.walk != 0 ? ", const H& h, const TB& tb, const PR& pr" : "";
        const std::string h_tmpl = f.walk != 0 ? ", class H, class TB, class PR" : "";
        const std::string root_name = ph.e.st[ph.root].ops.empty() ? ph.e.st[ph.root].text : ((ve.handed[ph.root] ? "h.t" : "t") + std::to_string(ph.root));
        o << "template <class PX, class PY, class PZ" << h_tmpl << "> __device__ __forceinline__ auto tape_dist" << f.suffix
          << "(PX px, PY py, PZ pz, const float* __restrict__ extra, uint32_t flags" << h_param << ")\n{\n" << head
          << vd.main << "    return as<T>(" << root_name << ");\n}\n";
        o << "template <class PX, class PY, class PZ" << h_tmpl << "> __device__ __forceinline__ auto tape_eval" << f.suffix
          << "(PX px, PY py, PZ pz, const float* __restrict__ extra, uint32_t flags" << h_param << ")\n{\n" << head
          << ve.main << phase2_for(ve.handed, tabc, &tab_index, nullptr)
          << "    return v4<T>(dir.x, dir.y, dir.z, as<T>(" << root_name << "));\n}\n";
    }
    o << "// deferred directions: " << paths.size() << " (primitive, path) pairs; " << ph.e.st.size() << " statements in phase 1; box pruning: "
      << prune.n_bits << " scopes\n";
    return true;
}

inline std::string specialised_source(const SpecProgram& p, bool allow_deferred, SpecMeta* meta = nullptr)
{
    std::ostringstream o, d;
    SpecMeta m;
    static const size_t max_paths = [] { const char* e = std::getenv("HU_MAX_PATHS"); return e && *e ? (size_t)std::atoi(e) : (size_t)400; }();
    const bool ok = allow_deferred && emit_deferred(d, p, max_paths, &m);
    if (!ok) m = SpecMeta();
    m.deferred = ok;
    if (meta) *meta = m;
    o << "#include \"kernels.hpp\"\nnamespace sdfk {\nusing sdf::Rec;\n";
    if (ok) o << d.str();
    if (!ok || m.plain_in_place) emit_plain(o, p);
    o << "struct JitEval {\n    static constexpr bool kBricks = " << (ok ? "true" : "false") << ";\n"
      << "    const float* extra;\n"
      << "    uint32_t flags;   // sdf::kFlagInRange: the launch's coordinates cannot leave the fast range of sqrt_cr\n";
    if (ok) {
        if (m.plain_in_place)
            o << "    template <class T> __device__ __forceinline__ sdf::V4<T> operator()(T px, T py, T pz, void*) const\n"
              << "    { return tape_eval<T>(px, py, pz, extra); }\n"
              << "    template <class T> __device__ __forceinline__ T dist(T px, T py, T pz, void*) const\n"
              << "    { return tape_dist<T>(px, py, pz, extra); }\n";
        else
            o << "    template <class T> __device__ __forceinline__ sdf::V4<T> operator()(T px, T py, T pz, void*) const\n"
              << "    { return tape_eval(px, py, pz, extra, flags); }\n"
              << "    template <class T> __device__ __forceinline__ T dist(T px, T py, T pz, void*) const\n"
              << "    { return tape_dist(px, py, pz, extra, flags); }\n";
        o
          << "    static constexpr int kTabXX = " << m.tabs[0] << ", kTabXY = " << m.tabs[1] << ", kTabXZ = " << m.tabs[2]
          << ", kPairXY = " << m.tabs[3] << ", kPairXZ = " << m.tabs[4] << ", kPairYZ = " << m.tabs[5] << ";\n"
          << "    static constexpr int kPruneWords = " << m.prune_words << ";\n"
          << "    static constexpr bool kPruneAll = " << (m.prune_all ? "true" : "false") << ";\n"
          << "    template <class PR> __device__ __forceinline__ void prune(float cx, float cy, float cz, float hx, float hy, float hz, PR& out) const\n"
          << "    { tape_prune(cx, cy, cz, hx, hy, hz, extra, out); }\n";
        for (const char* axis : {"x", "y", "z"})
            o << "    template <int S, class L> __device__ __forceinline__ void tab_x_" << axis << "(float p, L out) const\n"
              << "    { tape_tab_x_" << axis << "<S>(p, extra, flags, out); }\n";
        o << "    template <int S, class TB, class PR, class L> __device__ __forceinline__ void tab_x_xy(float a, float b, const TB& tb, const PR& pr, L out) const\n"
          << "    { tape_tab_x_xy<S>(a, b, 0.0f, extra, flags, tb, pr, out); }\n"
          << "    template <int S, class TB, class PR, class L> __device__ __forceinline__ void tab_x_xz(float a, float b, const TB& tb, const PR& pr, L out) const\n"
          << "    { tape_tab_x_xz<S>(a, 0.0f, b, extra, flags, tb, pr, out); }\n"
          << "    template <int S, class TB, class PR, class L> __device__ __forceinline__ void tab_x_yz(float a, float b, const TB& tb, const PR& pr, L out) const\n"
          << "    { tape_tab_x_yz<S>(0.0f, a, b, extra, flags, tb, pr, out); }\n"
          << "    template <class PY, class PZ, class TB, class PR> __device__ __forceinline__ auto hoist_x(PY py, PZ pz, const TB& tb, const PR& pr) const\n"
          << "    { return tape_pre_x(0.0f, py, pz, extra, flags, tb, pr); }\n"
          << "    template <class PX, class PY, class PZ, class H, class TB, class PR> __device__ __forceinline__ auto eval_hoisted_x(PX px, PY py, PZ pz, const H& h, const TB& tb, const PR& pr) const\n"
          << "    { return tape_eval_x(px, py, pz, extra, flags, h, tb, pr); }\n"
          << "    template <class PX, class PY, class PZ, class H, class TB, class PR> __device__ __forceinline__ auto dist_hoisted_x(PX px, PY py, PZ pz, const H& h, const TB& tb, const PR& pr) const\n"
          << "    { return tape_dist_x(px, py, pz, extra, flags, h, tb, pr); }\n";
    } else {
        o << "    template <class T> __device__ __forceinline__ sdf::V4<T> operator()(T px, T py, T pz, void*) const\n"
          << "    { return tape_eval<T>(px, py, pz, extra); }\n"
          << "    template <class T> __device__ __forceinline__ T dist(T px, T py, T pz, void*) const\n"
          << "    { return tape_dist<T>(px, py, pz, extra); }\n";
    }
    o << "};\n}  // namespace sdfk\n";
    return o.str();
}

}
```

Before: 495,500.

## Fold min/max chains by axis dependence and build separate distance-only tables

Adds a compiler pass that flattens chains of min/max (through positive scales) and regroups the terms by which axes they depend on. Terms depending on only some axes can then be hoisted or tabulated per box. It also builds a separate table layout and hoisted-value set for the distance-only path (layout 1 and subdivision), sized by its own table counts instead of reusing the eval layout. This aims to cut per-voxel work for deep CSG trees like the Menger sponge, at the cost of more generated code, more compile complexity and different LDS use.

```diff
diff --git a/codecad_amd/csrc/hip_util.hip b/codecad_amd/csrc/hip_util.hip
--- a/codecad_amd/csrc/hip_util.hip
+++ b/codecad_amd/csrc/hip_util.hip
@@ -211,6 +211,7 @@
     bool deferred = false;
     double coord_limit = 0.0;
     int tabs[6] = {0, 0, 0, 0, 0, 0};
+    int dtabs[6] = {0, 0, 0, 0, 0, 0};
     int prune_words = 0;
     int prune_bits = 0;
     bool prune_all = false;
@@ -252,10 +253,10 @@
 {
     return sdf::specialised_source(t->program, defer_directions(), meta);
 }
-uint32_t box_table_bytes(const SpecKernels* k)
-{
-    return (uint32_t)((k->tabs[0] + k->tabs[1] + k->tabs[2]) * sdf::BoxTabs::kAxis + (k->tabs[3] + k->tabs[4]) * sdf::BoxTabs::kPairX +
-                      k->tabs[5] * sdf::BoxTabs::kPairYZ) * 4u;
+uint32_t box_table_bytes(const SpecKernels* k, bool dist)
+{
+    const int* n = dist ? k->dtabs : k->tabs;
+    return (uint32_t)((n[0] + n[1] + n[2]) * sdf::BoxTabs::kAxis + (n[3] + n[4]) * sdf::BoxTabs::kPairX + n[5] * sdf::BoxTabs::kPairYZ) * 4u;
 }
 
 void keep_programs(hu_tape_s* t, const sdf::DecodedTape& d)
@@ -583,7 +584,7 @@
             } else {
                 void* args[] = {&ev, &cx, &cy, &cz, &step, &sx, &sy, &sz, &xs, &n_cells, &boxes, &o, &masks};
                 HU_HIP(hipModuleLaunchKernel(ragged ? t->spec->dense_ragged[layout] : t->spec->dense[layout], grid, 1, 1, block, 1, 1,
-                                             boxes ? box_table_bytes(t->spec) : idle_lds, (hipStream_t)stream, args, nullptr));
+                                             boxes ? box_table_bytes(t->spec, layout != 0) : idle_lds, (hipStream_t)stream, args, nullptr));
             }
             done += nx;
         }
@@ -680,7 +681,7 @@
             } else {
                 void* args[] = {&ev, &b, &n_dev, &first, &chunks, &bricks, &res, &ox, &oy, &oz, &step, &sx, &sy, &sz, &out_dev, &masks};
                 HU_HIP(hipModuleLaunchKernel(ragged ? t->spec->blocks_ragged[layout] : t->spec->blocks[layout], chunks * count, 1, 1, kSpecBlock, 1, 1,
-                                             bricks ? box_table_bytes(t->spec) : 0u, (hipStream_t)stream, args, nullptr));
+                                             bricks ? box_table_bytes(t->spec, layout != 0) : 0u, (hipStream_t)stream, args, nullptr));
             }
         }
         return HU_OK;
@@ -757,7 +758,7 @@
         if (t->spec->deferred && cells > 256u && bxn * byn * bzn * n_parents >= enough && boxes_worthwhile(dims[0], dims[1], dims[2])) {
             a.boxes = ((uint32_t)byn << 16) | (uint32_t)bzn;
             a.chunks = (uint32_t)(bxn * byn * bzn);
-            a.scratch_offset = box_table_bytes(t->spec);
+            a.scratch_offset = box_table_bytes(t->spec, true);
         }
         const double extent = (double)a.step * (double)std::max(dims[0], std::max(dims[1], dims[2]));
         const float c3[3] = {a.cx, a.cy, a.cz};
@@ -1692,6 +1693,7 @@
     k->prune_bits = meta.prune_bits;
     k->prune_all = meta.prune_all;
     std::memcpy(k->tabs, meta.tabs, sizeof k->tabs);
+    std::memcpy(k->dtabs, meta.dtabs, sizeof k->dtabs);
     return HU_OK;
 }
 
diff --git a/codecad_amd/csrc/kernels.hpp b/codecad_amd/csrc/kernels.hpp
--- a/codecad_amd/csrc/kernels.hpp
+++ b/codecad_amd/csrc/kernels.hpp
@@ -171,12 +171,13 @@
 struct BoxTables {
     sdf::lds_float *x, *y, *z, *xy, *xz, *yz;
 };
-template <class E, class PR>
+template <bool DIST, class E, class PR>
 __device__ __forceinline__ BoxTables box_tables(const E& ev, float4* lds, float cx, float cy, float cz, float step, uint32_t xs0,
                                                 uint32_t x0, uint32_t y0, uint32_t z0, uint32_t nx, uint32_t ny, uint32_t nz, const PR& pr)
 {
     const uint32_t lane = threadIdx.x & 63u, wave = threadIdx.x >> 6;
-    constexpr int NX = E::kTabXX, NY = E::kTabXY, NZ = E::kTabXZ, NXY = E::kPairXY, NXZ = E::kPairXZ, NYZ = E::kPairYZ;
+    constexpr int NX = DIST ? E::kDTabXX : E::kTabXX, NY = DIST ? E::kDTabXY : E::kTabXY, NZ = DIST ? E::kDTabXZ : E::kTabXZ;
+    constexpr int NXY = DIST ? E::kDPairXY : E::kPairXY, NXZ = DIST ? E::kDPairXZ : E::kPairXZ, NYZ = DIST ? E::kDPairYZ : E::kPairYZ;
     using Tabs = sdf::BoxTabs;
     sdf::lds_float* const tx = (sdf::lds_float*)lds;
     sdf::lds_float* const ty = tx + NX * Tabs::kAxis;
@@ -187,30 +188,45 @@
     if constexpr (NX + NY + NZ > 0) {
         if (wave == 0u) {
             if constexpr (NX > 0)
-                if (lane < nx) ev.template tab_x_x<Tabs::kAxis>(sample(cx, step, xs0 + x0 + lane), tx + lane);
+                if (lane < nx) {
+                    if constexpr (DIST) ev.template tab_d_x<Tabs::kAxis>(sample(cx, step, xs0 + x0 + lane), tx + lane);
+                    else ev.template tab_x_x<Tabs::kAxis>(sample(cx, step, xs0 + x0 + lane), tx + lane);
+                }
         } else if (wave == 1u) {
             if constexpr (NY > 0)
-                if (lane < ny) ev.template tab_x_y<Tabs::kAxis>(sample(cy, step, y0 + lane), ty + lane);
+                if (lane < ny) {
+                    if constexpr (DIST) ev.template tab_d_y<Tabs::kAxis>(sample(cy, step, y0 + lane), ty + lane);
+                    else ev.template tab_x_y<Tabs::kAxis>(sample(cy, step, y0 + lane), ty + lane);
+                }
         } else if (wave == 2u) {
             if constexpr (NZ > 0)
-                if (lane < nz) ev.template tab_x_z<Tabs::kAxis>(sample(cz, step, z0 + lane), tz + lane);
+                if (lane < nz) {
+                    if constexpr (DIST) ev.template tab_d_z<Tabs::kAxis>(sample(cz, step, z0 + lane), tz + lane);
+                    else ev.template tab_x_z<Tabs::kAxis>(sample(cz, step, z0 + lane), tz + lane);
+                }
         }
         __syncthreads();
     }
     if constexpr (NXY + NXZ + NYZ > 0) {
         const uint32_t r = threadIdx.x >> 4, c = threadIdx.x & 15u;
         if constexpr (NXY > 0)
-            if (r < ny && c < nx)
-                ev.template tab_x_xy<Tabs::kPairX>(sample(cx, step, xs0 + x0 + c), sample(cy, step, y0 + r), Tabs{tx + c, ty + r, tz, txy, txz, tyz}, pr,
-                                                   txy + (r * Tabs::kRowX + c));
+            if (r < ny && c < nx) {
+                const Tabs at{tx + c, ty + r, tz, txy, txz, tyz};
+                if constexpr (DIST) ev.template tab_d_xy<Tabs::kPairX>(sample(cx, step, xs0 + x0 + c), sample(cy, step, y0 + r), at, pr, txy + (r * Tabs::kRowX + c));
+                else ev.template tab_x_xy<Tabs::kPairX>(sample(cx, step, xs0 + x0 + c), sample(cy, step, y0 + r), at, pr, txy + (r * Tabs::kRowX + c));
+            }
         if constexpr (NXZ > 0)
-            if (r < nz && c < nx)
-                ev.template tab_x_xz<Tabs::kPairX>(sample(cx, step, xs0 + x0 + c), sample(cz, step, z0 + r), Tabs{tx + c, ty, tz + r, txy, txz, tyz}, pr,
-                                                   txz + (r * Tabs::kRowX + c));
+            if (r < nz && c < nx) {
+                const Tabs at{tx + c, ty, tz + r, txy, txz, tyz};
+                if constexpr (DIST) ev.template tab_d_xz<Tabs::kPairX>(sample(cx, step, xs0 + x0 + c), sample(cz, step, z0 + r), at, pr, txz + (r * Tabs::kRowX + c));
+                else ev.template tab_x_xz<Tabs::kPairX>(sample(cx, step, xs0 + x0 + c), sample(cz, step, z0 + r), at, pr, txz + (r * Tabs::kRowX + c));
+            }
         if constexpr (NYZ > 0)
-            if (r < ny && c < nz)
-                ev.template tab_x_yz<Tabs::kPairYZ>(sample(cy, step, y0 + r), sample(cz, step, z0 + c), Tabs{tx, ty + r, tz + c, txy, txz, tyz}, pr,
-                                                    tyz + (r * Tabs::kRowYZ + c));
+            if (r < ny && c < nz) {
+                const Tabs at{tx, ty + r, tz + c, txy, txz, tyz};
+                if constexpr (DIST) ev.template tab_d_yz<Tabs::kPairYZ>(sample(cy, step, y0 + r), sample(cz, step, z0 + c), at, pr, tyz + (r * Tabs::kRowYZ + c));
+                else ev.template tab_x_yz<Tabs::kPairYZ>(sample(cy, step, y0 + r), sample(cz, step, z0 + c), at, pr, tyz + (r * Tabs::kRowYZ + c));
+            }
         __syncthreads();
     }
     return BoxTables{tx, ty, tz, txy, txz, tyz};
@@ -227,7 +243,7 @@
     const uint32_t sx = o.sxa, sy = o.sy, sz = o.sz;
     const uint32_t nx = min(16u, o.nx - x0), ny = min(16u, sy - y0), nz = min(16u, sz - z0);
     const sdf::Prune<E::kPruneWords> pr = sdf::load_prune<E::kPruneWords>(masks, box);
-    const BoxTables t = box_tables(ev, lds, cx, cy, cz, step, xs0, x0, y0, z0, nx, ny, nz, pr);
+    const BoxTables t = box_tables<LAYOUT != 0>(ev, lds, cx, cy, cz, step, xs0, x0, y0, z0, nx, ny, nz, pr);
     sdf::lds_float* const tx = t.x; sdf::lds_float* const ty = t.y; sdf::lds_float* const tz = t.z;
     sdf::lds_float* const txy = t.xy; sdf::lds_float* const txz = t.xz; sdf::lds_float* const tyz = t.yz;
     const uint32_t nbz = RAGGED ? (nz + 7u) >> 3 : nz >> 3;
@@ -247,7 +263,10 @@
         const float py = sample(cy, step, y0 + yl);
         const bool row_inside = !RAGGED || (z_inside && yl < ny);
         Tabs tb = col;
-        const auto hoisted = ev.hoist_x(py, walk_coordinate<E>(pz), tb, pr);
+        const auto hoisted = [&] {
+            if constexpr (LAYOUT == 0) return ev.hoist_x(py, walk_coordinate<E>(pz), tb, pr);
+            else return ev.hoist_d(py, walk_coordinate<E>(pz), tb, pr);
+        }();
         size_t p = at;
 #pragma unroll 1
         for (uint32_t j = 0; j < bricks_x; ++j) {
@@ -258,7 +277,7 @@
             const T px = pack(xs);
             const float pyb = walk_coordinate<E>(py), pzb = walk_coordinate<E>(pz);
             const auto prb = pr.fresh();
-            if (LAYOUT == 0) {
+            if constexpr (LAYOUT == 0) {
                 const sdf::V4<T> r = ev.eval_hoisted_x(px, pyb, pzb, hoisted, tb, prb);
 #pragma unroll
                 for (int i = 0; i < N; ++i)
@@ -512,7 +531,7 @@
             const uint32_t x0 = qx * 16u, y0 = qy * 16u, z0 = qz * 16u;
             const uint32_t nx = min(16u, a.sx - x0), ny = min(16u, a.sy - y0), nz = min(16u, a.sz - z0);
             const sdf::Prune<E::kPruneWords> pr = sdf::load_prune<E::kPruneWords>(a.masks, blockIdx.x);
-            const BoxTables t = box_tables(ev, lds, cx, cy, cz, a.step, 0u, x0, y0, z0, nx, ny, nz, pr);
+            const BoxTables t = box_tables<true>(ev, lds, cx, cy, cz, a.step, 0u, x0, y0, z0, nx, ny, nz, pr);
             if (MASS) __syncthreads();
             const bool nothing_ambiguous = MASS && a.thr == 0.0f;
             const uint64_t below = (1ull << lane) - 1ull;
@@ -574,7 +593,7 @@
                 const bool live = (zl < nz) & (yl < ny);
                 const float py = sample(cy, a.step, y);
                 Tabs tb{t.x + xl, t.y + yl, t.z + zl, t.xy + (yl * Tabs::kRowX + xl), t.xz + (zl * Tabs::kRowX + xl), t.yz + (yl * Tabs::kRowYZ + zl)};
-                const auto hoisted = ev.hoist_x(py, walk_coordinate<E>(pz), tb, pr);
+                const auto hoisted = ev.hoist_d(py, walk_coordinate<E>(pz), tb, pr);
 #pragma unroll 1
                 for (uint32_t j = 0; j < ((nx + 3u) >> 2); ++j) {
                     asm volatile("" ::: "memory");
diff --git a/codecad_amd/csrc/specialise.hpp b/codecad_amd/csrc/specialise.hpp
--- a/codecad_amd/csrc/specialise.hpp
+++ b/codecad_amd/csrc/specialise.hpp
@@ -7,6 +7,7 @@
 #include <cstdlib>
 #include <cstring>
 #include <functional>
+#include <map>
 #include <numeric>
 #include <sstream>
 #include <string>
@@ -725,6 +726,82 @@
     return pi;
 }
 
+inline int fold_chains(Phase1& ph, const PruneInfo& pi, int root)
+{
+    Emitter& e = ph.e;
+    auto in_scope0 = [&](int v) { return !pi.guarded(v) && (v >= (int)pi.scope_of.size() || pi.scope_of[v] == 0); };
+    auto kind_of = [&](int v) -> uint8_t {
+        const Stmt& s = e.st[v];
+        if (s.iv == IV_MIN && s.text == "min_x($0, $1)" && in_scope0(v)) return IV_MIN;
+        if (s.iv == IV_MAX && s.text == "max_x($0, $1)" && in_scope0(v)) return IV_MAX;
+        return 0;
+    };
+    auto positive_scale = [&](int v) {
+        const Stmt& s = e.st[v];
+        return s.iv == IV_SCALE && s.ops.size() == 1 && s.iv_a == s.ops[0] && s.iv_c > 0.0f && std::isfinite(s.iv_c) && in_scope0(v) &&
+               s.text == "$0 * " + flit(s.iv_c);
+    };
+    std::function<uint8_t(int)> chain_kind = [&](int v) -> uint8_t {
+        if (const uint8_t k = kind_of(v)) return k;
+        return positive_scale(v) ? chain_kind(e.st[v].ops[0]) : 0;
+    };
+    struct Term { int leaf; std::vector<float> scales; };
+    std::function<void(int, uint8_t, std::vector<float>, std::vector<Term>&)> expand = [&](int v, uint8_t k, std::vector<float> scales, std::vector<Term>& out) {
+        if (kind_of(v) == k) {
+            expand(e.st[v].ops[0], k, scales, out);
+            expand(e.st[v].ops[1], k, scales, out);
+        } else if (positive_scale(v) && chain_kind(e.st[v].ops[0]) == k) {
+            scales.insert(scales.begin(), e.st[v].iv_c);
+            expand(e.st[v].ops[0], k, scales, out);
+        } else out.push_back(Term{v, scales});
+    };
+    std::map<int, int> memo;
+    std::function<int(int)> rewrite = [&](int v) -> int {
+        auto it = memo.find(v);
+        if (it != memo.end()) return it->second;
+        int r = v;
+        const uint8_t k = chain_kind(v);
+        std::vector<Term> terms;
+        if (k) expand(v, k, {}, terms);
+        std::vector<uint8_t> group_deps;
+        std::vector<std::vector<size_t>> groups;
+        for (size_t i = 0; i < terms.size(); ++i) {
+            const uint8_t d = e.st[terms[i].leaf].deps;
+            const size_t g = std::find(group_deps.begin(), group_deps.end(), d) - group_deps.begin();
+            if (g == group_deps.size()) { group_deps.push_back(d); groups.emplace_back(); }
+            groups[g].push_back(i);
+        }
+        bool worth = false;
+        for (size_t g = 0; g < groups.size(); ++g)
+            worth |= groups[g].size() > 1 && group_deps[g] != 0 && group_deps[g] != (DX | DY | DZ);
+        if (k && worth) {
+            const char* op = k == IV_MIN ? "min_x($0, $1)" : "max_x($0, $1)";
+            int acc = -1;
+            for (const std::vector<size_t>& g : groups) {
+                int part = -1;
+                for (size_t i : g) {
+                    int t = rewrite(terms[i].leaf);
+                    for (float c : terms[i].scales) t = e.add("$0 * " + flit(c), {t});
+                    part = part < 0 ? t : e.add(op, {part, t});
+                }
+                acc = acc < 0 ? part : e.add(op, {acc, part});
+            }
+            r = acc;
+        } else if (!e.st[v].ops.empty() && !e.st[v].mask && in_scope0(v)) {
+            std::vector<int> ops;
+            for (int o : e.st[v].ops) ops.push_back(rewrite(o));
+            if (ops != e.st[v].ops) {
+                const Stmt old = e.st[v];
+                r = e.add(old.text, ops);
+                e.st[r].g = old.g; e.st[r].o = old.o; e.st[r].bounded = old.bounded; e.st[r].abs_h = old.abs_h;
+            }
+        }
+        memo[v] = r;
+        return r;
+    };
+    return rewrite(root);
+}
+
 struct ScopedItem {
     int id;
     std::string decl;
@@ -1012,6 +1089,8 @@
     bool deferred = false;
     double coord_limit = 0.0;
     int tabs[6] = {0, 0, 0, 0, 0, 0};
+    int dtabs[6] = {0, 0, 0, 0, 0, 0};
+    bool folded = false;
     int prune_words = 0;
     int prune_bits = 0;
     bool prune_all = false;
@@ -1050,10 +1129,18 @@
         const char* e = std::getenv("HU_PRUNE_MIN");
         return e && *e ? std::atoi(e) : 6;
     }();
-    const PruneInfo prune = analyse_pruning(ph, prune_min);
+    PruneInfo prune = analyse_pruning(ph, prune_min);
     static const int prune_eval_min = [] { const char* e = std::getenv("HU_PRUNE_EVAL_MIN"); return e && *e ? std::atoi(e) : 64; }();
     const bool prune_all = prune.n_bits >= prune_eval_min;
     if (meta) { meta->prune_bits = prune.n_bits; meta->prune_words = prune.words(); meta->prune_all = prune_all; }
+    static const bool fold = [] { const char* e = std::getenv("HU_FOLD"); return !(e && e[0] == '0'); }();
+    const int folded_root = fold ? fold_chains(ph, prune, ph.root) : ph.root;
+    ph.n_phase1 = (int)ph.e.st.size();
+    prune.scope_of.resize(ph.e.st.size(), 0);
+    prune.sel.resize(ph.e.st.size());
+    prune.select_of_choice.resize(ph.e.st.size(), -1);
+    prune.need_iv.resize(ph.e.st.size(), 0);
+    if (meta) meta->folded = folded_root != ph.root;
     std::vector<int> dist_roots{ph.root}, eval_roots{ph.root};
     for (int v : ph.choice_of_rec) if (v >= 0) eval_roots.push_back(v);
     for (int v : ph.keep_w_of_rec) if (v >= 0) eval_roots.push_back(v);
@@ -1245,90 +1332,108 @@
     const int tab_min = knob("HU_TAB_MIN", 2);
     const bool plain_in_place = paths.size() > kInPlaceDeferredPaths;
     if (meta) meta->plain_in_place = plain_in_place;
+    struct Layout {
+        std::vector<char> tabc, held, used;
+        std::vector<int> tab_index;
+        int n_tab[6] = {0, 0, 0, 0, 0, 0};
+    };
+    auto allocate = [&](const std::vector<char>& hoistable, uint8_t walk, const std::vector<int>& probe_roots, const std::vector<int>& roots,
+                        bool directions, Layout& L) {
+        L.tab_index.assign(ph.e.st.size(), -1);
+        const std::vector<int> tab_cost = statement_costs(ph);
+        L.tabc = table_candidates(ph, tab_min, knob("HU_TAB_PAIR_MIN", 3));
+        std::vector<char>& tabc = L.tabc;
+        std::vector<int>& tab_index = L.tab_index;
+        std::vector<char>& held = L.held;
+        std::vector<char>& used = L.used;
+        int* n_tab = L.n_tab;
+        for (;;) {
+            const Variant probe = render_variant(ph, hoistable, probe_roots, tabc);
+            held.assign(ph.e.st.size(), 0);
+            int budget = knob("HU_TAB_HOLD_X", prune_all ? 0 : 12);
+            for (int i = 0; i < (int)probe.tab_main.size(); ++i) {
+                if (!probe.tab_main[i] || !tabc[i] || (ph.e.st[i].deps & walk)) continue;
+                const int regs = (ph.e.st[i].deps & DX) ? 2 : 1;
+                if (budget >= regs) { held[i] = 1; budget -= regs; }
+            }
+            const Variant all = render_variant(ph, hoistable, roots, tabc, nullptr, held);
+            used = all.tab_read;
+            for (int i = 0; i < (int)held.size(); ++i) if (held[i]) used[i] = 1;
+            if (directions) (void)phase2_for(all.handed, tabc, nullptr, &used);
+            for (uint8_t pair : {(uint8_t)(DX | DY), (uint8_t)(DX | DZ), (uint8_t)(DY | DZ)})
+                (void)render_table_builder(ph, pair, tab_index, tabc, std::vector<char>(used), &used);
+            std::fill(tab_index.begin(), tab_index.end(), -1);
+            std::fill(n_tab, n_tab + 6, 0);
+            bool over = false;
+            std::vector<int> order;
+            for (int i = 0; i < (int)used.size(); ++i) if (used[i]) order.push_back(i);
+            int wanted[6] = {0, 0, 0, 0, 0, 0};
+            for (int i : order) ++wanted[table_slot(ph.e.st[i].deps)];
+            const bool crowded = wanted[0] > kMaxTableColumns || wanted[1] > kMaxTableColumns || wanted[2] > kMaxTableColumns || wanted[3] > kMaxPairColumns ||
+                                 wanted[4] > kMaxPairColumns || wanted[5] > kMaxPairColumns || wanted[3] + wanted[4] + wanted[5] > kMaxPairTotal;
+            if (crowded) std::stable_sort(order.begin(), order.end(), [&](int x, int y) { return tab_cost[x] > tab_cost[y]; });
+            for (int i : order) {
+                const int slot = table_slot(ph.e.st[i].deps);
+                const bool fits = slot < 3 ? n_tab[slot] < kMaxTableColumns
+                                           : n_tab[slot] < kMaxPairColumns && n_tab[3] + n_tab[4] + n_tab[5] < kMaxPairTotal;
+                if (fits) tab_index[i] = n_tab[slot]++;
+                else { over = true; used[i] = 0; }
+            }
+            if (!over) break;
+            for (int i = 0; i < (int)tabc.size(); ++i) if (tab_index[i] < 0) tabc[i] = 0;
+        }
+        if (std::accumulate(n_tab, n_tab + 6, 0) == 0) { tabc.clear(); held.clear(); }
+    };
+    const char* slot_name[6] = {"x", "y", "z", "xy", "xz", "yz"};
+    const uint8_t slot_deps[6] = {DX, DY, DZ, DX | DY, DX | DZ, DY | DZ};
+    auto emit_tables = [&](const std::string& tag, const Layout& L, const Variant& pre_of, const PruneInfo* pi) {
+        o << "// " << tag << ": hoisted out of walks along x: " << pre_of.n_hoisted << " values; table columns: "
+          << L.n_tab[0] << " / " << L.n_tab[1] << " / " << L.n_tab[2] << " (x / y / z), " << L.n_tab[3] << " / " << L.n_tab[4] << " / " << L.n_tab[5] << " (xy / xz / yz)\n"
+          << "template <class PX, class PY, class PZ, class TB, class PR> __device__ __forceinline__ auto tape_pre" << tag
+          << "(PX px, PY py, PZ pz, const float* __restrict__ extra, uint32_t flags, const TB& tb, const PR& pr)\n{\n    using namespace sdf;\n";
+        if (pre_of.n_hoisted > 0) o << pre_of.pre;
+        else o << "    struct Hoisted {};\n    return Hoisted{};\n";
+        o << "}\n";
+        for (int a = 0; a < 3; ++a)
+            o << "template <int S, class L> __device__ __forceinline__ void tape_tab" << tag << "_" << slot_name[a] << "(float p"
+              << slot_name[a] << ", const float* __restrict__ extra, uint32_t flags, L out)\n{\n    using namespace sdf;\n"
+              << (L.n_tab[a] ? render_table_builder(ph, slot_deps[a], L.tab_index, L.tabc, L.used) : std::string()) << "}\n";
+        for (int a = 3; a < 6; ++a)
+            o << "template <int S, class TB, class PR, class L> __device__ __forceinline__ void tape_tab" << tag << "_" << slot_name[a]
+              << "(float px, float py, float pz, const float* __restrict__ extra, uint32_t flags, const TB& tb, const PR& pr, L out)\n{\n    using namespace sdf;\n"
+              << (L.n_tab[a] ? render_table_builder(ph, slot_deps[a], L.tab_index, L.tabc, L.used, nullptr, pi) : std::string()) << "}\n";
+    };
     for (const Form& f : forms) {
         if (f.walk == 0 && plain_in_place) continue;
         const std::vector<char> hoistable = hoistable_set(ph, f.walk, knob("HU_HOIST_MIN_X", 8));
-        std::vector<char> tabc;
-        std::vector<int> tab_index(ph.e.st.size(), -1);
-        int n_tab[6] = {0, 0, 0, 0, 0, 0};
-        std::vector<char> held, used;
+        const std::vector<int> walk_dist_roots{f.walk != 0 ? folded_root : ph.root};
+        Layout le, ld;
         if (f.walk != 0 && tab_min > 0) {
-            const std::vector<int> tab_cost = statement_costs(ph);
-            tabc = table_candidates(ph, tab_min, knob("HU_TAB_PAIR_MIN", 3));
-            for (;;) {
-                const Variant probe = render_variant(ph, hoistable, dist_roots, tabc);
-                held.assign(ph.e.st.size(), 0);
-                int budget = knob("HU_TAB_HOLD_X", prune_all ? 0 : 12);
-                for (int i = 0; i < (int)probe.tab_main.size(); ++i) {
-                    if (!probe.tab_main[i] || !tabc[i] || (ph.e.st[i].deps & f.walk)) continue;
-                    const int regs = (ph.e.st[i].deps & DX) ? 2 : 1;
-                    if (budget >= regs) { held[i] = 1; budget -= regs; }
-                }
-                const Variant all = render_variant(ph, hoistable, eval_roots, tabc, nullptr, held);
-                used = all.tab_read;
-                for (int i = 0; i < (int)held.size(); ++i) if (held[i]) used[i] = 1;
-                (void)phase2_for(all.handed, tabc, nullptr, &used);
-                for (uint8_t pair : {(uint8_t)(DX | DY), (uint8_t)(DX | DZ), (uint8_t)(DY | DZ)})
-                    (void)render_table_builder(ph, pair, tab_index, tabc, std::vector<char>(used), &used);
-                std::fill(tab_index.begin(), tab_index.end(), -1);
-                std::fill(n_tab, n_tab + 6, 0);
-                bool over = false;
-                std::vector<int> order;
-                for (int i = 0; i < (int)used.size(); ++i) if (used[i]) order.push_back(i);
-                int wanted[6] = {0, 0, 0, 0, 0, 0};
-                for (int i : order) ++wanted[table_slot(ph.e.st[i].deps)];
-                const bool crowded = wanted[0] > kMaxTableColumns || wanted[1] > kMaxTableColumns || wanted[2] > kMaxTableColumns || wanted[3] > kMaxPairColumns ||
-                                     wanted[4] > kMaxPairColumns || wanted[5] > kMaxPairColumns || wanted[3] + wanted[4] + wanted[5] > kMaxPairTotal;
-                if (crowded) std::stable_sort(order.begin(), order.end(), [&](int x, int y) { return tab_cost[x] > tab_cost[y]; });
-                for (int i : order) {
-                    const int slot = table_slot(ph.e.st[i].deps);
-                    const bool fits = slot < 3 ? n_tab[slot] < kMaxTableColumns
-                                               : n_tab[slot] < kMaxPairColumns && n_tab[3] + n_tab[4] + n_tab[5] < kMaxPairTotal;
-                    if (fits) tab_index[i] = n_tab[slot]++;
-                    else { over = true; used[i] = 0; }
-                }
-                if (!over) break;
-                for (int i = 0; i < (int)tabc.size(); ++i) if (tab_index[i] < 0) tabc[i] = 0;
-            }
-            if (std::accumulate(n_tab, n_tab + 6, 0) == 0) { tabc.clear(); held.clear(); }
-        }
-        if (meta && f.walk != 0) for (int a = 0; a < 6; ++a) meta->tabs[a] = n_tab[a];
+            allocate(hoistable, f.walk, dist_roots, eval_roots, true, le);
+            allocate(hoistable, f.walk, walk_dist_roots, walk_dist_roots, false, ld);
+        }
+        if (meta && f.walk != 0) for (int a = 0; a < 6; ++a) { meta->tabs[a] = le.n_tab[a]; meta->dtabs[a] = ld.n_tab[a]; }
         const PruneInfo* pi_dist = f.walk != 0 ? &prune : nullptr;
         const PruneInfo* pi = f.walk != 0 && prune_all ? &prune : nullptr;
-        const Variant vd = render_variant(ph, hoistable, dist_roots, tabc, &tab_index, held, pi_dist),
-                      ve = render_variant(ph, hoistable, eval_roots, tabc, &tab_index, held, pi);
-        const Variant& pre_of = ve;
-        const bool hoists = f.walk != 0 && pre_of.n_hoisted > 0;
+        const Variant vd = render_variant(ph, hoistable, walk_dist_roots, ld.tabc, &ld.tab_index, ld.held, pi_dist),
+                      ve = render_variant(ph, hoistable, eval_roots, le.tabc, &le.tab_index, le.held, pi);
         if (f.walk != 0) {
-            o << "// hoisted out of walks along x: " << pre_of.n_hoisted << " values; table columns: "
-              << n_tab[0] << " / " << n_tab[1] << " / " << n_tab[2] << " (x / y / z), " << n_tab[3] << " / " << n_tab[4] << " / " << n_tab[5] << " (xy / xz / yz)\n"
-              << "template <class PX, class PY, class PZ, class TB, class PR> __device__ __forceinline__ auto tape_pre" << f.suffix
-              << "(PX px, PY py, PZ pz, const float* __restrict__ extra, uint32_t flags, const TB& tb, const PR& pr)\n{\n    using namespace sdf;\n";
-            if (hoists) o << pre_of.pre;
-            else o << "    struct Hoisted {};\n    return Hoisted{};\n";
-            o << "}\n";
-            const char* slot_name[6] = {"x", "y", "z", "xy", "xz", "yz"};
-            const uint8_t slot_deps[6] = {DX, DY, DZ, DX | DY, DX | DZ, DY | DZ};
-            for (int a = 0; a < 3; ++a)
-                o << "template <int S, class L> __device__ __forceinline__ void tape_tab" << f.suffix << "_" << slot_name[a] << "(float p"
-                  << slot_name[a] << ", const float* __restrict__ extra, uint32_t flags, L out)\n{\n    using namespace sdf;\n"
-                  << (n_tab[a] ? render_table_builder(ph, slot_deps[a], tab_index, tabc, used) : std::string()) << "}\n";
-            for (int a = 3; a < 6; ++a)
-                o << "template <int S, class TB, class PR, class L> __device__ __forceinline__ void tape_tab" << f.suffix << "_" << slot_name[a]
-                  << "(float px, float py, float pz, const float* __restrict__ extra, uint32_t flags, const TB& tb, const PR& pr, L out)\n{\n    using namespace sdf;\n"
-                  << (n_tab[a] ? render_table_builder(ph, slot_deps[a], tab_index, tabc, used, nullptr, pi) : std::string()) << "}\n";
+            emit_tables(f.suffix, le, ve, pi);
+            emit_tables("_d", ld, vd, pi);
             o << render_prune_function(ph, prune);
         }
         const std::string h_param = f.walk != 0 ? ", const H& h, const TB& tb, const PR& pr" : "";
         const std::string h_tmpl = f.walk != 0 ? ", class H, class TB, class PR" : "";
-        const std::string root_name = ph.e.st[ph.root].ops.empty() ? ph.e.st[ph.root].text : ((ve.handed[ph.root] ? "h.t" : "t") + std::to_string(ph.root));
+        auto root_of = [&](const Variant& v, int root) {
+            return ph.e.st[root].ops.empty() ? ph.e.st[root].text : ((v.handed[root] ? "h.t" : "t") + std::to_string(root));
+        };
         o << "template <class PX, class PY, class PZ" << h_tmpl << "> __device__ __forceinline__ auto tape_dist" << f.suffix
           << "(PX px, PY py, PZ pz, const float* __restrict__ extra, uint32_t flags" << h_param << ")\n{\n" << head
-          << vd.main << "    return as<T>(" << root_name << ");\n}\n";
+          << vd.main << "    return as<T>(" << root_of(vd, walk_dist_roots[0]) << ");\n}\n";
         o << "template <class PX, class PY, class PZ" << h_tmpl << "> __device__ __forceinline__ auto tape_eval" << f.suffix
           << "(PX px, PY py, PZ pz, const float* __restrict__ extra, uint32_t flags" << h_param << ")\n{\n" << head
-          << ve.main << phase2_for(ve.handed, tabc, &tab_index, nullptr)
-          << "    return v4<T>(dir.x, dir.y, dir.z, as<T>(" << root_name << "));\n}\n";
+          << ve.main << phase2_for(ve.handed, le.tabc, &le.tab_index, nullptr)
+          << "    return v4<T>(dir.x, dir.y, dir.z, as<T>(" << root_of(ve, ph.root) << "));\n}\n";
     }
     o << "// deferred directions: " << paths.size() << " (primitive, path) pairs; " << ph.e.st.size() << " statements in phase 1; box pruning: "
       << prune.n_bits << " scopes\n";
@@ -1364,21 +1469,26 @@
         o
           << "    static constexpr int kTabXX = " << m.tabs[0] << ", kTabXY = " << m.tabs[1] << ", kTabXZ = " << m.tabs[2]
           << ", kPairXY = " << m.tabs[3] << ", kPairXZ = " << m.tabs[4] << ", kPairYZ = " << m.tabs[5] << ";\n"
+          << "    static constexpr int kDTabXX = " << m.dtabs[0] << ", kDTabXY = " << m.dtabs[1] << ", kDTabXZ = " << m.dtabs[2]
+          << ", kDPairXY = " << m.dtabs[3] << ", kDPairXZ = " << m.dtabs[4] << ", kDPairYZ = " << m.dtabs[5] << ";\n"
           << "    static constexpr int kPruneWords = " << m.prune_words << ";\n"
           << "    static constexpr bool kPruneAll = " << (m.prune_all ? "true" : "false") << ";\n"
           << "    template <class PR> __device__ __forceinline__ void prune(float cx, float cy, float cz, float hx, float hy, float hz, PR& out) const\n"
           << "    { tape_prune(cx, cy, cz, hx, hy, hz, extra, out); }\n";
-        for (const char* axis : {"x", "y", "z"})
-            o << "    template <int S, class L> __device__ __forceinline__ void tab_x_" << axis << "(float p, L out) const\n"
-              << "    { tape_tab_x_" << axis << "<S>(p, extra, flags, out); }\n";
-        o << "    template <int S, class TB, class PR, class L> __device__ __forceinline__ void tab_x_xy(float a, float b, const TB& tb, const PR& pr, L out) const\n"
-          << "    { tape_tab_x_xy<S>(a, b, 0.0f, extra, flags, tb, pr, out); }\n"
-          << "    template <int S, class TB, class PR, class L> __device__ __forceinline__ void tab_x_xz(float a, float b, const TB& tb, const PR& pr, L out) const\n"
-          << "    { tape_tab_x_xz<S>(a, 0.0f, b, extra, flags, tb, pr, out); }\n"
-          << "    template <int S, class TB, class PR, class L> __device__ __forceinline__ void tab_x_yz(float a, float b, const TB& tb, const PR& pr, L out) const\n"
-          << "    { tape_tab_x_yz<S>(0.0f, a, b, extra, flags, tb, pr, out); }\n"
-          << "    template <class PY, class PZ, class TB, class PR> __device__ __forceinline__ auto hoist_x(PY py, PZ pz, const TB& tb, const PR& pr) const\n"
-          << "    { return tape_pre_x(0.0f, py, pz, extra, flags, tb, pr); }\n"
+        for (const char* kind : {"x", "d"}) {
+            for (const char* axis : {"x", "y", "z"})
+                o << "    template <int S, class L> __device__ __forceinline__ void tab_" << kind << "_" << axis << "(float p, L out) const\n"
+                  << "    { tape_tab_" << kind << "_" << axis << "<S>(p, extra, flags, out); }\n";
+            o << "    template <int S, class TB, class PR, class L> __device__ __forceinline__ void tab_" << kind << "_xy(float a, float b, const TB& tb, const PR& pr, L out) const\n"
+              << "    { tape_tab_" << kind << "_xy<S>(a, b, 0.0f, extra, flags, tb, pr, out); }\n"
+              << "    template <int S, class TB, class PR, class L> __device__ __forceinline__ void tab_" << kind << "_xz(float a, float b, const TB& tb, const PR& pr, L out) const\n"
+              << "    { tape_tab_" << kind << "_xz<S>(a, 0.0f, b, extra, flags, tb, pr, out); }\n"
+              << "    template <int S, class TB, class PR, class L> __device__ __forceinline__ void tab_" << kind << "_yz(float a, float b, const TB& tb, const PR& pr, L out) const\n"
+              << "    { tape_tab_" << kind << "_yz<S>(0.0f, a, b, extra, flags, tb, pr, out); }\n"
+              << "    template <class PY, class PZ, class TB, class PR> __device__ __forceinline__ auto hoist_" << kind << "(PY py, PZ pz, const TB& tb, const PR& pr) const\n"
+              << "    { return tape_pre_" << kind << "(0.0f, py, pz, extra, flags, tb, pr); }\n";
+        }
+        o
           << "    template <class PX, class PY, class PZ, class H, class TB, class PR> __device__ __forceinline__ auto eval_hoisted_x(PX px, PY py, PZ pz, const H& h, const TB& tb, const PR& pr) const\n"
           << "    { return tape_eval_x(px, py, pz, extra, flags, h, tb, pr); }\n"
           << "    template <class PX, class PY, class PZ, class H, class TB, class PR> __device__ __forceinline__ auto dist_hoisted_x(PX px, PY py, PZ pz, const H& h, const TB& tb, const PR& pr) const\n"
```

After: 521,300 (median of 6 runs). +5.2%, better.
